# cvg/limap

Measured on AMD Instinct MI355X. Metric: 3D line candidates scored/sec (100 views x 500 segs per GPU, matched topk=10), higher is better.
Workload: dtype f64

## Files before the change

### limap_amd/csrc/lt_api_run.cpp

```cpp
#include "lt_host.h"

using namespace lt;
using namespace lt_impl;

extern "C" {

int lt_upload(lt_ctx *ctx) {
  LT_RANGE("lt_upload (match rows + job tables -> HBM)");
  LT_FINISH(ctx);
  if (!ctx->inited) return fail(ctx, LT_ERR_STATE, "upload before Init");
  if (ctx->uploaded) return LT_OK;
  HIPCHK(ctx, hipSetDevice(ctx->device));
  double t0 = now_ms();
  build_job_tables(ctx);
  ctx->blk_vorder_ok = false;
  int rc;
  {
    std::vector<char> need((size_t)std::max(ctx->n_img, 1), 0);
    for (size_t j = 0; j < ctx->job_imgs.size(); ++j) {
      need[(size_t)ctx->job_imgs[j]] = 1;
      for (int nb : ctx->job_nbs[j]) need[(size_t)nb] = 1;
    }
    std::vector<int> list;
    ctx->max_needed_segs = 0;
    for (int i = 0; i < ctx->n_img; ++i)
      if (need[(size_t)i]) {
        list.push_back(i);
        ctx->max_needed_segs = std::max(ctx->max_needed_segs, ctx->seg_off[i + 1] - ctx->seg_off[i]);
      }
    ctx->n_needed = (int)list.size();
    if (list.empty()) list.push_back(0);
    if ((rc = upload_vec(ctx, ctx->d_needed, list))) return rc;
  }
  if ((rc = upload_vec(ctx, ctx->d_nb_off, ctx->h_nb_off))) return rc;
  if ((rc = upload_vec(ctx, ctx->d_blk_img, ctx->h_blk_img))) return rc;
  if ((rc = upload_vec(ctx, ctx->d_blk_nb, ctx->h_blk_nb))) return rc;
  if ((rc = upload_vec(ctx, ctx->d_blk_slot, ctx->h_blk_slot))) return rc;
  if ((rc = upload_vec(ctx, ctx->d_blk_order, ctx->h_blk_order))) return rc;
  if ((rc = upload_vec(ctx, ctx->d_blk_line_base, ctx->h_blk_line_base))) return rc;
  if (ctx->job_mode == 1) {
    std::vector<long long> call_first_blk(ctx->job_imgs.size() + 1, 0);
    for (size_t j = 0; j < ctx->job_imgs.size(); ++j) call_first_blk[j + 1] = call_first_blk[j] + (long long)ctx->job_nbs[j].size();
    std::vector<int> job_pos(ctx->n_img, -1);
    for (size_t j = 0; j < ctx->job_imgs.size(); ++j) job_pos[ctx->job_imgs[j]] = (int)j;
    std::vector<long long> m_off(ctx->n_blk + 1, 0);
    std::vector<lt::RowDesc> desc((size_t)std::max(ctx->n_blk, 1));
    {
      long long b = 0;
      for (int i = 0; i < ctx->n_img; ++i) {
        int j = job_pos[i];
        if (j < 0) continue;
        for (size_t k = 0; k < ctx->job_nbs[j].size(); ++k, ++b) {
          long long cb = call_first_blk[j] + (long long)k;
          const long long n = ctx->h_m_off[cb + 1] - ctx->h_m_off[cb];
          m_off[b + 1] = m_off[b] + n;
          desc[(size_t)b] = lt::RowDesc{ctx->h_c_off[(size_t)cb], ctx->h_ovf_off[(size_t)cb], m_off[b], (int)n, ctx->h_line0[(size_t)cb]};
        }
      }
    }
    ctx->P = m_off[ctx->n_blk];
    ctx->n_conn = ctx->P;
    ctx->max_rows = 0;
    for (int bq = 0; bq < ctx->n_blk; ++bq) ctx->max_rows = std::max(ctx->max_rows, m_off[bq + 1] - m_off[bq]);
    if (ctx->P >= (1ll << 32) - 1) return fail(ctx, LT_ERR_ARGUMENT, "too many match rows in one batch (>= 2^32-1)");
    ENSURE(ctx, ctx->d_m_pairs, sizeof(int) * (size_t)std::max<long long>(ctx->P, 1));
    const size_t total_w = ctx->h_m_pairs.size();
    if (sizeof(int) * std::max<size_t>(total_w, 1) > ctx->d_c_stream.cap) {
      HIPCHK(ctx, hipStreamSynchronize(ctx->stream));
      ctx->streamed_ints = 0;
      ENSURE(ctx, ctx->d_c_stream, sizeof(int) * std::max<size_t>(total_w, 1));
    }
    {
      const size_t sent = std::min(ctx->streamed_ints, total_w);
      if (total_w > sent)
        HIPCHK(ctx, hipMemcpyAsync(ctx->d_c_stream.as<int>() + sent, ctx->h_m_pairs.data() + sent, sizeof(int) * (total_w - sent),
                                   hipMemcpyHostToDevice, ctx->stream));
      ctx->streamed_ints = total_w;
    }
    if ((rc = upload_vec(ctx, ctx->d_ovf, ctx->h_ovf))) return rc;
    if ((rc = upload_vec(ctx, ctx->d_rowdesc, desc))) return rc;
    const bool extras_cfg = (ctx->cfg.use_vp && !ctx->cfg.disable_vp_triangulation) ||
                            (ctx->pts_ready && (!ctx->cfg.disable_many_points_triangulation || !ctx->cfg.disable_one_point_triangulation));
    bool try_ln = ctx->rows_sorted && ctx->n_blk > 0 && ctx->P > 0 && ctx->max_nb_segs <= 1024 && !extras_cfg &&
                  !test_switch("LT_GEN_ROW_SLOTS") && !test_switch("LT_GEN_NO_LDS_TABLE");
    for (size_t cb = 0; try_ln && cb < ctx->h_ovf_off.size(); ++cb)
      if (ctx->h_ovf_off[cb] >= 0) try_ln = false;
    ctx->rows_ln = false;
    ctx->ln_slots = 0;
    if (try_ln) {
      ctx->ln_slots = gen_slots_ln(ctx->max_own_segs);
      const size_t n_entries = (size_t)std::max<long long>(ctx->h_blk_line_base[ctx->n_blk], 1);
      ENSURE(ctx, ctx->d_run_len, 4 * n_entries);
      ENSURE(ctx, ctx->d_base_bl, 4 * n_entries);
      ENSURE(ctx, ctx->d_slot_row0, 4 * (size_t)ctx->n_blk * (size_t)ctx->ln_slots);
      ENSURE(ctx, ctx->d_blk_nruns, 4 * (size_t)ctx->n_blk);
      ENSURE(ctx, ctx->d_ln_flag, 4);
      HIPCHK(ctx, hipMemsetAsync(ctx->d_ln_flag.p, 0, 4, ctx->stream));
      launch_rows_ln(ctx->stream, ctx->n_blk, ctx->ln_slots, ctx->d_rowdesc.p, ctx->d_c_stream.as<unsigned>(),
                     ctx->d_blk_line_base.as<long long>(), ctx->d_base_bl.as<unsigned>(), ctx->d_blk_nruns.as<int>(),
                     ctx->d_run_len.as<unsigned>(), ctx->d_slot_row0.as<unsigned>(), ctx->d_m_pairs.as<unsigned short>(),
                     ctx->d_ln_flag.as<int>());
      std::vector<unsigned> rnd0((size_t)ctx->n_blk + 1, 0u);
      for (int bq = 0; bq < ctx->n_blk; ++bq) rnd0[(size_t)bq + 1] = rnd0[(size_t)bq] + (unsigned)((m_off[bq + 1] - m_off[bq] + 63) / 64);
      ctx->n_round_slots = (long long)rnd0[(size_t)ctx->n_blk];
      if ((rc = upload_vec(ctx, ctx->d_blk_rnd0, rnd0))) return rc;
      int flag = 0;
      HIPCHK(ctx, hipMemcpyAsync(&flag, ctx->d_ln_flag.p, 4, hipMemcpyDeviceToHost, ctx->stream));
      HIPCHK(ctx, hipStreamSynchronize(ctx->stream));
      ctx->rows_ln = flag == 0;
    }
    if (!ctx->rows_ln)
      launch_expand_rows(ctx->stream, ctx->n_blk, ctx->d_rowdesc.p, ctx->d_c_stream.as<unsigned>(), ctx->d_ovf.as<unsigned>(),
                         ctx->d_m_pairs.as<unsigned>());
    if ((rc = upload_vec(ctx, ctx->d_m_off, m_off))) return rc;
    {
      std::vector<int> vo((size_t)std::max(ctx->n_blk, 1), 0);
      for (int b = 0; b < ctx->n_blk; ++b) vo[(size_t)b] = b;
      std::stable_sort(vo.begin(), vo.begin() + ctx->n_blk, [&](int x, int y) {
        return ctx->h_blk_nb[(size_t)x] != ctx->h_blk_nb[(size_t)y] ? ctx->h_blk_nb[(size_t)x] < ctx->h_blk_nb[(size_t)y]
                                                                    : ctx->h_blk_img[(size_t)x] < ctx->h_blk_img[(size_t)y];
      });
      if ((rc = upload_vec(ctx, ctx->d_blk_vorder, vo))) return rc;
      ctx->blk_vorder_ok = true;
    }
    ENSURE(ctx, ctx->d_blkrec, blk_rec_bytes() * (size_t)std::max(ctx->n_blk, 1));
    launch_build_blk(ctx->stream, ctx->n_blk, ctx->d_m_off.as<long long>(), ctx->d_blk_img.as<int>(),
                     ctx->d_blk_nb.as<int>(), ctx->d_blk_slot.as<int>(), ctx->d_seg_off.as<long long>(),
                     ctx->d_blk_line_base.as<long long>(), ctx->d_blkrec.p);
  } else if (ctx->job_mode == 2) {
    ctx->h_item_off.assign(ctx->G + 1, 0);
    std::vector<int> blk_chunk_off((size_t)std::max(ctx->n_blk, 1), 0);
    ctx->max_chunks = 1;
    long long items = 0, conns = 0;
    for (int i = 0; i < ctx->n_img; ++i) {
      long long per_node = 0, conn_node = 0;
      for (long long b = ctx->h_nb_off[i]; b < ctx->h_nb_off[i + 1]; ++b) {
        int i2 = ctx->h_blk_nb[b];
        long long M2 = ctx->seg_off[i2 + 1] - ctx->seg_off[i2];
        blk_chunk_off[(size_t)b] = (int)per_node;
        ctx->max_chunks = std::max(ctx->max_chunks, (int)((M2 + 63) / 64));
        per_node += (M2 + 63) / 64;
        conn_node += M2;
      }
      for (long long g = ctx->seg_off[i]; g < ctx->seg_off[i + 1]; ++g) {
        ctx->h_item_off[g] = items;
        items += per_node;
        conns += conn_node;
      }
    }
    ctx->h_item_off[ctx->G] = items;
    ctx->P = items;
    ctx->n_conn = conns;
    if ((rc = upload_vec(ctx, ctx->d_item_off, ctx->h_item_off))) return rc;
// ... 36 lines not shown
  }
  ctx->stat_survivors = -1;
  if (derr == 5) {
    if (ctx->ex_retry_depth > 0 || !ctx->ex_staged_set[ctx->pend_set])
      return fail(ctx, LT_ERR_RUNTIME, "internal: candidate staging overflow outside the one-pass exhaustive mode");
    ctx->ex_two_pass = true;
    if (hp && hp[3] > 0 && ctx->n_conn > 0)
      ctx->ex_frac = 1.4 * (double)hp[3] * (double)ex_regions() / (double)ctx->n_conn;
    if (ctx->in_run_async) return LT_OK;
    ctx->ex_retry_depth = 1;
    int rc2 = lt_run_device_async(ctx);
    if (!rc2) rc2 = finish_run(ctx);
    ctx->ex_retry_depth = 0;
    return rc2;
  }
  if (derr == 8) {
    if (ctx->score_two_kernels)
      return fail(ctx, LT_ERR_RUNTIME, "internal: device flag 8 outside the one-kernel scoring form");
    ctx->score_two_kernels = true;
    if (ctx->in_run_async) return LT_OK;
    const int depth = ctx->ex_retry_depth;
    ctx->ex_retry_depth = depth + 1;
    int rc2 = lt_run_device_async(ctx);
    if (!rc2) rc2 = finish_run(ctx);
    ctx->ex_retry_depth = depth;
    return rc2;
  }
  if (derr == 7) {
    if (ctx->ex_retry_depth > 1)
      return fail(ctx, LT_ERR_RUNTIME, "internal: pair chunk overflow outside the split scoring form");
    ctx->score_fused = true;
    if (ctx->in_run_async) return LT_OK;
    const int depth = ctx->ex_retry_depth;
    ctx->ex_retry_depth = depth + 1;
    int rc2 = lt_run_device_async(ctx);
    if (!rc2) rc2 = finish_run(ctx);
    ctx->ex_retry_depth = depth;
    return rc2;
  }
  ctx->timers[17] = ctx->timers[18] = 0.0;
  if (hp && ctx->ex_staged_set[ctx->pend_set]) {
    ctx->timers[17] = (double)hp[3] * (double)ex_regions();
    ctx->timers[18] = (double)ctx->ex_region_cap * (double)ex_regions();
  }
  if (ctx->job_mode == 2 && derr == 0 && ctx->n_conn > 0) {
    if (hp && ctx->ex_staged_set[ctx->pend_set])
      ctx->ex_frac = std::max(1.4 * (double)hp[3] * (double)ex_regions() / (double)ctx->n_conn, 1e-4);
    else if (ctx->ex_frac <= 0.0)
      ctx->ex_frac = std::max(2.2 * (double)ctx->C_last / (double)ctx->n_conn, 1e-4);
    ctx->ex_two_pass = false;
  }
  if (derr == 4) return fail(ctx, LT_ERR_RUNTIME, "internal: the scan of the node counts did not complete");
  if (derr == 3)
    return fail(ctx, LT_ERR_RUNTIME, "more than 65 000 candidates on one connection of the exhaustive mode (16-bit counts)");
  if (derr == 2)
    return fail(ctx, LT_ERR_RUNTIME, "map::at: a point shared by two lines has a point3D_id that is not among the SfM points");
  if (derr != 0) return fail(ctx, LT_ERR_RUNTIME, "IndexError! Out-of-index matches detected on the device");
  float ms;
  ctx->timers[1] = ctx->timers[2] = ctx->timers[7] = 0.0;
  const int eg = ctx->pend_ev_gen_end, ep = ctx->pend_ev_place_end;
  const hipEvent_t e_start = ctx->pend_ev_start ? ctx->pend_ev_start : ev[0];
  const hipEvent_t e_end = hp ? ctx->pend_ev_end : ev[7];
  HIPCHK(ctx, hipEventElapsedTime(&ms, e_start, e_end));
  ctx->timers[0] = ms;
  const bool sampled = ctx->pend_sampled;
  if (sampled) {
  const hipEvent_t kA[4] = {e_start, ev[eg], ev[ep], ev[5]}, kB[4] = {ev[eg], ev[ep], ev[5], e_end};
  const int kT[4] = {3, 4, 5, 6};
  for (int k = 0; k < 4; ++k) {
    HIPCHK(ctx, hipEventElapsedTime(&ms, kA[k], kB[k]));
    ctx->timers[kT[k]] = ms;
  }
  ctx->timers[13] = ctx->timers[14] = ctx->timers[15] = 0.0;
  if (ctx->pend_fine_gen && ctx->job_mode == 1 && ctx->n_blk > 0 && ctx->max_rows > 0) {
    if (hipEventElapsedTime(&ms, ev[8], ev[9]) == hipSuccess) ctx->timers[13] = ms;
    if (hipEventElapsedTime(&ms, ev[9], ev[10]) == hipSuccess) ctx->timers[14] = ms;
  }
  if (ctx->pend_fine_score && ctx->C_last > 0 && hipEventElapsedTime(&ms, ev[11], ev[5]) == hipSuccess) ctx->timers[15] = ms;
  (void)hipGetLastError();
  ++ctx->timer_stage_runs;
  }
  ctx->timers[11] = (double)ctx->stat_pairs_eval;
  for (int k = 0; k < 24; ++k) {
    const bool stage = (k >= 3 && k <= 6) || (k >= 13 && k <= 15);
    if (k != 8 && k != 9 && k != 10 && k != 12 && k != 16 && (sampled || !stage)) ctx->timer_sums[k] += ctx->timers[k];
  }
  ++ctx->timer_runs;
  return LT_OK;
}
}
}
int lt_sync(lt_ctx *ctx) { return finish_run(ctx); }

int lt_run_device_async(lt_ctx *ctx) {
  LT_RANGE("lt_run_device (enqueue: generation, placement, scoring, selection)");
  if (!ctx->uploaded) return fail(ctx, LT_ERR_STATE, "lt_run_device before lt_upload");
  if (!ctx->h_pinned) LT_FINISH(ctx);
  ctx->shard_keys = ctx->shard_own_keys = -1;
  if (ctx->inited && !ctx->best_c_set.empty())
    for (int idx : ctx->job_imgs)
      if (ctx->best_c_set[(size_t)idx] == 1) {
        ctx->best_c_set[(size_t)idx] = 0;
        for (long long g = ctx->seg_off[idx]; g < ctx->seg_off[idx + 1]; ++g) {
          if ((size_t)g < ctx->has_best.size()) ctx->has_best[(size_t)g] = 0;
          if ((size_t)g < ctx->valid_edges.cnt.size()) ctx->valid_edges.cnt[(size_t)g] = 0;
        }
      }
  const int set = ctx->run_pending ? (ctx->pend_set ^ 1) : 0;
  if (ctx->h_pinned) std::memset(ctx->h_pinned + 8 * set, 0, 32);
  if (set == 1 && !ctx->ev_b[0])
    for (auto &e : ctx->ev_b) HIPCHK(ctx, hipEventCreate(&e));
  hipEvent_t *ev = set ? ctx->ev_b : ctx->ev;
  long long *hp = ctx->h_pinned ? ctx->h_pinned + 8 * set : nullptr;
  ctx->ex_staged_set[set] = false;
  int sample_n = 8;
  if (const char *e = getenv("LT_TIMER_SAMPLE")) sample_n = std::max(1, atoi(e));
  if (!(ctx->run_pending && hp)) ctx->async_seq = 0;
  const bool sampled = (ctx->async_seq++ % (unsigned)sample_n) == 0u;
  const bool fine_gen = sampled && fine_gen_timers(), fine_score = sampled && fine_timers();
  HIPCHK(ctx, hipSetDevice(ctx->device));
  hipStream_t st = ctx->stream;
  const long long G = ctx->G, P = ctx->P;
  {
    int rcp = upload_points(ctx);
    if (rcp) return rcp;
  }
  GenCfg gcfg = make_gen(ctx);
  if (ctx->pts_ready && (!ctx->cfg.disable_many_points_triangulation || !ctx->cfg.disable_one_point_triangulation))
    gcfg.force_undecided = 1;
  const ScoreCfg scfg = make_score(ctx);
  const bool score_f32 = !test_switch("LT_TEST_SCORE_F64");
  const bool guards_on = scfg.l3.th_scaleinv > 0.0 && scfg.l3.score_th > 0.0 && scfg.l3.score_th < 1.0 &&
                         !test_switch("LT_TEST_NO_SCORE_GUARDS");
  const double guard2 = guards_on ? (scfg.l3.th_scaleinv * (1.0 + 1e-6)) * (scfg.l3.th_scaleinv * (1.0 + 1e-6)) : 1e300;
  ENSURE(ctx, ctx->d_err, sizeof(int));
  ENSURE(ctx, ctx->d_pair_counter, 8);
  ENSURE(ctx, ctx->d_result3, 32);
  ENSURE(ctx, ctx->d_pairs, sizeof(PairRec) * (size_t)std::max(ctx->n_blk, 1));
  ENSURE(ctx, ctx->d_tri_off, sizeof(long long) * (size_t)(G + 1));
  hipEvent_t ev_start = ev[0];
  if (ctx->run_pending && hp && ctx->pend_ev_end && !test_switch("LT_TEST_OWN_START_EVENT")) ev_start = ctx->pend_ev_end;
  else HIPCHK(ctx, hipEventRecord(ev[0], st));
  const int n_status_scan = (int)((G + 1 + 255) / 256) + 1;
  const int n_status = n_status_scan + score3_tile_buckets() * 16 + ex_regions() * 16 + 8 * 16;
  ENSURE(ctx, ctx->d_scan_status, 8 * (size_t)n_status);
  const bool ln_job = ctx->job_mode == 1 && ctx->rows_ln && ctx->rows_sorted;
  if (ln_job) ENSURE(ctx, ctx->d_blk_surv, 4 * (size_t)std::max(ctx->n_blk, 1));
  launch_build_pairs(st, ctx->n_blk, ctx->d_blk_img.as<int>(), ctx->d_blk_nb.as<int>(), ctx->d_cams.as<Cam>(),
                     ctx->d_pairs.as<PairRec>(), ctx->d_err.as<int>(),
                     ctx->d_pair_counter.as<unsigned long long>(), ctx->d_scan_status.as<unsigned long long>(),
                     n_status, ln_job ? ctx->d_blk_surv.as<unsigned>() : nullptr);

  bool node_rec_valid = false;
  long long C_known = -1;
  long long C_bound = 0;
  int ev_gen_end = 3, ev_place_end = 4;
  long long C_run = 0;
  if (ctx->job_mode == 1) {
    const size_t Pn = (size_t)std::max<long long>(P, 1);
    const bool fast = ctx->rows_sorted;
    {
      const bool vp_now = ctx->cfg.use_vp && !ctx->cfg.disable_vp_triangulation;
      const bool pts_now = ctx->pts_ready && (!ctx->cfg.disable_many_points_triangulation || !ctx->cfg.disable_one_point_triangulation);
      if (ctx->rows_ln && (vp_now || pts_now)) {
        launch_expand_rows(st, ctx->n_blk, ctx->d_rowdesc.p, ctx->d_c_stream.as<unsigned>(), ctx->d_ovf.as<unsigned>(),
                           ctx->d_m_pairs.as<unsigned>());
        ctx->rows_ln = false;
      }
    }
    const bool ln = ctx->rows_ln && fast;
    const int ln_slots = ln ? ctx->ln_slots : 0;
    if (ln) ENSURE(ctx, ctx->d_round_count, 4 * (size_t)std::max<long long>(ctx->n_round_slots, 1));
    const long long n_waves = (long long)ctx->n_blk * gen_groups(ctx->max_rows);
    const long long n_slots_all = (long long)ctx->n_blk * (ln ? ln_slots : gen_slots(ctx->max_rows));
    const long long n_entries = ctx->h_blk_line_base[ctx->n_blk];
    const bool vp_on = ctx->cfg.use_vp && !ctx->cfg.disable_vp_triangulation;
    if (vp_on && !ctx->vp_ready) return fail(ctx, LT_ERR_STATE, "use_vp is set but InitVPResults was not called");
    const bool pts_any = ctx->pts_ready && (!ctx->cfg.disable_many_points_triangulation || !ctx->cfg.disable_one_point_triangulation);
    const bool many_on = pts_any && !ctx->cfg.disable_many_points_triangulation;
    const bool one_on = pts_any && !ctx->cfg.disable_one_point_triangulation;
    const bool pts_on = pts_any;
    const bool extras = vp_on || pts_on;
    long long staged_total = -1;
    if (!extras) {
      ENSURE(ctx, ctx->d_st_c, sizeof(CRec) * Pn); ENSURE(ctx, ctx->d_st_l, sizeof(double) * Pn);
      ENSURE(ctx, ctx->d_st_key, 4 * (Pn + 64));
    }
    ENSURE(ctx, ctx->d_wave_count, 4 * (size_t)(n_waves + 1));
    if (extras) ENSURE(ctx, ctx->d_wave_pos, 8 * (size_t)(n_waves + 1));
    const long long *group_base = extras ? ctx->d_wave_pos.as<long long>() : nullptr;
    ENSURE(ctx, ctx->d_ntris_u, 4 * (size_t)(G + 1));
    if (fast) {
      const size_t nb = 4 * (size_t)std::max<long long>(n_entries, 1);
      const void *before = ctx->d_cnt_bl.p;
      ENSURE(ctx, ctx->d_cnt_bl, nb);
      ENSURE(ctx, ctx->d_base_bl, nb);
      if (ctx->d_cnt_bl.p != before || !ctx->cnt_bl_clean || ctx->cnt_bl_bytes != nb) {
        HIPCHK(ctx, hipMemsetAsync(ctx->d_cnt_bl.p, 0, ctx->d_cnt_bl.cap, st));
        ctx->cnt_bl_bytes = nb;
      }
      ctx->cnt_bl_clean = false;
    }
    const bool no_lds_table = test_switch("LT_GEN_NO_LDS_TABLE") != nullptr;
    int lds_segs = (!no_lds_table && ctx->max_nb_segs <= 1024) ? ctx->max_nb_segs : 0;
    int lds_segs1 = (!no_lds_table && ctx->max_own_segs <= 1024) ? ctx->max_own_segs : 0;
    if (lds_segs + lds_segs1 > 1024) lds_segs1 = 0;
    if (ln) {
      lds_segs = std::max(ctx->max_nb_segs, 1);
      lds_segs1 = 0;
    }
    {
      ENSURE(ctx, ctx->d_st_row, 8 * Pn);
      ENSURE(ctx, ctx->d_surv_count, 4 * (size_t)(n_slots_all + 1));
      if (!ctx->d_seg_gates.p) return fail(ctx, LT_ERR_STATE, "segment gate records missing (Init not run?)");
      auto gen = [&](int phase) {
      launch_gen_split(st, ctx->n_blk, ctx->max_rows, gcfg, ctx->d_m_off.as<long long>(), ctx->d_m_pairs.as<int>(),
                       ctx->d_blk_img.as<int>(), ctx->d_blk_nb.as<int>(), ctx->d_blk_slot.as<int>(),
                       ctx->d_seg_off.as<long long>(), ctx->d_cams.as<Cam>(), ctx->d_segs.as<Seg>(),
                       ctx->d_pairs.as<PairRec>(), ctx->d_blk_line_base.as<long long>(), ctx->d_st_c.as<CRec>(),
                       ctx->d_st_l.as<double>(), ctx->d_st_key.as<unsigned>(), ctx->d_wave_count.as<unsigned>(),
                       fast ? ctx->d_cnt_bl.as<unsigned>() : nullptr, lds_segs, lds_segs1, ctx->d_st_row.p,
                       ctx->d_surv_count.as<unsigned>(), G, ctx->d_seg_gates.p, ctx->d_blkrec.p, fine_gen ? &ev[8] : nullptr,
                       vp_on ? ctx->d_seg_vp.as<double>() : nullptr,
                       vp_on ? ctx->d_seg_has_vp.as<unsigned char>() : nullptr,
                       pts_on ? ctx->d_seg_pt_off.as<long long>() : nullptr, pts_on ? ctx->d_seg_pts.p : nullptr,
                       (pts_on && ctx->sfm_given) ? ctx->d_sfm_xyz.as<double>() : nullptr, ctx->d_err.as<int>(),
                       many_on ? 1 : 0, one_on ? 1 : 0, group_base, phase, ln_slots, ctx->d_m_pairs.as<unsigned short>(),
                       ctx->d_run_len.as<unsigned>(), ctx->d_slot_row0.as<unsigned>(), ctx->d_blk_surv.as<unsigned>(),
                       ctx->d_blk_rnd0.as<unsigned>(), ctx->d_round_count.as<unsigned>(),
                       (ctx->blk_vorder_ok && !test_switch("LT_TEST_GATES_IMAGE_MAJOR")) ? ctx->d_blk_vorder.as<int>() : nullptr,
                       test_switch("LT_TEST_TRI_STATIC") ? nullptr
                           : (unsigned *)(ctx->d_scan_status.as<unsigned long long>() + n_status_scan + score3_tile_buckets() * 16 + ex_regions() * 16));
      };
      if (!extras) {
        gen(0);
      } else {
        gen(1);
        HIPCHK(ctx, hipMemsetAsync(ctx->d_wave_count.as<unsigned>() + n_waves, 0, 4, st));
        size_t tmp = scan_temp_bytes_u32_to_i64(n_waves + 1);
        ENSURE(ctx, ctx->d_scan_tmp, std::max<size_t>(tmp, 16));
        if (launch_scan_u32_to_i64(st, ctx->d_scan_tmp.p, tmp, n_waves + 1, ctx->d_wave_count.as<unsigned>(),
                                   ctx->d_wave_pos.as<long long>()) != 0)
          return fail(ctx, LT_ERR_HIP, "rocprim scan failed");
        HIPCHK(ctx, hipMemcpyAsync(&staged_total, ctx->d_wave_pos.as<long long>() + n_waves, 8, hipMemcpyDeviceToHost, st));
        HIPCHK(ctx, hipStreamSynchronize(st));
        if (staged_total >= (1ll << 32) - 1)
          return fail(ctx, LT_ERR_ARGUMENT, "too many candidates in one batch (>= 2^32-1): triangulate the images in smaller batches");
        const size_t Sn = (size_t)std::max<long long>(staged_total, 1);
        ENSURE(ctx, ctx->d_st_c, sizeof(CRec) * Sn); ENSURE(ctx, ctx->d_st_l, sizeof(double) * Sn);
        ENSURE(ctx, ctx->d_st_key, 4 * Sn);
        gen(2);
      }
    }
    bool gen_event_pending = false;
    if (fine_gen && ctx->n_blk > 0 && ctx->max_rows > 0) ev_gen_end = 10;
    else gen_event_pending = true;
    long long *hC = hp;
    long long hC_fallback = 0;
    if (!hC) hC = &hC_fallback;
    if (fast) {
      ENSURE(ctx, ctx->d_node_rec, 16 * (size_t)std::max<long long>(G, 1));
      launch_node_prefix(st, G, ctx->d_node_img.as<int>(), ctx->d_seg_off.as<long long>(),
                         ctx->d_nb_off.as<long long>(), ctx->d_blk_line_base.as<long long>(),
                         ctx->d_cnt_bl.as<unsigned>(), ctx->d_base_bl.as<unsigned>(), ctx->d_ntris_u.as<unsigned>(),
                         ctx->d_tri_off.as<long long>(), ctx->d_scan_status.as<unsigned long long>(),
                         ctx->d_err.as<int>(), ctx->d_node_rec.p);
      node_rec_valid = true;
      ctx->cnt_bl_clean = true;
      const long long bound = P;
      constexpr long long kCountFreeBytes = 48ll << 30;
      const bool perm_bound = !test_switch("LT_TEST_PLACE_COPY");
      const long long per_cand = (perm_bound ? 4 : (long long)(sizeof(CRec) + 8)) + 8 + 4 + 4 + (long long)cand_meta_bytes() +
                                 (long long)score_split_entry_bytes() * 256 / 64;
      if (extras) {
        C_known = staged_total;
      } else if (ctx->h_pinned && bound * per_cand <= kCountFreeBytes && !test_switch("LT_TEST_SYNC_COUNT")) {
        C_known = -1;
        C_bound = bound;
      } else {
        HIPCHK(ctx, hipMemcpyAsync(hC, ctx->d_tri_off.as<long long>() + G, 8, hipMemcpyDeviceToHost, st));
        HIPCHK(ctx, hipStreamSynchronize(st));
        C_known = *hC;
      }
    } else {
      ENSURE(ctx, ctx->d_wave_pos, 8 * (size_t)(n_waves + 1));
      HIPCHK(ctx, hipMemsetAsync(ctx->d_wave_count.as<unsigned>() + n_waves, 0, 4, st));
      size_t tmp = scan_temp_bytes_u32_to_i64(n_waves + 1);
      ENSURE(ctx, ctx->d_scan_tmp, std::max<size_t>(tmp, 16));
      if (launch_scan_u32_to_i64(st, ctx->d_scan_tmp.p, tmp, n_waves + 1, ctx->d_wave_count.as<unsigned>(),
                                 ctx->d_wave_pos.as<long long>()) != 0)
        return fail(ctx, LT_ERR_HIP, "rocprim scan failed");
      HIPCHK(ctx, hipMemcpyAsync(hC, ctx->d_wave_pos.as<long long>() + n_waves, 8, hipMemcpyDeviceToHost, st));
      HIPCHK(ctx, hipStreamSynchronize(st));
      C_known = *hC;
    }
    const bool perm_mode = fast && !test_switch("LT_TEST_PLACE_COPY");
    ctx->perm_mode = perm_mode;
    ctx->compact_valid = !perm_mode;
    if (C_known < 0) {
      const size_t Bn = (size_t)std::max<long long>(C_bound, 1);
      const bool got = (perm_mode ? ctx->d_place_perm.ensure(4 * Bn)
                                  : (ctx->d_cand.ensure(sizeof(CRec) * Bn) && ctx->d_lite.ensure(sizeof(double) * Bn))) &&
                       ctx->d_score.ensure(8 * Bn) && ctx->d_edge_flag.ensure(4 * Bn) && ctx->d_cand_node.ensure(4 * Bn) &&
                       ctx->d_cand_meta.ensure(cand_meta_bytes() * Bn);
      if (!got) {
        (void)hipGetLastError();
        HIPCHK(ctx, hipMemcpyAsync(hC, ctx->d_tri_off.as<long long>() + G, 8, hipMemcpyDeviceToHost, st));
        HIPCHK(ctx, hipStreamSynchronize(st));
        C_known = *hC;
      }
    }
    if (C_known >= 0) C_bound = C_known;
    const size_t Cn = (size_t)std::max<long long>(C_bound, 1);
    if (perm_mode) {
      ENSURE(ctx, ctx->d_place_perm, 4 * Cn);
    } else {
      ENSURE(ctx, ctx->d_cand, sizeof(CRec) * Cn); ENSURE(ctx, ctx->d_lite, sizeof(double) * Cn);
    }
    ENSURE(ctx, ctx->d_score, 8 * Cn); ENSURE(ctx, ctx->d_edge_flag, 4 * Cn); ENSURE(ctx, ctx->d_cand_node, 4 * Cn);
    ctx->cand_cap = (long long)Cn;
    if (fast) {
      launch_place(st, ctx->n_blk, ctx->max_rows, ctx->d_m_off.as<long long>(), ctx->d_blk_img.as<int>(),
                   ctx->d_seg_off.as<long long>(), ctx->d_blk_line_base.as<long long>(),
                   ctx->d_base_bl.as<unsigned>(), ctx->d_wave_count.as<unsigned>(), ctx->d_tri_off.as<long long>(),
                   ctx->d_st_c.as<CRec>(), ctx->d_st_l.as<double>(), ctx->d_st_key.as<unsigned>(),
                   ctx->d_cand.as<CRec>(), ctx->d_lite.as<double>(), ctx->d_cand_node.as<unsigned>(), group_base,
                   perm_mode ? ctx->d_place_perm.as<unsigned>() : nullptr, ctx->d_blk_surv.as<unsigned>(),
                   ctx->d_blk_rnd0.as<unsigned>(), ln ? ctx->d_round_count.as<unsigned>() : nullptr);
    } else {
      ENSURE(ctx, ctx->d_keys, 4 * Cn); ENSURE(ctx, ctx->d_rows, 4 * Cn);
      ENSURE(ctx, ctx->d_skeys, 4 * Cn); ENSURE(ctx, ctx->d_srows, 4 * Cn);
      launch_pack_keys(st, ctx->n_blk, ctx->max_rows, ctx->d_m_off.as<long long>(),
                       ctx->d_wave_count.as<unsigned>(), ctx->d_wave_pos.as<long long>(),
                       ctx->d_st_key.as<unsigned>(), ctx->d_keys.as<unsigned>(), ctx->d_rows.as<unsigned>(), group_base);
      if (C_known > 0) {
        int end_bit = bits_for(G + 1);
        size_t tmp = sort_temp_bytes(C_known, end_bit);
        ENSURE(ctx, ctx->d_sort_tmp, std::max<size_t>(tmp, 16));
        if (launch_sort(st, ctx->d_sort_tmp.p, tmp, C_known, ctx->d_keys.as<unsigned>(), ctx->d_skeys.as<unsigned>(),
                        ctx->d_rows.as<unsigned>(), ctx->d_srows.as<unsigned>(), end_bit) != 0)
          return fail(ctx, LT_ERR_HIP, "rocprim radix sort failed");
      }
      launch_node_offsets(st, C_known, G, ctx->d_skeys.as<unsigned>(), ctx->d_tri_off.as<long long>());
      launch_permute(st, C_known, ctx->d_skeys.as<unsigned>(), ctx->d_srows.as<unsigned>(), ctx->d_st_c.as<CRec>(),
                     ctx->d_st_l.as<double>(), ctx->d_cand.as<CRec>(), ctx->d_lite.as<double>(),
                     ctx->d_cand_node.as<unsigned>());
    }
    if (fine_score && C_bound > 0) ev_place_end = 11;
    else if (sampled) HIPCHK(ctx, hipEventRecord(ev[4], st));
    if (gen_event_pending) ev_gen_end = ev_place_end;
  } else if (ctx->job_mode == 2) {
    ctx->perm_mode = false;
    ctx->compact_valid = true;
    const size_t In = (size_t)std::max<long long>(P, 1);
    const bool vp_on = ctx->cfg.use_vp && !ctx->cfg.disable_vp_triangulation;
    if (vp_on && !ctx->vp_ready) return fail(ctx, LT_ERR_STATE, "use_vp is set but InitVPResults was not called");
    const double *seg_vp = vp_on ? ctx->d_seg_vp.as<double>() : nullptr;
    const unsigned char *seg_has_vp = vp_on ? ctx->d_seg_has_vp.as<unsigned char>() : nullptr;
    const int n_masks = vp_on ? 3 : 1;
    const bool pts_any = ctx->pts_ready && (!ctx->cfg.disable_many_points_triangulation || !ctx->cfg.disable_one_point_triangulation);
    const int many_on = (pts_any && !ctx->cfg.disable_many_points_triangulation) ? 1 : 0;
    const int one_on = (pts_any && !ctx->cfg.disable_one_point_triangulation) ? 1 : 0;
    const double *sfm_xyz = (pts_any && ctx->sfm_given) ? ctx->d_sfm_xyz.as<double>() : nullptr;
    ENSURE(ctx, ctx->d_masks, pts_any ? 128 * In : 8 * (In * n_masks + 1)); ENSURE(ctx, ctx->d_mask_cnt, 4 * (In + 1));
    ENSURE(ctx, ctx->d_mask_pos, 8 * (In + 1));
    const bool plain = !pts_any && !vp_on;
    bool staged = plain && ctx->h_pinned && !ctx->ex_two_pass && P > 0 && !test_switch("LT_TEST_EX_TWO_PASS") &&
                  !test_switch("LT_TEST_EX_PASS1_BLOCK");
    long long ex_cap = 0;
    unsigned region_cap = 0;
    unsigned long long *ex_ctr = ctx->d_scan_status.as<unsigned long long>() + n_status_scan + score3_tile_buckets() * 16;
    if (staged) {
      double frac = ctx->ex_frac > 0.0 ? ctx->ex_frac : 1.0 / 6.0;
      long long slack = 65536;
      if (const char *f = test_switch("LT_TEST_EX_CAP_FRAC")) {
        frac = atof(f);
        slack = 0;
      }
      const long long want = (long long)((double)ctx->n_conn * frac) + slack;
      const long long nreg = ex_regions();
      const long long rc8 = ((want + nreg - 1) / nreg + 63) & ~63ll;
      ex_cap = nreg * rc8;
      if (ex_cap >= (1ll << 32) - 1 || ex_cap * 210 > (64ll << 30)) staged = false;
      else {
        region_cap = (unsigned)rc8;
        const size_t Bn = (size_t)ex_cap;
        const bool got = ctx->d_st_c.ensure(sizeof(CRec) * Bn) && ctx->d_st_l.ensure(sizeof(double) * Bn) &&
                         ctx->d_st_key.ensure(4 * Bn) && ctx->d_place_perm.ensure(4 * Bn) && ctx->d_score.ensure(8 * Bn) &&
                         ctx->d_edge_flag.ensure(4 * Bn) && ctx->d_cand_node.ensure(4 * Bn) &&
                         ctx->d_cand_meta.ensure(cand_meta_bytes() * Bn) && ctx->d_ex_rec.ensure(4 * Bn) &&
                         ctx->d_ex_ent.ensure(8 * Bn) && ctx->d_ex_z.ensure(4 * Bn);
        if (!got) {
          (void)hipGetLastError();
          staged = false;
        }
      }
    }
    ctx->ex_staged_set[set] = staged;
    if (pts_any) {
      launch_gen_exhaustive_pts(st, false, P, gcfg, ctx->d_item_off.as<long long>(), G, ctx->d_node_img.as<int>(),
                                ctx->d_nb_off.as<long long>(), ctx->d_blk_nb.as<int>(), ctx->d_seg_off.as<long long>(),
                                ctx->d_cams.as<Cam>(), ctx->d_segs.as<Seg>(), ctx->d_pairs.as<PairRec>(),
                                ctx->d_masks.as<unsigned short>(), ctx->d_mask_cnt.as<unsigned>(), nullptr, nullptr,
                                nullptr, seg_vp, seg_has_vp, ctx->d_seg_pt_off.as<long long>(), ctx->d_seg_pts.p,
                                sfm_xyz, ctx->d_err.as<int>(), many_on, one_on, ctx->d_blk_chunk_off.as<int>(),
                                ctx->max_nb, ctx->max_chunks, ctx->d_seg_gates.p);
    } else {
      if (plain && !test_switch("LT_TEST_EX_PASS1_BLOCK"))
        launch_gates_exhaustive(st, ctx->n_blk, ctx->max_chunks, P, gcfg, ctx->d_item_off.as<long long>(),
                                ctx->d_blk_img.as<int>(), ctx->d_blk_nb.as<int>(), ctx->d_seg_off.as<long long>(),
                                ctx->d_cams.as<Cam>(), ctx->d_segs.as<Seg>(), ctx->d_pairs.as<PairRec>(),
                                ctx->d_masks.as<unsigned long long>(), ctx->d_blk_chunk_off.as<int>(), ctx->d_seg_gates.p,
                                staged ? ctx->d_ex_ent.as<unsigned long long>() : nullptr, ex_ctr, region_cap,
                                ctx->d_err.as<int>());
      else
      launch_gen_exhaustive(st, false, P, gcfg, ctx->d_item_off.as<long long>(), G, ctx->d_node_img.as<int>(),
                            ctx->d_nb_off.as<long long>(), ctx->d_blk_nb.as<int>(), ctx->d_seg_off.as<long long>(),
                            ctx->d_cams.as<Cam>(), ctx->d_segs.as<Seg>(), ctx->d_pairs.as<PairRec>(),
                            ctx->d_masks.as<unsigned long long>(), nullptr, nullptr, nullptr, seg_vp, seg_has_vp,
                            ctx->d_blk_chunk_off.as<int>(), ctx->max_nb, ctx->max_chunks, ctx->d_seg_gates.p);
      if (staged) {
        HIPCHK(ctx, hipMemsetAsync(ctx->d_masks.p, 0, 8 * In, st));
        launch_tri_exhaustive(st, ctx->d_ex_ent.as<unsigned long long>(), ex_ctr, region_cap, gcfg, P,
                              ctx->d_item_off.as<long long>(), ctx->d_blk_img.as<int>(), ctx->d_blk_nb.as<int>(),
                              ctx->d_nb_off.as<long long>(), ctx->d_seg_off.as<long long>(), ctx->d_cams.as<Cam>(),
                              ctx->d_segs.as<Seg>(), ctx->d_pairs.as<PairRec>(), ctx->d_blk_chunk_off.as<int>(),
                              ctx->d_masks.as<unsigned long long>(), ctx->d_st_c.as<CRec>(), ctx->d_st_l.as<double>(),
                              ctx->d_st_key.as<unsigned>(), ctx->d_ex_z.as<float>());
      }
      if (!plain) launch_popc(st, P, ctx->d_masks.as<unsigned long long>(), ctx->d_mask_cnt.as<unsigned>(), n_masks);
    }
    if (plain) {
      HIPCHK(ctx, hipMemsetAsync(ctx->d_masks.as<unsigned long long>() + P, 0, 8, st));
      size_t tmp = scan_temp_bytes_popc(P + 1);
      ENSURE(ctx, ctx->d_scan_tmp, std::max<size_t>(tmp, 16));
      if (launch_scan_popc(st, ctx->d_scan_tmp.p, tmp, P + 1, ctx->d_masks.as<unsigned long long>(),
                           ctx->d_mask_pos.as<long long>()) != 0)
        return fail(ctx, LT_ERR_HIP, "rocprim scan failed");
    } else {
      HIPCHK(ctx, hipMemsetAsync(ctx->d_mask_cnt.as<unsigned>() + P, 0, 4, st));
      size_t tmp = scan_temp_bytes_u32_to_i64(P + 1);
      ENSURE(ctx, ctx->d_scan_tmp, std::max<size_t>(tmp, 16));
      if (launch_scan_u32_to_i64(st, ctx->d_scan_tmp.p, tmp, P + 1, ctx->d_mask_cnt.as<unsigned>(),
                                 ctx->d_mask_pos.as<long long>()) != 0)
        return fail(ctx, LT_ERR_HIP, "rocprim scan failed");
    }
    if (staged) {
      launch_tri_offsets_ex(st, G, ctx->d_item_off.as<long long>(), ctx->d_mask_pos.as<long long>(), P, -1, ex_cap,
                            ctx->d_tri_off.as<long long>(), ctx->d_err.as<int>());
      if (sampled) HIPCHK(ctx, hipEventRecord(ev[3], st));
      launch_place_exhaustive(st, ex_ctr, region_cap, ctx->d_ex_ent.as<unsigned long long>(),
                              ctx->d_st_key.as<unsigned>(), ctx->d_item_off.as<long long>(),
                              ctx->d_blk_chunk_off.as<int>(), ctx->d_masks.as<unsigned long long>(),
                              ctx->d_mask_pos.as<long long>(), P, ctx->d_tri_off.as<long long>(), G,
                              ctx->d_place_perm.as<unsigned>(), (hp ? hp : ctx->d_result3.as<long long>()) + 3);
      ctx->ex_region_cap = region_cap;
      launch_cand_node(st, G, ctx->d_tri_off.as<long long>(), ctx->d_cand_node.as<unsigned>());
      ctx->perm_mode = true;
      ctx->compact_valid = false;
      ctx->cand_cap = ex_cap;
      C_known = -1;
      C_bound = ex_cap;
      if (sampled) HIPCHK(ctx, hipEventRecord(ev[4], st));
    } else {
    long long total = 0;
    HIPCHK(ctx, hipMemcpyAsync(&total, ctx->d_mask_pos.as<long long>() + P, 8, hipMemcpyDeviceToHost, st));
    HIPCHK(ctx, hipStreamSynchronize(st));
    if (sampled) HIPCHK(ctx, hipEventRecord(ev[3], st));
    const size_t Cn = (size_t)std::max<long long>(total, 1);
    ENSURE(ctx, ctx->d_cand, sizeof(CRec) * Cn); ENSURE(ctx, ctx->d_lite, sizeof(double) * Cn);
    ENSURE(ctx, ctx->d_score, 8 * Cn); ENSURE(ctx, ctx->d_edge_flag, 4 * Cn);
    ctx->cand_cap = (long long)Cn;
    if (pts_any)
      launch_gen_exhaustive_pts(st, true, P, gcfg, ctx->d_item_off.as<long long>(), G, ctx->d_node_img.as<int>(),
                                ctx->d_nb_off.as<long long>(), ctx->d_blk_nb.as<int>(), ctx->d_seg_off.as<long long>(),
                                ctx->d_cams.as<Cam>(), ctx->d_segs.as<Seg>(), ctx->d_pairs.as<PairRec>(),
                                ctx->d_masks.as<unsigned short>(), ctx->d_mask_cnt.as<unsigned>(),
                                ctx->d_mask_pos.as<long long>(), ctx->d_cand.as<CRec>(), ctx->d_lite.as<double>(),
                                seg_vp, seg_has_vp, ctx->d_seg_pt_off.as<long long>(), ctx->d_seg_pts.p, sfm_xyz,
                                ctx->d_err.as<int>(), many_on, one_on, ctx->d_blk_chunk_off.as<int>(), ctx->max_nb,
                                ctx->max_chunks, ctx->d_seg_gates.p);
    else if (!vp_on && !test_switch("LT_TEST_EX_PASS2_BLOCK"))
      launch_fill_exhaustive(st, ctx->n_blk, P, gcfg, ctx->d_item_off.as<long long>(), ctx->d_blk_img.as<int>(),
                             ctx->d_blk_nb.as<int>(), ctx->d_nb_off.as<long long>(), ctx->d_seg_off.as<long long>(),
                             ctx->d_cams.as<Cam>(), ctx->d_segs.as<Seg>(), ctx->d_pairs.as<PairRec>(),
                             ctx->d_masks.as<unsigned long long>(), ctx->d_mask_pos.as<long long>(),
                             ctx->d_cand.as<CRec>(), ctx->d_lite.as<double>(), ctx->d_blk_chunk_off.as<int>());
    else
      launch_gen_exhaustive(st, true, P, gcfg, ctx->d_item_off.as<long long>(), G, ctx->d_node_img.as<int>(),
                            ctx->d_nb_off.as<long long>(), ctx->d_blk_nb.as<int>(), ctx->d_seg_off.as<long long>(),
                            ctx->d_cams.as<Cam>(), ctx->d_segs.as<Seg>(), ctx->d_pairs.as<PairRec>(),
                            ctx->d_masks.as<unsigned long long>(), ctx->d_mask_pos.as<long long>(),
                            ctx->d_cand.as<CRec>(), ctx->d_lite.as<double>(), seg_vp, seg_has_vp,
                            ctx->d_blk_chunk_off.as<int>(), ctx->max_nb, ctx->max_chunks, ctx->d_seg_gates.p);
    launch_tri_offsets_ex(st, G, ctx->d_item_off.as<long long>(), ctx->d_mask_pos.as<long long>(), P, total, -1,
                          ctx->d_tri_off.as<long long>(), ctx->d_err.as<int>());
    ENSURE(ctx, ctx->d_cand_node, 4 * Cn);
    launch_cand_node(st, G, ctx->d_tri_off.as<long long>(), ctx->d_cand_node.as<unsigned>());
    C_known = total;
    C_bound = total;
    if (sampled) HIPCHK(ctx, hipEventRecord(ev[4], st));
    }
  } else {
    ctx->perm_mode = false;
    ctx->compact_valid = true;
    HIPCHK(ctx, hipMemsetAsync(ctx->d_tri_off.p, 0, sizeof(long long) * (size_t)(G + 1), st));
    ENSURE(ctx, ctx->d_cand, sizeof(CRec)); ENSURE(ctx, ctx->d_lite, sizeof(double));
    ENSURE(ctx, ctx->d_score, 8); ENSURE(ctx, ctx->d_edge_flag, 4); ENSURE(ctx, ctx->d_cand_node, 4);
    C_known = 0;
    C_bound = 0;
    for (int k = 3; k <= 4; ++k)
      if (sampled) HIPCHK(ctx, hipEventRecord(ev[k], st));
  }

  if (score3_lds_bytes(ctx->max_nb, score_f32) > 160 * 1024)
    return fail(ctx, LT_ERR_ARGUMENT, "too many neighbours for the scoring kernel's LDS budget");
  {
    if (ctx->h_nb_off[ctx->n_img] >= (1ll << 24))
      return fail(ctx, LT_ERR_ARGUMENT, "too many (image, neighbour) blocks in one batch (>= 2^24)");
    ENSURE(ctx, ctx->d_cand_meta, cand_meta_bytes() * (size_t)std::max<long long>(C_bound, 1));
    ENSURE(ctx, ctx->d_tile_order, 64 * 128);
    const bool tile_classes = !test_switch("LT_TEST_NO_TILE_CLASSES") && ctx->job_mode == 1;
    const unsigned tile_cap = (unsigned)(((std::max<long long>(C_bound, 1) + 63) / 64 + 7) / 8);
    if (tile_classes) ENSURE(ctx, ctx->d_tile_list, 16 * (size_t)tile_cap * (size_t)score3_tile_buckets());
    const bool score_sorted = score_f32 && ctx->job_mode == 2 && !test_switch("LT_TEST_SCORE_UNSORTED");
    if (score_sorted) {
      ENSURE(ctx, ctx->d_perm, 4 * (size_t)std::max<long long>(C_bound, 1));
      ENSURE(ctx, ctx->d_rng, 4 * (size_t)std::max<long long>(C_bound, 1));
    }
    const bool staged_sorted = score_sorted && ctx->perm_mode && ctx->job_mode == 2;
    C_run = C_bound;
    const bool split = score_f32 && !ctx->score_fused && !test_switch("LT_SCORE_FUSED") &&
                       (tile_classes || staged_sorted || test_switch("LT_SCORE_SPLIT"));
    long long sp_chunks = 0;
    int sp_slot_cap = ctx->job_mode == 2 ? 64 : 256;
    if (split) {
      const long long n_tiles_b = (std::max<long long>(C_bound, 1) + 63) / 64;
      sp_chunks = score_split_chunks(std::max<long long>(C_bound, 1));
      if (const char *e = test_switch("LT_TEST_SPLIT_CHUNKS")) sp_chunks = std::max(0, atoi(e));
      if (const char *e = test_switch("LT_TEST_SPLIT_SLOT")) sp_slot_cap = std::max(1, atoi(e));
      ENSURE(ctx, ctx->d_sp_slots, score_split_entry_bytes() * (size_t)sp_slot_cap * (size_t)n_tiles_b);
      ENSURE(ctx, ctx->d_sp_cnt, 4 * (size_t)n_tiles_b);
      ENSURE(ctx, ctx->d_sp_ovf, 4 * (size_t)n_tiles_b);
      ENSURE(ctx, ctx->d_sp_pairs, score_split_chunk_bytes() * (size_t)std::max<long long>(sp_chunks, 1));
      ENSURE(ctx, ctx->d_sp_desc, 8 * (size_t)std::max<long long>(sp_chunks, 1));
    }
    const bool pair_classes = split && tile_classes && !test_switch("LT_TEST_NO_PAIR_CLASSES");
    if (pair_classes) {
      ENSURE(ctx, ctx->d_pc_cnt, 128 * (size_t)score3_tile_buckets());
      ENSURE(ctx, ctx->d_pc_list, 8 * (size_t)tile_cap * (size_t)score3_tile_buckets());
    }
    launch_score3(st, C_bound, G, ctx->d_tri_off.as<long long>(), ctx->d_cand_node.as<unsigned>(), ctx->d_cand_meta.p,
                  ctx->perm_mode ? ctx->d_st_c.as<CRec>() : ctx->d_cand.as<CRec>(), ctx->d_node_img.as<int>(),
                  ctx->d_nb_off.as<long long>(), ctx->d_blk_order.as<int>(), ctx->d_cams.as<Cam>(),
                  ctx->d_score.as<double>(), ctx->d_pair_counter.as<unsigned long long>(), ctx->max_nb, scfg,
                  guard2, fine_score ? ev[11] : nullptr, ctx->d_tile_order.as<unsigned>(), score_f32,
                  (ctx->perm_mode && !staged_sorted) ? ctx->d_place_perm.as<unsigned>()
                                                     : (score_sorted ? ctx->d_perm.as<unsigned>() : nullptr),
                  score_sorted ? ctx->d_rng.p : nullptr, ctx->perm_mode && !staged_sorted,
                  tile_classes ? (unsigned *)(ctx->d_scan_status.as<unsigned long long>() + n_status_scan) : nullptr,
                  tile_classes ? ctx->d_tile_list.as<unsigned>() : nullptr, tile_cap,
                  staged_sorted ? ctx->d_place_perm.as<unsigned>() : nullptr,
                  staged_sorted ? ctx->d_ex_rec.as<unsigned>() : nullptr,
                  staged_sorted ? ctx->d_ex_z.as<float>() : nullptr, ctx->d_err.as<int>(),
                  split ? ctx->d_sp_slots.p : nullptr, sp_slot_cap, ctx->d_sp_cnt.as<unsigned>(),
                  ctx->d_sp_ovf.as<unsigned>(), ctx->d_sp_pairs.p, ctx->d_sp_desc.p, sp_chunks, sampled ? ev[5] : nullptr,
                  node_rec_valid ? ctx->d_node_rec.p : nullptr, pair_classes ? ctx->d_pc_cnt.as<unsigned>() : nullptr,
                  pair_classes ? ctx->d_pc_list.p : nullptr, tile_cap,
                  (((ctx->score_two_kernels || test_switch("LT_SCORE_TWO_KERNELS") || ctx->n_img >= (1 << 18))
                        ? 0 : (test_switch("LT_TEST_Q_LOSE_TILE") ? 2 : 1)) |
                   (test_switch("LT_TEST_DENSE_TABLES") ? 4 : 0) | (test_switch("LT_TEST_DENSE_FEW_ROWS") ? 8 : 0)));
    if (C_bound <= 0 && sampled) HIPCHK(ctx, hipEventRecord(ev[5], st));
  }
  ENSURE(ctx, ctx->d_best_idx, 8 * (size_t)std::max<long long>(G, 1));
  ENSURE(ctx, ctx->d_nvalid, 4 * (size_t)(G + 1));
  ENSURE(ctx, ctx->d_edge_off, 8 * (size_t)(G + 1));
  ENSURE(ctx, ctx->d_best_c, sizeof(Cand) * (size_t)std::max<long long>(G, 1));
  ENSURE(ctx, ctx->d_best_score, 8 * (size_t)std::max<long long>(G, 1));
  ENSURE(ctx, ctx->d_best_src, 8 * (size_t)std::max<long long>(G, 1));
  ENSURE(ctx, ctx->d_ntris, 4 * (size_t)std::max<long long>(G, 1));
  launch_select(st, G, ctx->d_tri_off.as<long long>(), ctx->d_score.as<double>(), scfg.fullscore_th,
                scfg.max_valid_conns, ctx->d_best_idx.as<long long>(), ctx->d_edge_flag.as<unsigned>(),
                ctx->d_nvalid.as<unsigned>(), ctx->perm_mode ? ctx->d_st_c.as<CRec>() : ctx->d_cand.as<CRec>(),
                ctx->perm_mode ? ctx->d_st_l.as<double>() : ctx->d_lite.as<double>(),
                ctx->d_best_c.as<Cand>(), ctx->d_best_score.as<double>(), ctx->d_best_src.as<int>(),
                ctx->d_ntris.as<int>(), ctx->job_mode == 2, ctx->d_err.as<int>(),
                ctx->d_pair_counter.as<unsigned long long>(), hp ? hp : ctx->d_result3.as<long long>(),
                ctx->perm_mode ? ctx->d_place_perm.as<unsigned>() : nullptr);
  if (!hp) HIPCHK(ctx, hipEventRecord(ev[7], st));
  HIPCHK(ctx, hipGetLastError());
  hipEvent_t ev_end = nullptr;
  if (hp) {
    if (!ctx->ev_end[0])
      for (auto &e : ctx->ev_end) HIPCHK(ctx, hipEventCreate(&e));
    ev_end = ctx->ev_end[ctx->run_seq++ % 3u];
    HIPCHK(ctx, hipEventRecord(ev_end, st));
  }
  int rc_prev = LT_OK;
  if (ctx->run_pending) {
    ctx->in_run_async = true;
    rc_prev = finish_run(ctx);
    ctx->in_run_async = false;
  }
  ctx->run_pending = true;
  ctx->pend_ev_start = ev_start;
  ctx->pend_sampled = sampled;
  ctx->pend_ev_end = ev_end;
  ctx->pend_set = set;
  ctx->pend_count_on_device = C_known < 0;
  ctx->pend_fine_gen = fine_gen;
  ctx->pend_fine_score = fine_score;
  ctx->pend_C = C_run;
  ctx->pend_ev_gen_end = ev_gen_end;
  ctx->pend_ev_place_end = ev_place_end;
  ctx->ran = true;
  ctx->downloaded = false;
  ctx->host_view_valid = false;
  return rc_prev;
}

int lt_run_device(lt_ctx *ctx) {
  int rc = lt_run_device_async(ctx);
  if (rc) return rc;
  return finish_run(ctx);
}

extern "C++" {
namespace lt_impl {
void define_best_of_other_images(lt_ctx *ctx) {
  for (int i = 0; i < ctx->n_img; ++i)
    if (!ctx->best_c_set[(size_t)i]) {
      const long long a = ctx->seg_off[i], b = ctx->seg_off[i + 1];
      if (b > a) std::memset((void *)(ctx->best_c + a), 0, sizeof(Cand) * (size_t)(b - a));
      ctx->best_c_set[(size_t)i] = 2;
    }
}
}
}

extern "C++" {
namespace lt_impl {
int materialize_compact(lt_ctx *ctx) {
  if (ctx->host_view_valid) return LT_OK;
  const long long C = ctx->C_last;
  const size_t Cn = (size_t)std::max<long long>(C, 1);
  ENSURE(ctx, ctx->d_hcand, sizeof(Cand) * Cn); ENSURE(ctx, ctx->d_hlite, sizeof(CandLite) * Cn);
  launch_host_view(ctx->stream, C, ctx->perm_mode ? ctx->d_place_perm.as<unsigned>() : nullptr,
                   ctx->perm_mode ? ctx->d_st_c.as<CRec>() : ctx->d_cand.as<CRec>(),
                   ctx->perm_mode ? ctx->d_st_l.as<double>() : ctx->d_lite.as<double>(), ctx->d_hcand.as<Cand>(),
                   ctx->d_hlite.as<CandLite>());
  HIPCHK(ctx, hipStreamSynchronize(ctx->stream));
  ctx->host_view_valid = true;
  return LT_OK;
}
}
}

int lt_download(lt_ctx *ctx) {
  LT_RANGE("lt_download (per-node results -> host)");
  LT_FINISH(ctx);
  if (!ctx->ran) return fail(ctx, LT_ERR_STATE, "lt_download before lt_run_device");
  if (ctx->downloaded) return LT_OK;
  HIPCHK(ctx, hipSetDevice(ctx->device));
  double t0 = now_ms();
  hipStream_t st = ctx->stream;
  const long long G = ctx->G;
  HIPCHK(ctx, hipMemsetAsync(ctx->d_nvalid.as<unsigned>() + G, 0, 4, st));
  {
    size_t tmp = scan_temp_bytes_u32_to_i64(G + 1);
    ENSURE(ctx, ctx->d_scan_tmp, std::max<size_t>(tmp, 16));
    if (launch_scan_u32_to_i64(st, ctx->d_scan_tmp.p, tmp, G + 1, ctx->d_nvalid.as<unsigned>(),
                               ctx->d_edge_off.as<long long>()) != 0)
      return fail(ctx, LT_ERR_HIP, "rocprim scan failed");
  }
  std::vector<long long> tri_off(G + 1), edge_off(G + 1);
  HIPCHK(ctx, hipMemcpyAsync(tri_off.data(), ctx->d_tri_off.p, 8 * (size_t)(G + 1), hipMemcpyDeviceToHost, st));
  HIPCHK(ctx, hipMemcpyAsync(edge_off.data(), ctx->d_edge_off.p, 8 * (size_t)(G + 1), hipMemcpyDeviceToHost, st));
  HIPCHK(ctx, hipStreamSynchronize(st));
  ctx->C = tri_off[G];
  ctx->E = edge_off[G];
  ENSURE(ctx, ctx->d_edges, 8 * (size_t)std::max<long long>(ctx->E, 1));
  launch_edge_fill(st, G, ctx->d_tri_off.as<long long>(), ctx->d_edge_flag.as<unsigned>(),
                   ctx->d_edge_off.as<long long>(), ctx->perm_mode ? ctx->d_st_c.as<CRec>() : ctx->d_cand.as<CRec>(),
                   ctx->d_edges.as<int>(), ctx->perm_mode ? ctx->d_place_perm.as<unsigned>() : nullptr);
  const size_t Gn = (size_t)std::max<long long>(G, 1), En = (size_t)std::max<long long>(ctx->E, 1);
  const size_t o_bc = 0, o_bs = o_bc + sizeof(Cand) * Gn, o_src = o_bs + 8 * Gn, o_nt = o_src + 8 * Gn,
               o_ed = (o_nt + 4 * Gn + 15) / 16 * 16, total = o_ed + 8 * En;
  lt_host::HostBlock hb = lt_host::host_block_acquire(total);
  if (!hb.p) return fail(ctx, LT_ERR_RUNTIME, "out of host memory for the results");
  struct Rel {
    lt_host::HostBlock b;
    ~Rel() { lt_host::host_block_release(b); }
  } rel{hb};
  char *base = (char *)hb.p;
  const Cand *bc = (const Cand *)(base + o_bc);
  const double *bs = (const double *)(base + o_bs);
  const int *bsrc = (const int *)(base + o_src);
  const int *nt = (const int *)(base + o_nt);
  const int *edges = (const int *)(base + o_ed);
  if (G > 0) {
    HIPCHK(ctx, hipMemcpyAsync(base + o_bc, ctx->d_best_c.p, sizeof(Cand) * (size_t)G, hipMemcpyDeviceToHost, st));
    HIPCHK(ctx, hipMemcpyAsync(base + o_bs, ctx->d_best_score.p, 8 * (size_t)G, hipMemcpyDeviceToHost, st));
    HIPCHK(ctx, hipMemcpyAsync(base + o_src, ctx->d_best_src.p, 8 * (size_t)G, hipMemcpyDeviceToHost, st));
    HIPCHK(ctx, hipMemcpyAsync(base + o_nt, ctx->d_ntris.p, 4 * (size_t)G, hipMemcpyDeviceToHost, st));
  }
  if (ctx->E > 0)
    HIPCHK(ctx, hipMemcpyAsync(base + o_ed, ctx->d_edges.p, 8 * (size_t)ctx->E, hipMemcpyDeviceToHost, st));
  HIPCHK(ctx, hipStreamSynchronize(st));
  const long long pool_base = (long long)ctx->valid_edges.pool.size();
  ctx->valid_edges.pool.insert(ctx->valid_edges.pool.end(), edges, edges + 2 * (size_t)ctx->E);
  long long pairs = 0;
  const long long n_job = (long long)ctx->job_imgs.size();
#pragma omp parallel for num_threads(lt::host_threads()) schedule(dynamic, 4) reduction(+ : pairs)
  for (long long j = 0; j < n_job; ++j) {
    const int idx = ctx->job_imgs[(size_t)j];
    ctx->best_c_set[(size_t)idx] = 1;
    for (long long g = ctx->seg_off[idx]; g < ctx->seg_off[idx + 1]; ++g) {
      ctx->n_tris[g] = nt[g];
      pairs += (long long)nt[g] * nt[g];
      ctx->has_best[g] = nt[g] > 0 ? 1 : 0;
      ctx->best_c[g] = bc[g];
      ctx->best_score[g] = bs[g];
      ctx->best_src2[2 * g] = nt[g] > 0 ? ctx->img_ids[bsrc[2 * g]] : 0;
      ctx->best_src2[2 * g + 1] = nt[g] > 0 ? bsrc[2 * g + 1] : 0;
// ... 55 lines not shown
```

### limap_amd/csrc/lt_devfn.h

```cpp
#pragma once

#include "lt_device.h"

namespace lt {

static __device__ __forceinline__ int lane_id() { return threadIdx.x & 63; }
static __device__ __forceinline__ unsigned long long lanemask_lt() {
  return (1ull << lane_id()) - 1ull;
}
template <class Op>
static __device__ __forceinline__ int wave_reduce_dpp(int v, Op op) {
  v = op(v, __builtin_amdgcn_update_dpp(v, v, 0x111, 0xF, 0xF, false));
  v = op(v, __builtin_amdgcn_update_dpp(v, v, 0x112, 0xF, 0xF, false));
  v = op(v, __builtin_amdgcn_update_dpp(v, v, 0x114, 0xF, 0xF, false));
  v = op(v, __builtin_amdgcn_update_dpp(v, v, 0x118, 0xF, 0xF, false));
  v = op(v, __builtin_amdgcn_update_dpp(v, v, 0x142, 0xA, 0xF, false));
  v = op(v, __builtin_amdgcn_update_dpp(v, v, 0x143, 0xC, 0xF, false));
  return __builtin_amdgcn_readlane(v, 63);
}
static __device__ __forceinline__ unsigned wave_incl_scan_u32(unsigned x) {
  int v = (int)x;
  v += __builtin_amdgcn_update_dpp(0, v, 0x111, 0xF, 0xF, true);
  v += __builtin_amdgcn_update_dpp(0, v, 0x112, 0xF, 0xF, true);
  v += __builtin_amdgcn_update_dpp(0, v, 0x114, 0xF, 0xF, true);
  v += __builtin_amdgcn_update_dpp(0, v, 0x118, 0xF, 0xF, true);
  v += __builtin_amdgcn_update_dpp(0, v, 0x142, 0xA, 0xF, true);
  v += __builtin_amdgcn_update_dpp(0, v, 0x143, 0xC, 0xF, true);
  return (unsigned)v;
}
static __device__ __forceinline__ int wave_max_i32(int v) {
  return wave_reduce_dpp(v, [](int a, int b) { return a > b ? a : b; });
}
static __device__ __forceinline__ unsigned wave_max_u32(unsigned v) {
  return (unsigned)wave_reduce_dpp((int)v, [](int a, int b) { return (unsigned)a > (unsigned)b ? a : b; });
}
static __device__ __forceinline__ unsigned wave_min_u32(unsigned v) {
  return (unsigned)wave_reduce_dpp((int)v, [](int a, int b) { return (unsigned)a < (unsigned)b ? a : b; });
}
static __device__ __forceinline__ float wave_max_f32_nan(float v) {
  return __int_as_float(wave_reduce_dpp(__float_as_int(v), [](int a, int b) {
    const float x = __int_as_float(a), y = __int_as_float(b);
    return (y > x || y != y) ? b : a;
  }));
}
static __device__ __forceinline__ double readlane_f64(double v, int src) {
  const int lo = __builtin_amdgcn_readlane(__double2loint(v), src);
  const int hi = __builtin_amdgcn_readlane(__double2hiint(v), src);
  return __hiloint2double(hi, lo);
}

static __device__ __forceinline__ void wave_lds_sync() {
  asm volatile("s_waitcnt lgkmcnt(0)" ::: "memory");
  __builtin_amdgcn_wave_barrier();
}


struct GenOut {
  CRec r;
  double unc;
};

static __device__ __forceinline__ bool tri_point(const Cam &c1, d3 r1, const Cam &c2, d3 r2, d3 *out) {
  d3 C1 = cam_center(c1), C2 = cam_center(c2);
  double a00 = dot(r1, r1), a10 = -dot(r2, r1), a11 = dot(r2, r2);
  double b0 = dot(r1, sub(C2, C1));
  double b1 = dot(r2, sub(C1, C2));
  bool sw = fabs(a11) > fabs(a00);
  double dd0 = sw ? a11 : a00, dd1 = sw ? a00 : a11;
  double q0 = sw ? b1 : b0, q1 = sw ? b0 : b1;
  double l10 = a10 / dd0;
  double s1d = dd1 - l10 * (dd0 * l10);
  double y1 = q1 - l10 * q0;
  double z0 = q0 / dd0, z1 = y1 / s1d;
  double s0 = z0 - l10 * z1;
  double x0 = sw ? z1 : s0, x1 = sw ? s0 : z1;
  d3 p = add(add(add(scale(r1, x0), C1), scale(r2, x1)), C2);
  p = d3{0.5 * p.x, 0.5 * p.y, 0.5 * p.z};
  if (cam_depth(c1, p) < kEps || cam_depth(c2, p) < kEps) return false;
  *out = p;
  return true;
}

static __device__ __forceinline__ double sensitivity(const Cam &c, d3 s, d3 e, d3 dir3) {
  d2 ps = cam_project(c, s), pe = cam_project(c, e);
  d2 mid = d2{0.5 * (ps.x + pe.x), 0.5 * (ps.y + pe.y)};
  d3 ray = cam_ray(c, mid);
  double cv = fabs(dot(dir3, ray));
  return 90 - acos(cv) * 180.0 / kPi;
}

static __device__ __forceinline__ bool sensitivity_gt(const GenCfg &cfg, const Cam &c, d3 s, d3 e, d3 dir3) {
  d2 ps = cam_project(c, s), pe = cam_project(c, e);
  d2 mid = d2{0.5 * (ps.x + pe.x), 0.5 * (ps.y + pe.y)};
  d3 ray = cam_ray(c, mid);
  double cv = fabs(dot(dir3, ray));
  if (cv > cfg.sens_hi) return true;
  if (cv < cfg.sens_lo) return false;
  return 90 - acos(cv) * 180.0 / kPi > cfg.sens_th;
}

static __device__ __forceinline__ double epipolar_iou(const Seg &s1, const Seg &s2, const double *F) {
  L2 l2{mk2(s2.x1, s2.y1), mk2(s2.x2, s2.y2)};
  double ln2 = len(l2);
  d3 lc2 = mk3(s2.lc[0], s2.lc[1], s2.lc[2]);
  d3 eps = unit(mv(F, mk3(s1.x1, s1.y1, 1.0)));
  d3 hs = cross(lc2, eps);
  double zs = hs.z + kEps;
  d2 cs = d2{hs.x / zs, hs.y / zs};
  d3 epe = unit(mv(F, mk3(s1.x2, s1.y2, 1.0)));
  d3 he = cross(lc2, epe);
  double ze = he.z + kEps;
  d2 ce = d2{he.x / ze, he.y / ze};
  d2 dv = dir(l2);
  double c1v = dot(sub(cs, l2.s), dv) / ln2;
  double c2v = dot(sub(ce, l2.s), dv) / ln2;
  if (c1v > c2v) {
    double t = c1v; c1v = c2v; c2v = t;
  }
  return (dmin(c2v, 1.0) - dmax(c1v, 0.0)) / (dmax(c2v, 1.0) - dmin(c1v, 0.0));
}

static __device__ __forceinline__ bool tri_line(const Cam &c1, const Cam &c2, const Seg &s1, const Seg &s2,
                                                const double *Bv, d3 *ps_o, d3 *pe_o, double *z_start,
                                                double *z_end, double *d21, double *d22) {
  d3 r1s = mk3(s1.rs[0], s1.rs[1], s1.rs[2]), r1e = mk3(s1.re[0], s1.re[1], s1.re[2]);
  d3 c2s = mk3(s2.rs[0], s2.rs[1], s2.rs[2]), c2e = mk3(s2.re[0], s2.re[1], s2.re[2]);
  d3 u = mk3(-c2s.x, -c2s.y, -c2s.z), v = mk3(-c2e.x, -c2e.y, -c2e.z);
  double k0 = u.y * v.z - v.y * u.z;
  double k1 = u.z * v.x - v.z * u.x;
  double k2 = u.x * v.y - v.x * u.y;
  d3 B = mk3(Bv[0], Bv[1], Bv[2]);
  d3 C1 = cam_center(c1);
  d3 ps, pe;
  {
    double det = (k0 * r1s.x + k1 * r1s.y) + k2 * r1s.z;
    double id = 1.0 / det;
    double x0 = ((k0 * id) * B.x + (k1 * id) * B.y) + (k2 * id) * B.z;
    ps = add(scale(r1s, x0), C1);
    *z_start = cam_depth(c1, ps);
  }
  {
    double det = (k0 * r1e.x + k1 * r1e.y) + k2 * r1e.z;
    double id = 1.0 / det;
    double x0 = ((k0 * id) * B.x + (k1 * id) * B.y) + (k2 * id) * B.z;
    pe = add(scale(r1e, x0), C1);
    *z_end = cam_depth(c1, pe);
  }
  *ps_o = ps;
  *pe_o = pe;
  if (*z_start < kEps || *z_end < kEps) return false;
  *d21 = cam_depth(c2, ps);
  *d22 = cam_depth(c2, pe);
  if (*d21 < kEps || *d22 < kEps) return false;
  if (isnan(ps.x) || isnan(pe.x)) return false;
  return true;
}

static __device__ __forceinline__ bool gen_gates(const GenCfg &cfg, const Seg &s1, const Seg &s2,
                                                 const double *F) {
  L2 l1{mk2(s1.x1, s1.y1), mk2(s1.x2, s1.y2)};
  L2 l2{mk2(s2.x1, s2.y1), mk2(s2.x2, s2.y2)};
  if (len(l1) <= cfg.min_length_2d) return false;
  if (len(l2) <= cfg.min_length_2d) return false;
  if (cfg.disable_algebraic) return false;
  d3 n2 = mk3(s2.n[0], s2.n[1], s2.n[2]);
  d3 r1s = mk3(s1.rs[0], s1.rs[1], s1.rs[2]), r1e = mk3(s1.re[0], s1.re[1], s1.re[2]);
  double as = fabs(dot(n2, r1s));
  if (as < cfg.sin_lo) return false;
  if (!(as > cfg.sin_hi)) {
    double ang = 90 - acos(as) * 180.0 / kPi;
    if (ang < cfg.angle_th) return false;
  }
  double ae = fabs(dot(n2, r1e));
  if (ae < cfg.sin_lo) return false;
  if (!(ae > cfg.sin_hi)) {
    double ang = 90 - acos(ae) * 180.0 / kPi;
    if (ang < cfg.angle_th) return false;
  }
  double iou = epipolar_iou(s1, s2, F);
  if (iou < cfg.iou_th) return false;
  return true;
}

static __device__ __forceinline__ double fast_rcp(double x) {
  double r = __builtin_amdgcn_rcp(x);
  r = __builtin_fma(__builtin_fma(-x, r, 1.0), r, r);
  r = __builtin_fma(__builtin_fma(-x, r, 1.0), r, r);
  return r;
}

struct SegGate {
  double n[3];
  double lcx, lcy;
  double P, Q, w1;
  double sv;
  double q2;
};
static_assert(sizeof(SegGate) == 80, "SegGate layout");

static __device__ __forceinline__ void seg_gate_build(const Seg &s, SegGate *g) {
  const double vx = s.x2 - s.x1, vy = s.y2 - s.y1;
  g->n[0] = s.n[0]; g->n[1] = s.n[1]; g->n[2] = s.n[2];
  g->lcx = s.lc[0]; g->lcy = s.lc[1];
  g->P = s.lc[2] * vy;
  g->Q = -(s.lc[2] * vx);
  g->w1 = s.lc[1] * vx - s.lc[0] * vy;
// ... 620 lines not shown
```

### limap_amd/csrc/lt_device.h

```cpp
#pragma once

#include "lt_geom.h"

#include <hip/hip_runtime.h>
#include <stddef.h>

#define LT_ERR_MATCH_LINE_RANGE 1
#define LT_ERR_MATCH_NGLINE_RANGE 2

namespace lt {

struct SceneChunk {
  const double *k, *q, *t, *s;
  long long seg_begin;
  int img_begin, pad_;
};
void launch_build_scene_chunked(hipStream_t st, int n_img, long long n_segs, int n_chunks, const SceneChunk *ch,
                                const long long *seg_off, double halfpix, Cam *cams, Seg *segs,
                                const int *img_list, int n_list, long long max_segs_per_img, void *gates);

void launch_build_cams(hipStream_t st, int n, const double *k, const double *q, const double *t, Cam *cams);
void launch_build_segs(hipStream_t st, long long n_segs, int n_img, const long long *seg_off,
                       const double *segs, double halfpix, const Cam *cams, Seg *out, void *gates);
void launch_build_pairs(hipStream_t st, int n_blk, const int *blk_img, const int *blk_nb, const Cam *cams,
                        PairRec *out, int *err_flag, unsigned long long *pair_counter,
                        unsigned long long *scan_status, int n_status, unsigned *blk_surv);
size_t sort_temp_bytes(long long P, int end_bit);
int launch_sort(hipStream_t st, void *temp, size_t temp_bytes, long long P, const unsigned *keys_in,
                unsigned *keys_out, const unsigned *vals_in, unsigned *vals_out, int end_bit);
void launch_node_offsets(hipStream_t st, long long P, long long G, const unsigned *skeys, long long *conn_off);
size_t scan_temp_bytes_u32_to_i64(long long n);
size_t scan_temp_bytes_popc(long long n);
int launch_scan_popc(hipStream_t st, void *temp, size_t temp_bytes, long long n, const unsigned long long *masks,
                     long long *out);
int launch_scan_u32_to_i64(hipStream_t st, void *temp, size_t temp_bytes, long long n, const unsigned *in,
                           long long *out);
void launch_gen_exhaustive(hipStream_t st, bool fill, long long n_items, const GenCfg &cfg,
                           const long long *item_off, long long G, const int *node_img, const long long *nb_off,
                           const int *blk_nb, const long long *seg_off, const Cam *cams, const Seg *segs,
                           const PairRec *pairs, unsigned long long *masks, const long long *mask_pos,
                           CRec *out_r, double *out_unc, const double *seg_vp, const unsigned char *seg_has_vp,
                           const int *blk_chunk_off, int max_nb, int max_chunks, const void *gates);
int ex_regions();
void launch_gates_exhaustive(hipStream_t st, int n_blk, int max_chunks, long long n_items, const GenCfg &cfg,
                             const long long *item_off, const int *blk_img, const int *blk_nb, const long long *seg_off,
                             const Cam *cams, const Seg *segs, const PairRec *pairs, unsigned long long *masks,
                             const int *blk_chunk_off, const void *gates, unsigned long long *ent_out,
                             unsigned long long *ctr, unsigned region_cap, int *err_flag);
void launch_tri_exhaustive(hipStream_t st, unsigned long long *ent, const unsigned long long *ctr,
                           unsigned region_cap, const GenCfg &cfg, long long n_items, const long long *item_off,
                           const int *blk_img, const int *blk_nb, const long long *nb_off, const long long *seg_off,
                           const Cam *cams, const Seg *segs, const PairRec *pairs, const int *blk_chunk_off,
                           unsigned long long *masks, CRec *st_r, double *st_unc, unsigned *st_node, float *st_z);
void launch_place_exhaustive(hipStream_t st, const unsigned long long *ctr, unsigned region_cap,
                             const unsigned long long *ent, const unsigned *st_node, const long long *item_off,
                             const int *blk_chunk_off, const unsigned long long *masks, const long long *mask_pos,
                             long long n_items, const long long *tri_off, long long G, unsigned *perm,
                             long long *fill_out);
void launch_fill_exhaustive(hipStream_t st, int n_blk, long long n_items, const GenCfg &cfg, const long long *item_off,
                            const int *blk_img, const int *blk_nb, const long long *nb_off, const long long *seg_off,
                            const Cam *cams, const Seg *segs, const PairRec *pairs, const unsigned long long *masks,
                            const long long *mask_pos, CRec *out_r, double *out_unc, const int *blk_chunk_off);
void launch_gen_exhaustive_pts(hipStream_t st, bool fill, long long n_items, const GenCfg &cfg,
                               const long long *item_off, long long G, const int *node_img, const long long *nb_off,
                               const int *blk_nb, const long long *seg_off, const Cam *cams, const Seg *segs,
                               const PairRec *pairs, unsigned short *cnt8, unsigned *item_cnt,
                               const long long *mask_pos, CRec *out_r, double *out_unc, const double *seg_vp,
                               const unsigned char *seg_has_vp, const long long *seg_pt_off, const void *seg_pts,
                               const double *sfm_xyz, int *err_flag, int many_on, int one_on,
                               const int *blk_chunk_off, int max_nb, int max_chunks, const void *gates);
void launch_popc(hipStream_t st, long long n, const unsigned long long *masks, unsigned *cnt, int n_masks);
void launch_tri_offsets_ex(hipStream_t st, long long G, const long long *item_off, const long long *mask_pos,
                           long long n_items, long long total, long long cap, long long *tri_off, int *err_flag);

void launch_select(hipStream_t st, long long G, const long long *tri_off, const double *score, double th,
                   int max_valid, long long *best_idx, unsigned *edge_flag, unsigned *n_valid, const CRec *cand,
                   const double *cand_unc, Cand *best_c, double *best_score, int *best_src2, int *n_tris,
                   bool wide, const int *err_flag, const unsigned long long *pair_counter, long long *result3,
                   const unsigned *perm);
void launch_edge_fill(hipStream_t st, long long G, const long long *tri_off, const unsigned *edge_flag,
                      const long long *edge_off, const CRec *cand, int *edges2, const unsigned *perm);

size_t tail_rec_bytes();
size_t tail_sort_temp_bytes(long long E, int end_bit);
void launch_tail_keys(hipStream_t st, long long G, const long long *tri_off, const unsigned *edge_flag,
                      const long long *edge_off, const CRec *cand, const long long *seg_off, int kb,
                      unsigned long long *keys, const unsigned *perm, int directed);
int launch_tail_sort(hipStream_t st, void *temp, size_t temp_bytes, long long E, const unsigned long long *keys_in,
                     unsigned long long *keys_out, int end_bit);
void launch_tail_sims(hipStream_t st, long long E, const unsigned long long *skeys, const int *n_tris, const Cand *best_c,
                      const LinkCfg3 &cfg, int kb, double *sims, unsigned *mark, unsigned *keep, const unsigned char *flags);
void launch_check_keys(hipStream_t st, long long n, const unsigned long long *keys, int kb, long long G, int *bad, int directed);
void launch_outer_pass_keys(hipStream_t st, long long E, const unsigned long long *keys, int kb, long long G, unsigned *counts,
                            int min_outer, unsigned char *flags, int *changed);
void launch_keys_undirect(hipStream_t st, long long E, unsigned long long *keys, int kb);
void launch_outer_filter(hipStream_t st, long long G, const long long *tri_off, const unsigned *edge_flag, const CRec *cand,
                         const long long *seg_off, const unsigned *perm, int min_outer, unsigned char *flags, int *changed);
void launch_tail_compact(hipStream_t st, long long E, const unsigned long long *skeys, const double *sims,
                         const unsigned *keep, const long long *kpos, void *out_pairs, long long *n_out, const long long *npos,
                         int kb);
void launch_tail_gather(hipStream_t st, long long G, const unsigned *mark, const long long *pos, const Cand *best_c,
                        const double *best_score, const int *best_src2, void *recs, int *nodes, long long *n_out);

struct MLine {
  double s[3], e[3];
  double dir[3];
  double unc;
  double len;
  double seg[4];
  double pad_;
};
static_assert(sizeof(MLine) == 128, "MLine layout");
struct MBlock {
  int img, nb, slot, row0;
  int img_id, nb_id, pad_[2];
};
struct MEdge {
  int img, line, slot, ng_line;
};
void launch_merge_pairs(hipStream_t st, bool self, int n_blk, const MBlock *blks, const long long *seg_off,
                        const MLine *lines, const Cam *cams, const LinkCfg2 &l2, const LinkCfg3 &l3, double cos_guard,
                        int parity_fast, MEdge *edges, unsigned long long capacity, unsigned long long *n_edges);

void launch_track_connect(hipStream_t st, int T, const double *line7, const unsigned char *active, int all_active,
                          const LinkCfg3 &cfg, double cos_guard, unsigned long long *edges,
                          unsigned long long capacity, unsigned long long *n_edges);

}
```

### limap_amd/csrc/lt_host.h

```cpp
#pragma once

#include "lt_ctx.h"
#include "lt_hostutil.h"
#include "lt_tail.h"
#include "lt_rows.h"
#include "lt_pool.h"

#include <algorithm>
#include <atomic>
#include <parallel/algorithm>
#include <chrono>
#include <cmath>
#include <cstdio>
#include <cstring>
#include <dlfcn.h>
#include <map>
#include <mutex>
#include <queue>
#include <set>
#include <string>
#include <unordered_map>
#include <vector>

namespace lt {
void launch_fn_query(hipStream_t st, const double *in30, int by_endpoints, double *out32);
void launch_fn_gate_outcomes(hipStream_t st, int n, const double *conn30, const GenCfg &cfg, int *out10,
                             unsigned long long *iou_bits);
int gen_slots(long long max_rows);
int gen_groups(long long max_rows);
int gen_slots_ln(int max_own_segs);
int gen_max_run();
void launch_rows_ln(hipStream_t st, int n_blk, int n_slots, const void *desc, const unsigned *stream,
                    const long long *blk_line_base, unsigned *rstart, int *blk_nruns, unsigned *run_len,
                    unsigned *slot_row0, unsigned short *tr, int *ln_flag);
size_t seg_gate_bytes();
void launch_build_blk(hipStream_t st, int n_blk, const long long *m_off, const int *blk_img, const int *blk_nb,
                      const int *blk_slot, const long long *seg_off, const long long *blk_line_base, void *blkrec);
size_t blk_rec_bytes();
void launch_gen_split(hipStream_t st, int n_blk, long long max_rows, const GenCfg &cfg, const long long *m_off,
                      const int *m_pairs, const int *blk_img, const int *blk_nb, const int *blk_slot,
                      const long long *seg_off, const Cam *cams, const Seg *segs, const PairRec *pairs,
                      const long long *blk_line_base, CRec *st_r, double *st_unc, unsigned *st_key,
                      unsigned *wave_count, unsigned *cnt_bl, int lds_segs, int lds_segs1, void *st_row,
                      unsigned *surv_count, long long n_segs, void *gates, void *blkrec, hipEvent_t *ev3,
                      const double *seg_vp, const unsigned char *seg_has_vp, const long long *seg_pt_off,
                      const void *seg_pts, const double *sfm_xyz, int *err_flag, int many_on, int one_on,
                      const long long *group_base, int phase, int ln_slots, const unsigned short *tr,
                      const unsigned *run_len, const unsigned *slot_row0, unsigned *blk_surv, const unsigned *blk_rnd0,
                      unsigned *round_count, const int *blk_vorder, unsigned *tri_unit_ctr);
size_t seg_point_bytes();
void launch_node_prefix(hipStream_t st, long long G, const int *node_img, const long long *seg_off,
                        const long long *nb_off, const long long *blk_line_base, unsigned *cnt_bl,
                        unsigned *base_bl, unsigned *n_tris, long long *tri_off, unsigned long long *status,
                        int *err_flag, void *node_rec);
void launch_expand_rows(hipStream_t st, int n_blk, const void *desc, const unsigned *stream, const unsigned *ovf, unsigned *rows);
void launch_place(hipStream_t st, int n_blk, long long max_rows, const long long *m_off, const int *blk_img,
                  const long long *seg_off, const long long *blk_line_base, const unsigned *base_bl,
                  const unsigned *wave_count, const long long *tri_off, const CRec *st_r, const double *st_unc,
                  const unsigned *st_key, CRec *cand, double *cand_unc, unsigned *cand_node, const long long *group_base,
                  unsigned *perm, const unsigned *blk_surv, const unsigned *blk_rnd0, const unsigned *round_count);
void launch_pack_keys(hipStream_t st, int n_blk, long long max_rows, const long long *m_off,
                      const unsigned *wave_count, const long long *wave_pos, const unsigned *st_key,
                      unsigned *keys_c, unsigned *src_c, const long long *group_base);
void launch_permute(hipStream_t st, long long C, const unsigned *skeys, const unsigned *ssrc, const CRec *st_r,
                    const double *st_unc, CRec *cand, double *cand_unc, unsigned *cand_node);
void launch_host_view(hipStream_t st, long long C, const unsigned *perm, const CRec *rec, const double *unc, Cand *out_c,
                      CandLite *out_l);
void launch_cand_node(hipStream_t st, long long G, const long long *tri_off, unsigned *cand_node);
size_t score3_lds_bytes(int max_nb, bool f32);
size_t cand_meta_bytes();
void launch_score3(hipStream_t st, long long C, long long G, const long long *tri_off, const unsigned *cand_node,
                   void *meta, const CRec *cand, const int *node_img, const long long *nb_off,
                   const int *blk_order, const Cam *cams, double *score, unsigned long long *pair_counter,
                   int max_nb, const ScoreCfg &cfg, double scaleinv_guard2, hipEvent_t ev_before, unsigned *draw,
                   bool f32, unsigned *perm, void *rng, bool perm_is_placement, unsigned *bucket_cnt,
                   unsigned *bucket_list, unsigned bucket_cap, const unsigned *place, unsigned *rec, const float *st_z,
                   int *err_flag, void *sp_slots, int sp_slot_cap, unsigned *sp_cnt, unsigned *sp_ovf, void *sp_pairs,
                   void *sp_desc, long long sp_chunks, hipEvent_t ev_after, const void *node_rec, unsigned *pc_cnt,
                   void *pc_list, unsigned pc_cap, int one_kernel);
size_t score_split_chunk_bytes();
size_t score_split_entry_bytes();
long long score_split_chunks(long long C);
int score3_tile_buckets();
}

namespace lt_trace {
struct Range {
  bool on;
  explicit Range(const char *name);
  ~Range();
};
}
#define LT_CONCAT2(a, b) a##b
#define LT_CONCAT(a, b) LT_CONCAT2(a, b)
#define LT_RANGE(name) lt_trace::Range LT_CONCAT(lt_range_, __LINE__)(name)

namespace lt_impl {
const char *test_switch(const char *name);
int fine_level();
bool fine_timers();
bool fine_gen_timers();
double now_ms();
double multiplier(double score_th);
lt::LinkCfg2 make_l2(const lt_config &c);
lt::LinkCfg3 make_l3(const lt_config &c);
lt::GenCfg make_gen(const lt_ctx *ctx);
lt::ScoreCfg make_score(const lt_ctx *ctx);
int bits_for(long long n);
void build_job_tables(lt_ctx *ctx);
int upload_points(lt_ctx *ctx);
int finish_run(lt_ctx *ctx);
void define_best_of_other_images(lt_ctx *ctx);
int materialize_compact(lt_ctx *ctx);
int refine_with_ctx_cams(lt_ctx *ctx, int64_t n_tracks, const double *line6, const int64_t *off, const int32_t *img,
                         const double *line2d4, const double *line3d6, const lt_refine_config *cfg);
}

#define LT_FINISH(ctx)                       \
  do {                                       \
    int rc_fin_ = lt_impl::finish_run(ctx);  \
    if (rc_fin_) return rc_fin_;             \
  } while (0)
```

### limap_amd/csrc/lt_kernels_score.hip

```cpp

#include "lt_devfn.h"

#include <hip/hip_ext.h>

#include <algorithm>

namespace lt {

#ifndef LT_SCORE_WIN
#define LT_SCORE_WIN 128
#endif
#ifndef LT_SCORE_RESIDENT
#define LT_SCORE_RESIDENT 16
#endif
#ifdef LT_SCORE_WAVES_PER_EU
#define LT_SCORE_OCC __attribute__((amdgpu_waves_per_eu(LT_SCORE_WAVES_PER_EU, LT_SCORE_WAVES_PER_EU)))
#else
#define LT_SCORE_OCC
#endif

#ifdef LT_TRACE
__device__ unsigned long long g_trace[4 * 4 * 65536];
#define LT_TRACE_MARK(kern, id, slot) \
  if (((kern) == 3 ? threadIdx.x == 0 : lane_id() == 0) && (id) < 65536u) g_trace[(kern) * 4 * 65536 + 4 * (id) + (slot)] = wall_clock64()
#else
#define LT_TRACE_MARK(kern, id, slot)
#endif

static inline unsigned nblk2(long long n, int bs) { return (unsigned)((n + bs - 1) / bs); }

struct CandMeta {
  unsigned off_lo, off_hi;
  unsigned n;
  unsigned nb;
};

constexpr int kTileQueues = 8;
constexpr int kTileBuckets = 32;
__device__ __forceinline__ int tile_bucket(unsigned cost_sum_n) {
  const unsigned b = cost_sum_n >> 7;
  return (int)(b < (unsigned)(kTileBuckets - 1) ? b : (unsigned)(kTileBuckets - 1));
}
__global__ void __launch_bounds__(256)
k_cand_meta(long long G, const unsigned *__restrict__ cand_node, const long long *__restrict__ tri_off,
            const int *__restrict__ node_img, const long long *__restrict__ nb_off, CandMeta *__restrict__ meta,
            unsigned *__restrict__ draw, unsigned *__restrict__ bucket_cnt, unsigned *__restrict__ bucket_list,
            unsigned bucket_cap, const uint4 *__restrict__ node_rec, unsigned *__restrict__ pc_cnt,
            uint2 *__restrict__ fifo, unsigned fifo_cap) {
  const long long C = tri_off[G];
  const long long stride = (long long)gridDim.x * blockDim.x;
  long long i = (long long)blockIdx.x * blockDim.x + threadIdx.x;
  if (pc_cnt && i < kTileQueues * kTileBuckets) pc_cnt[i * 32] = 0;
  if (i < 2 * kTileQueues + 1) draw[i * 32] = 0;
  if (fifo) {
    if (i >= 2 * kTileQueues + 1 && i < 3 * kTileQueues + 1) draw[i * 32] = 0xFFFFFFFFu;
    if (i >= 3 * kTileQueues + 1 && i < 4 * kTileQueues + 1) draw[i * 32] = 0;
    const long long per = ((C + 63) / 64 + kTileQueues - 1) / kTileQueues;
    for (long long j = i; j < per * kTileQueues; j += stride)
      fifo[(size_t)(j / per) * fifo_cap + (size_t)(j % per)] = make_uint2(0xFFFFFFFFu, 0u);
  }
  const long long C_up = (C + 63) & ~63ll;
  for (; i < C_up; i += stride) {
    unsigned n = 0, w_lo = 0, w_hi = 0;
    if (i < C) {
      const unsigned g = cand_node[i];
      CandMeta m;
      if (node_rec) {
        const uint4 r = node_rec[g];
        m.off_lo = r.x; m.off_hi = r.y; m.n = r.z; m.nb = r.w;
      } else {
        const long long off = tri_off[g];
        const int img = node_img[g];
        const long long nb0 = nb_off[img];
        m.off_lo = (unsigned)(off & 0xFFFFFFFFll);
        m.off_hi = (unsigned)(off >> 32);
        m.n = (unsigned)(tri_off[g + 1] - off);
        m.nb = ((unsigned)nb0 << 8) | (unsigned)(nb_off[img + 1] - nb0);
      }
      meta[i] = m;
      n = m.n;
      w_lo = m.off_lo; w_hi = m.off_lo + m.n;
    }
    if (bucket_cnt) {
      unsigned sum = n;
      for (int d = 32; d >= 1; d >>= 1) sum += (unsigned)__shfl_xor((int)sum, d);
      const long long base = i - lane_id();
      const int last = (int)((C - base) < 64 ? (C - base) : 64) - 1;
      const unsigned t_hi = (unsigned)__builtin_amdgcn_readlane((int)w_hi, last);
      if (lane_id() == 0) {
        const unsigned tile = (unsigned)(i >> 6);
        const int qb = (int)(tile & (kTileQueues - 1)) * kTileBuckets + tile_bucket(sum);
        const unsigned idx = atomicAdd(&bucket_cnt[qb * 32], 1u);
        if (idx < bucket_cap)
          reinterpret_cast<uint4 *>(bucket_list)[(size_t)qb * bucket_cap + idx] = uint4{tile, w_lo, t_hi, 0u};
      }
    }
  }
}

__global__ void __launch_bounds__(256)
k_cand_node(long long G, const long long *__restrict__ tri_off, unsigned *__restrict__ cand_node) {
  long long g = ((long long)blockIdx.x * blockDim.x + threadIdx.x) >> 6;
  if (g >= G) return;
  for (long long t = tri_off[g] + lane_id(); t < tri_off[g + 1]; t += 64) cand_node[t] = (unsigned)g;
}

static __device__ __forceinline__ unsigned mt_key(long long off) { return (unsigned)off & 0xFFFFFFu; }
constexpr int kSQCap = 512;
constexpr int kSQCapSplit = 384;
constexpr int kWin = LT_SCORE_WIN;

struct Score3Args {
  long long G;
  const long long *tri_off;
  const CandMeta *meta;
  const CRec *cand;
  const int *blk_order;
  const Cam *cams;
  double *score;
  unsigned long long *pair_counter;
  unsigned *draw;
  const unsigned *perm;
  const unsigned *spos;
  const unsigned *rng;
  const unsigned *bucket_cnt;
  const unsigned *bucket_list;
  unsigned bucket_cap;
  int max_nb;
  int *err_flag;
  uint4 *sp_slots;
  unsigned *sp_cnt;
  unsigned *sp_ovf;
  uint4 *sp_pairs;
  uint2 *sp_desc;
  unsigned *sp_counters;
  unsigned sp_chunk_cap;
  int sp_slot_cap;
  int sp_t_max;
  int sp_wave_lds;
  unsigned *pc_cnt;
  uint2 *pc_list;
  unsigned pc_cap;
};
__device__ __forceinline__ int pair_bucket(unsigned pairs) {
  const unsigned b = pairs >> 4;
  return (int)(b < (unsigned)(kTileBuckets - 1) ? b : (unsigned)(kTileBuckets - 1));
}

constexpr int kChunkCap = 512;
constexpr int kChunkTiles = 8;
constexpr unsigned kNoChunk = 0xFFFFFFFFu;
constexpr int kErrPairChunks = 7;
constexpr int kDenseHdrBytes = 16 + kChunkTiles * 8 + 256 * 4 + 64 * 4;

constexpr int kSortMax = 2048;

template <int kX>
static __device__ __forceinline__ unsigned lane_xor(unsigned x, int lane) {
  if constexpr (kX == 1) return (unsigned)__builtin_amdgcn_update_dpp(0, (int)x, 0xB1, 0xF, 0xF, true);
  else if constexpr (kX == 2) return (unsigned)__builtin_amdgcn_update_dpp(0, (int)x, 0x4E, 0xF, 0xF, true);
  else if constexpr (kX == 3) return (unsigned)__builtin_amdgcn_update_dpp(0, (int)x, 0x1B, 0xF, 0xF, true);
  else if constexpr (kX == 7) return (unsigned)__builtin_amdgcn_update_dpp(0, (int)x, 0x141, 0xF, 0xF, true);
  else if constexpr (kX == 4) return lane_xor<3>(lane_xor<7>(x, lane), lane);
  else if constexpr (kX == 8) return (unsigned)__builtin_amdgcn_update_dpp(0, (int)x, 0x128, 0xF, 0xF, true);
  else if constexpr (kX == 15) return (unsigned)__builtin_amdgcn_update_dpp(0, (int)x, 0x140, 0xF, 0xF, true);
  else if constexpr (kX == 16) {
    const auto p = __builtin_amdgcn_permlane16_swap(x, x, false, false);
    return (lane & 16) ? p[0] : p[1];
  } else if constexpr (kX == 32) {
    const auto p = __builtin_amdgcn_permlane32_swap(x, x, false, false);
    return (lane & 32) ? p[0] : p[1];
  } else {
    return (unsigned)__shfl_xor((int)x, kX);
  }
}

template <int R, int kStep, bool kMirror>
static __device__ __forceinline__ void bitonic_lanes(unsigned (&v)[R], int lane) {
  const bool lower = (lane & (kMirror ? (kStep + 1) >> 1 : kStep)) == 0;
  unsigned mn[R], mx[R];
#pragma unroll
  for (int r = 0; r < R; ++r) {
    if constexpr (!kMirror && (kStep == 16 || kStep == 32)) {
      const auto p = kStep == 16 ? __builtin_amdgcn_permlane16_swap(v[r], v[r], false, false)
                                 : __builtin_amdgcn_permlane32_swap(v[r], v[r], false, false);
      mn[r] = min(p[0], p[1]); mx[r] = max(p[0], p[1]);
    } else {
      const unsigned o = lane_xor<kStep>(v[kMirror ? R - 1 - r : r], lane);
      mn[r] = min(v[r], o); mx[r] = max(v[r], o);
    }
  }
#pragma unroll
  for (int r = 0; r < R; ++r) v[r] = lower ? mn[r] : mx[r];
}
template <int R, int K>
static __device__ __forceinline__ void bitonic_merge(unsigned (&v)[R], int lane) {
  if constexpr (K <= R) {
#pragma unroll
    for (int r = 0; r < R; ++r)
      if ((r & (K >> 1)) == 0) {
        const unsigned x = v[r], y = v[r ^ (K - 1)];
        v[r] = min(x, y);
        v[r ^ (K - 1)] = max(x, y);
      }
  } else {
    bitonic_lanes<R, K / R - 1, true>(v, lane);
  }
  if constexpr (K >= 4) {
    if constexpr (K / 4 >= 32 * R) bitonic_lanes<R, 32, false>(v, lane);
    if constexpr (K / 4 >= 16 * R) bitonic_lanes<R, 16, false>(v, lane);
    if constexpr (K / 4 >= 8 * R) bitonic_lanes<R, 8, false>(v, lane);
    if constexpr (K / 4 >= 4 * R) bitonic_lanes<R, 4, false>(v, lane);
    if constexpr (K / 4 >= 2 * R) bitonic_lanes<R, 2, false>(v, lane);
    if constexpr (K / 4 >= R) bitonic_lanes<R, 1, false>(v, lane);
#pragma unroll
    for (int j = (K / 4 < R ? K / 4 : R / 2); j > 0; j >>= 1) {
#pragma unroll
      for (int r = 0; r < R; ++r)
        if ((r & j) == 0) {
          const unsigned x = v[r], y = v[r | j];
          v[r] = min(x, y);
          v[r | j] = max(x, y);
        }
    }
  }
}
template <int R, int K>
static __device__ __forceinline__ void bitonic_from(unsigned (&v)[R], int lane) {
  bitonic_merge<R, K>(v, lane);
  if constexpr (K < R * 64) bitonic_from<R, 2 * K>(v, lane);
}
template <int R>
static __device__ __forceinline__ void wave_bitonic(unsigned (&v)[R], int lane) {
  bitonic_from<R, 2>(v, lane);
}

constexpr unsigned kDepthKeyMask = 0xFFFFF800u;
#ifndef LT_DEPTH_GROUP
#define LT_DEPTH_GROUP 4
#endif
constexpr int kDepthGroup = LT_DEPTH_GROUP;
static __device__ __forceinline__ float depth_key(unsigned w) { return __uint_as_float(w & kDepthKeyMask); }
template <bool kStrict>
static __device__ __forceinline__ int depth_bound(const unsigned *kw, int a, int b, float t) {
  while (a < b) {
    const int m = (a + b) >> 1;
    const float k = depth_key(kw[m]);
    if (kStrict ? (k <= t) : (k < t)) a = m + 1; else b = m;
  }
// ... 1476 lines not shown
      long long pos[2];
      unsigned rrec[2];
#pragma unroll
      for (int h = 0; h < 2; ++h) {
        const int ti = wave + kWaves * h;
        pos[h] = -1;
        rrec[h] = 0;
        mt[h] = CandMeta{0u, 0u, 0u, 0u};
        if (ti < nt) {
          const long long p = (long long)(unsigned)__builtin_amdgcn_readlane((int)h_tile, ti & (kChunkTiles - 1)) * 64 + lane;
          if (p < C) {
            pos[h] = p;
            if (score_by == 0) rrec[h] = a.perm ? a.perm[p] : (unsigned)p;
            mt[h] = a.meta[p];
          }
        }
      }
      __syncthreads();
      if (s_hdr[1]) return;
      LT_TRACE_MARK(3, u_cur * 8u + (unsigned)x, 1);
      int ordv[2] = {0, 0};
      long long wnb0[2] = {-1, -1};
      unsigned nb0_l[2] = {0u, 0u};
      int nn_l[2] = {0, 0};
#pragma unroll
      for (int h = 0; h < 2; ++h) {
        if (wave + kWaves * h < nt) {
          nb0_l[h] = mt[h].nb >> 8;
          nn_l[h] = pos[h] >= 0 ? (int)(mt[h].nb & 0xFFu) : 0;
          wnb0[h] = (long long)(unsigned)__builtin_amdgcn_readfirstlane((int)nb0_l[h]);
          const int n0 = __builtin_amdgcn_readfirstlane(nn_l[h]);
          if (lane < n0) ordv[h] = a.blk_order[wnb0[h] + lane];
          if (n0 > 64) wnb0[h] = -1;
        }
      }
      const int n_it3 = total > kThreads - 64 ? (total - (kThreads - 64) + kThreads - 1) / kThreads : 0;
      auto claim = [&]() {
        if (tid == kThreads - 64) c_raw = atomicAdd(q_claim, 1u);
      };
      if (n_it3 <= 1) claim();
      auto eval = [&](const uint4 e, const int k) {
        const CRec &ci = a.cand[e.y];
        const CRec &cj = a.cand[e.x];
        const int nbs_j = (int)(e.z >> 6);
        const d3 si_ = mk3(ci.s[0], ci.s[1], ci.s[2]), ei_ = mk3(ci.e[0], ci.e[1], ci.e[2]), di_ = mk3(ci.dir[0], ci.dir[1], ci.dir[2]);
        const d3 sj_ = mk3(cj.s[0], cj.s[1], cj.s[2]), ej_ = mk3(cj.e[0], cj.e[1], cj.e[2]), dj_ = mk3(cj.dir[0], cj.dir[1], cj.dir[2]);
        const Cam &camj = a.cams[(int)((unsigned)nbs_j >> 8)];
        double sc;
        if constexpr (kFast) sc = pair_score_fused(cfg, si_, ei_, di_, ci.depth[0], ci.depth[1], sj_, ej_, dj_, cj.seg, camj);
        else sc = pair_score_terms(cfg, si_, ei_, di_, ci.depth[0], ci.depth[1], sj_, ej_, dj_, cj.seg, camj);
        if (sc > 0.0)
          atomicMax(&S[(k * max_nb + (nbs_j & 0xFF)) * 64 + (int)(e.z & 63u)], (unsigned long long)__double_as_longlong(sc));
      };
      const int n_it = total > (wave << 6) ? (total - (wave << 6) + kThreads - 1) / kThreads : 0;
      for (int it = 0; it < n_it; ++it) {
        if (it > 0 && it == n_it3 - 1) claim();
        const int p = tid + it * kThreads;
        int k = k0e;
        uint4 e = e0v;
        if (it > 0) e = entry_of(p < total ? p : 0, k);
        if (p < total) eval(e, k);
      }
      for (int k = 0; k < nt; ++k) {
        if ((int)(unsigned)__builtin_amdgcn_readlane((int)h_cnt, k & (kChunkTiles - 1)) <= cap) continue;
        unsigned cc = q_word3(a.sp_slots + (size_t)(unsigned)__builtin_amdgcn_readlane((int)h_tile, k & (kChunkTiles - 1)) * (size_t)cap);
        while (cc != kNoChunk) {
          const unsigned nxt = q_word3(a.sp_pairs + (size_t)cc * kChunkCap);
          const unsigned fill = q_word3(a.sp_pairs + (size_t)cc * kChunkCap + 1);
          for (int p = tid; p < (int)fill; p += kThreads) eval(a.sp_pairs[(size_t)cc * kChunkCap + p], k);
          cc = nxt;
        }
      }
      if (tid == kThreads - 64) s_hdr[0] = d_wgs + c_raw;
      __syncthreads();
      LT_TRACE_MARK(3, u_cur * 8u + (unsigned)x, 2);
      asm volatile("" : "+v"(ordv[0]), "+v"(ordv[1]));
#pragma unroll
      for (int h = 0; h < 2; ++h) {
        const int ti = wave + kWaves * h;
        if (ti >= nt) continue;
        const bool act = pos[h] >= 0;
        const long long nb0 = (long long)nb0_l[h];
        const int n_nb = nn_l[h];
        const bool own = nb0 == wnb0[h];
        const int n_max = wave_max_i32(n_nb);
        double sum = 0.0;
        if (!__any(act && !own)) {
          for (int kk0 = 0; kk0 < n_max; kk0 += kSumChunk) {
            unsigned long long v[kSumChunk];
            int sl[kSumChunk];
#pragma unroll
            for (int u = 0; u < kSumChunk; ++u) {
              const int k = kk0 + u;
              sl[u] = __builtin_amdgcn_readlane(ordv[h], k & 63);
              v[u] = k < n_nb ? S[(ti * max_nb + sl[u]) * 64 + lane] : 0ull;
            }
#pragma unroll
            for (int u = 0; u < kSumChunk; ++u) sum += __longlong_as_double((long long)v[u]);
#pragma unroll
            for (int u = 0; u < kSumChunk; ++u)
              if (kk0 + u < n_nb) S[(ti * max_nb + sl[u]) * 64 + lane] = 0ull;
          }
        } else {
          for (int k = 0; k < n_nb; ++k) {
            unsigned long long *cell = &S[(ti * max_nb + a.blk_order[nb0 + k]) * 64 + lane];
            sum += __longlong_as_double((long long)*cell);
            *cell = 0ull;
          }
        }
        if (act) a.score[score_by == 1 ? pos[h] : (score_by == 2 ? (long long)a.spos[pos[h]] : (long long)rrec[h])] = sum;
      }
      LT_TRACE_MARK(3, u_cur * 8u + (unsigned)x, 3);
      u_cur = (unsigned)__builtin_amdgcn_readfirstlane((int)s_hdr[0]);
    }
  }
  if (tid < 64) {
    unsigned long long np = (unsigned long long)n_pairs_wg;
    for (int d = 32; d >= 1; d >>= 1) np += (unsigned long long)__shfl_xor((long long)np, d);
    if (tid == 0) {
      if (a.pair_counter && np) atomicAdd(a.pair_counter, np);
      unsigned xcc = 0;
      asm volatile("s_getreg_b32 %0, hwreg(HW_REG_XCC_ID)" : "=s"(xcc));
      xcc &= 0xFu;
      const unsigned seen = atomicCAS(&a.draw[(2 * kTileQueues + 1 + x) * 32], kFifoEmpty, xcc);
      if (seen != kFifoEmpty && seen != xcc && a.err_flag) atomicCAS(a.err_flag, 0, kErrXcdMap);
    }
  }
}

#ifdef LT_TRACE
int score_read_trace(unsigned long long *host, size_t n) {
  if (n < 4 * 4 * 65536) return -1;
  return (int)hipMemcpyFromSymbol(host + 2 * 4 * 65536, HIP_SYMBOL(g_trace), (size_t)2 * 4 * 65536 * 8,
                                  (size_t)2 * 4 * 65536 * 8, hipMemcpyDeviceToHost);
}
#endif
void launch_cand_node(hipStream_t st, long long G, const long long *tri_off, unsigned *cand_node) {
  if (G > 0)
    hipLaunchKernelGGL(k_cand_node, dim3(nblk2(G * 64, 256)), dim3(256), 0, st, G, tri_off, cand_node);
}
size_t score3_lds_bytes(int max_nb, bool f32) {
  const size_t base = (f32 ? (size_t)kWin * 48 : (size_t)9 * kWin * 8 + (size_t)kWin * 4) + 64 * 8 + kSQCap * 4;
  return ((base + (size_t)max_nb * 4 + 15) & ~(size_t)15) + (size_t)max_nb * 64 * 8;
}
size_t cand_meta_bytes() { return sizeof(CandMeta); }
int score_split_t_max(int max_nb) {
  const int t = (kDenseLdsBudget) / (std::max(max_nb, 1) * 512);
  return std::max(1, std::min(kChunkTiles, t));
}
size_t score_split_chunk_bytes() { return (size_t)kChunkCap * 16; }
size_t score_split_entry_bytes() { return 16; }
long long score_split_chunks(long long C) { return C / kChunkCap + 1024; }
int score3_tile_buckets() { return kTileBuckets * kTileQueues; }
void launch_score3(hipStream_t st, long long C, long long G, const long long *tri_off, const unsigned *cand_node,
                   void *meta, const CRec *cand, const int *node_img, const long long *nb_off,
                   const int *blk_order, const Cam *cams, double *score, unsigned long long *pair_counter,
                   int max_nb, const ScoreCfg &cfg, double scaleinv_guard2, hipEvent_t ev_before, unsigned *draw,
                   bool f32, unsigned *perm, void *rng, bool perm_is_placement, unsigned *bucket_cnt,
                   unsigned *bucket_list, unsigned bucket_cap, const unsigned *place, unsigned *rec, const float *st_z,
                   int *err_flag, void *sp_slots, int sp_slot_cap, unsigned *sp_cnt, unsigned *sp_ovf, void *sp_pairs,
                   void *sp_desc, long long sp_chunks, hipEvent_t ev_after, const void *node_rec, unsigned *pc_cnt,
                   void *pc_list, unsigned pc_cap, int one_kernel) {
  if (C <= 0) return;
  const bool dense_tables = (one_kernel & 4) != 0;
  const bool few_rows = (one_kernel & 8) != 0;
  one_kernel &= 3;
  const bool q_form = one_kernel != 0 && sp_slots != nullptr && f32 && perm != nullptr && perm_is_placement && rng == nullptr &&
                      bucket_cnt != nullptr && pc_list != nullptr;
  static int n_cu = 0;
  if (n_cu == 0) {
    int dev = 0;
    if (hipGetDevice(&dev) != hipSuccess ||
        hipDeviceGetAttribute(&n_cu, hipDeviceAttributeMultiprocessorCount, dev) != hipSuccess || n_cu <= 0)
      n_cu = 256;
  }
  const long long n_tiles = (C + 63) / 64;
  static const bool ev_markers = getenv("LT_EV_MARKERS") != nullptr;
  hipExtLaunchKernelGGL(k_cand_meta, dim3((unsigned)std::min<long long>(nblk2(C, 256), 16ll * n_cu)), dim3(256), 0, st,
                        nullptr, ev_markers ? nullptr : ev_before, 0, G, cand_node, tri_off, node_img, nb_off,
                        reinterpret_cast<CandMeta *>(meta), draw, bucket_cnt, bucket_list, bucket_cap,
                        reinterpret_cast<const uint4 *>(node_rec), pc_cnt,
                        q_form ? reinterpret_cast<uint2 *>(pc_list) : nullptr, pc_cap);
  hipEvent_t ev_stop = ev_markers ? nullptr : ev_after;
  Score3Args a;
  a.G = G; a.tri_off = tri_off; a.meta = reinterpret_cast<const CandMeta *>(meta); a.cand = cand;
  a.blk_order = blk_order; a.cams = cams; a.score = score; a.pair_counter = pair_counter;
  a.draw = draw;
  a.perm = perm; a.rng = reinterpret_cast<const unsigned *>(rng);
  a.spos = nullptr;
  a.bucket_cnt = bucket_cnt; a.bucket_list = bucket_list; a.bucket_cap = bucket_cap;
  a.max_nb = max_nb;
  a.err_flag = err_flag;
  const bool split = sp_slots != nullptr && f32;
  a.sp_slots = reinterpret_cast<uint4 *>(sp_slots);
  a.sp_cnt = sp_cnt;
  a.sp_ovf = sp_ovf;
  a.sp_pairs = reinterpret_cast<uint4 *>(sp_pairs);
  a.sp_desc = reinterpret_cast<uint2 *>(sp_desc);
  a.sp_counters = draw + kTileQueues * 32;
  a.sp_chunk_cap = (unsigned)std::max<long long>(0, std::min<long long>(sp_chunks, 0x7FFFFFFFll));
  a.sp_slot_cap = sp_slot_cap;
  a.sp_t_max = score_split_t_max(max_nb);
  const bool use_pc = split && bucket_cnt != nullptr && pc_cnt != nullptr && pc_list != nullptr;
  a.pc_cnt = use_pc ? pc_cnt : nullptr;
  a.pc_list = reinterpret_cast<uint2 *>(pc_list);
  a.pc_cap = pc_cap;
  if (ev_before && ev_markers) (void)hipEventRecord(ev_before, st);
  const bool sorted = perm != nullptr && f32 && !perm_is_placement;
  if (sorted && G > 0) {
    const double guard = scaleinv_guard2 < 1e299 ? std::sqrt(scaleinv_guard2) : 1e300;
    hipLaunchKernelGGL(k_depth_order<true>, dim3((unsigned)G), dim3(64), 0, st, G, tri_off, cand, guard, perm,
                       reinterpret_cast<unsigned *>(rng), place, rec, place ? st_z : nullptr);
    hipLaunchKernelGGL(k_depth_order<false>, dim3((unsigned)G), dim3(64), 0, st, G, tri_off, cand, guard, perm,
                       reinterpret_cast<unsigned *>(rng), place, rec, place ? st_z : nullptr);
  }
  if (sorted && place) {
    a.perm = rec;
    a.spos = perm;
  }
  const size_t lds = split ? (size_t)kWin * 48 + 64 * 8 + (size_t)kSQCapSplit * 8 + 64 * 4 : score3_lds_bytes(max_nb, f32);
  const long long per_cu = std::max<long long>(1, std::min<long long>(LT_SCORE_RESIDENT, (long long)(160 * 1024 / lds)));
  const dim3 grid((unsigned)std::min<long long>(n_tiles, per_cu * n_cu)), block(64);
  if (split && q_form) {
    a.pc_cnt = nullptr;
    const size_t ldsq = (size_t)kQHdrBytes + std::max((size_t)kDenseWaves * (size_t)kQSweepWaveBytes, (size_t)a.sp_t_max * (size_t)max_nb * 512);
    static int occ_q[2] = {0, 0};
    static size_t occ_q_lds[2] = {0, 0};
    const int v = cfg.fast ? 1 : 0;
    if (occ_q[v] == 0 || occ_q_lds[v] != ldsq) {
      int o = 0;
      hipError_t e = v ? hipOccupancyMaxActiveBlocksPerMultiprocessor(&o, k_score_q<true, true>, 64 * kDenseWaves, ldsq)
                       : hipOccupancyMaxActiveBlocksPerMultiprocessor(&o, k_score_q<false, true>, 64 * kDenseWaves, ldsq);
      occ_q[v] = (e == hipSuccess && o > 0) ? o : 1;
      occ_q_lds[v] = ldsq;
    }
    const long long slots = std::max<long long>(8, ((long long)occ_q[v] * n_cu) & ~7ll);
    const long long n_sw = std::max<long long>(8, std::min<long long>(slots, ((n_tiles + kDenseWaves - 1) / kDenseWaves + 7) & ~7ll));
    const long long n_units_b = (n_tiles + a.sp_t_max - 1) / a.sp_t_max;
    const long long n_de = std::max<long long>(0, std::min<long long>(slots - n_sw, (n_units_b + 7) & ~7ll));
    const dim3 gq((unsigned)(n_sw + n_de));
    if (cfg.fast) hipExtLaunchKernelGGL((k_score_q<true, true>), gq, dim3(64 * kDenseWaves), ldsq, st, nullptr, ev_stop, 0, a, cfg, scaleinv_guard2, 1, (unsigned)n_sw, one_kernel == 2 ? 1 : 0);
    else hipExtLaunchKernelGGL((k_score_q<false, true>), gq, dim3(64 * kDenseWaves), ldsq, st, nullptr, ev_stop, 0, a, cfg, scaleinv_guard2, 1, (unsigned)n_sw, one_kernel == 2 ? 1 : 0);
    if (ev_after && ev_markers) (void)hipEventRecord(ev_after, st);
    return;
  }
  if (split) {
    static int occ_split[3] = {0, 0, 0};
    const int var = perm_is_placement ? 0 : (sorted ? 1 : 2);
    if (occ_split[var] == 0) {
      int o = 0;
      const size_t ldsw = lds * kSweepWaves;
      hipError_t e = var == 0 ? hipOccupancyMaxActiveBlocksPerMultiprocessor(&o, k_score3<true, false, true, true>, 64 * kSweepWaves, ldsw)
                   : var == 1 ? hipOccupancyMaxActiveBlocksPerMultiprocessor(&o, k_score3<true, true, false, true>, 64 * kSweepWaves, ldsw)
                              : hipOccupancyMaxActiveBlocksPerMultiprocessor(&o, k_score3<true, false, false, true>, 64 * kSweepWaves, ldsw);
      occ_split[var] = (e == hipSuccess && o > 0) ? o : 8;
    }
    a.sp_wave_lds = (int)lds;
    const dim3 grid1((unsigned)std::max<long long>(1, std::min<long long>((n_tiles + kSweepWaves - 1) / kSweepWaves, (long long)occ_split[var] * n_cu)));
    const dim3 block1(64 * kSweepWaves);
    const size_t lds1 = lds * kSweepWaves;
    if (perm_is_placement) hipLaunchKernelGGL((k_score3<true, false, true, true>), grid1, block1, lds1, st, a, cfg, scaleinv_guard2);
    else if (sorted) hipLaunchKernelGGL((k_score3<true, true, false, true>), grid1, block1, lds1, st, a, cfg, scaleinv_guard2);
    else hipLaunchKernelGGL((k_score3<true, false, false, true>), grid1, block1, lds1, st, a, cfg, scaleinv_guard2);
    const size_t lds2 = (size_t)kDenseHdrBytes + (size_t)a.sp_t_max * (size_t)max_nb * 512;
    const long long fit = std::max<long long>(1, std::min<long long>(kDensePerCU, (long long)(160 * 1024 / lds2)));
    const int by = perm_is_placement ? 1 : (sorted && a.spos ? 2 : 0);
    const int rows_cap = few_rows ? 64 : kDenseLdsBudget / (std::max(max_nb, 1) * 8);
    if (sorted && !use_pc && bucket_cnt == nullptr && rows_cap >= 64 && !dense_tables) {
      const size_t lds3 = (size_t)((kRowsHdrBytes + 15) & ~15) + (size_t)rows_cap * (size_t)max_nb * 8;
      const long long fit3 = std::max<long long>(1, std::min<long long>(kDensePerCU, (long long)(160 * 1024 / lds3)));
      const dim3 g3((unsigned)std::max<long long>(8, (fit3 * n_cu) & ~7ll));
      if (cfg.fast) hipExtLaunchKernelGGL(k_dense_rows<true>, g3, dim3(64 * kDenseWaves), lds3, st, nullptr, ev_stop, 0, a, cfg, by, rows_cap);
      else hipExtLaunchKernelGGL(k_dense_rows<false>, g3, dim3(64 * kDenseWaves), lds3, st, nullptr, ev_stop, 0, a, cfg, by, rows_cap);
      if (ev_after && ev_markers) (void)hipEventRecord(ev_after, st);
      return;
    }
    const dim3 g2((unsigned)std::max<long long>(8, (fit * n_cu) & ~7ll));
    if (cfg.fast) hipExtLaunchKernelGGL(k_dense8<true>, g2, dim3(64 * kDenseWaves), lds2, st, nullptr, ev_stop, 0, a, cfg, by);
    else hipExtLaunchKernelGGL(k_dense8<false>, g2, dim3(64 * kDenseWaves), lds2, st, nullptr, ev_stop, 0, a, cfg, by);
    if (ev_after && ev_markers) (void)hipEventRecord(ev_after, st);
    return;
  }
  if (perm_is_placement) {
    if (f32) hipExtLaunchKernelGGL((k_score3<true, false, true, false>), grid, block, lds, st, nullptr, ev_stop, 0, a, cfg, scaleinv_guard2);
    else hipExtLaunchKernelGGL((k_score3<false, false, true, false>), grid, block, lds, st, nullptr, ev_stop, 0, a, cfg, scaleinv_guard2);
  } else if (sorted) hipExtLaunchKernelGGL((k_score3<true, true, false, false>), grid, block, lds, st, nullptr, ev_stop, 0, a, cfg, scaleinv_guard2);
  else if (f32) hipExtLaunchKernelGGL((k_score3<true, false, false, false>), grid, block, lds, st, nullptr, ev_stop, 0, a, cfg, scaleinv_guard2);
  else hipExtLaunchKernelGGL((k_score3<false, false, false, false>), grid, block, lds, st, nullptr, ev_stop, 0, a, cfg, scaleinv_guard2);
  if (ev_after && ev_markers) (void)hipEventRecord(ev_after, st);
}

}
```

### limap_amd/csrc/lt_kernels_v2.hip

```cpp

#include "lt_devfn.h"

#include <algorithm>

namespace lt {

#ifndef LT_GEN_CHUNKS
#define LT_GEN_CHUNKS 5
#endif
#ifndef LT_GATE_WAVES
#define LT_GATE_WAVES 8
#endif
#ifndef LT_GATE_WAVES_PER_EU
#define LT_GATE_WAVES_PER_EU 4
#endif
#define LT_GATE_OCC __attribute__((amdgpu_waves_per_eu(LT_GATE_WAVES_PER_EU, LT_GATE_WAVES_PER_EU)))
constexpr int kGenChunks = LT_GEN_CHUNKS;
constexpr int kRowsPerWave = 64 * kGenChunks;
constexpr int kGateWaves = LT_GATE_WAVES;
#ifndef LT_TRI_SLOTS
#define LT_TRI_SLOTS 4
#endif
constexpr int kTriSlots = LT_TRI_SLOTS;
#ifndef LT_TRI_WAVES
#define LT_TRI_WAVES 4
#endif
constexpr int kTriWaves = LT_TRI_WAVES;
constexpr int kTriRows = kTriSlots * kRowsPerWave;
static_assert(kGateWaves % kTriSlots == 0, "a group must not straddle k_gates workgroups' slot ranges");

#ifdef LT_TRACE
__device__ unsigned long long g_trace[4 * 4 * 65536];
#define LT_TRACE_MARK(kern, id, slot) \
  if (lane_id() == 0 && (id) < 65536u) g_trace[(kern) * 4 * 65536 + 4 * (id) + (slot)] = wall_clock64()
#else
#define LT_TRACE_MARK(kern, id, slot)
#endif

struct GenArgs {
  const long long *m_off;
  const int *m_pairs;
  const int *blk_img, *blk_nb, *blk_slot;
  const long long *seg_off;
  const Cam *cams;
  const Seg *segs;
  const SegGate *gates;
  const PairRec *pairs;
  const long long *blk_line_base;
  uint2 *st_row;
  unsigned *surv_count;
  CRec *st_r;
  double *st_unc;
  unsigned *st_key;
  unsigned *wave_count;
  unsigned *cnt_bl;
  const struct BlkRec *blk;
  int n_blk;
  int n_slots;
  int lds_segs;
  int lds_segs1;
  const double *seg_vp;
  const unsigned char *seg_has_vp;
  const long long *seg_pt_off;
  const SegPoint *seg_pts;
  const double *sfm_xyz;
  int *err_flag;
  const long long *group_base;
  int count_only;
  int many_on, one_on;
  const unsigned short *tr;
  const unsigned *run_len;
  const unsigned *slot_row0;
};
static __device__ __forceinline__ long long slot_first_row(const unsigned *__restrict__ slot_row0, int n_slots, int b, int s,
                                                           long long rb) {
  return slot_row0 ? (long long)slot_row0[(size_t)b * n_slots + s] : rb + (long long)s * kRowsPerWave;
}


struct BlkRec {
  long long rb, re;
  long long g1, g2;
  long long lbase;
  int M2;
  int i1, i2, nbslot;
  int M1;
  int pad_;
};
static_assert(sizeof(BlkRec) == 64, "BlkRec layout");

__global__ void k_build_blk(int n_blk, const long long *__restrict__ m_off, const int *__restrict__ blk_img,
                            const int *__restrict__ blk_nb, const int *__restrict__ blk_slot,
                            const long long *__restrict__ seg_off, const long long *__restrict__ blk_line_base,
                            BlkRec *__restrict__ out) {
  int b = blockIdx.x * blockDim.x + threadIdx.x;
  if (b >= n_blk) return;
  BlkRec r;
  r.rb = m_off[b]; r.re = m_off[b + 1];
  r.i1 = blk_img[b]; r.i2 = blk_nb[b]; r.nbslot = blk_slot[b];
  r.g1 = seg_off[r.i1]; r.g2 = seg_off[r.i2];
  r.M2 = (int)(seg_off[r.i2 + 1] - r.g2);
  r.lbase = blk_line_base[b];
  r.M1 = (int)(seg_off[r.i1 + 1] - r.g1);
  r.pad_ = 0;
  out[b] = r;
}

constexpr int kExpandWaves = 4;
__global__ void __launch_bounds__(64 * kExpandWaves)
k_expand_rows(int n_blk, const RowDesc *__restrict__ desc, const unsigned *__restrict__ stream,
              const unsigned *__restrict__ ovf, unsigned *__restrict__ rows) {
  const int b = blockIdx.x;
  if (b >= n_blk) return;
  const RowDesc d = desc[b];
  const int lane = lane_id();
  const int wave = threadIdx.x >> 6;
  unsigned *out = rows + d.row_off;
  if (d.ooff >= 0) {
    for (int r = threadIdx.x; r < d.n; r += 64 * kExpandWaves) out[r] = ovf[d.ooff + r];
    return;
  }
  const long long nbw = ((((long long)d.n + 1) / 2) + 1) & ~1ll;
  const unsigned short *nb = reinterpret_cast<const unsigned short *>(stream + d.coff);
  const unsigned long long *bits = reinterpret_cast<const unsigned long long *>(stream + d.coff + nbw);
  const int n_words = (d.n + 63) >> 6;
  unsigned base = (unsigned)d.line0;
  for (int w0 = 0; w0 < n_words; w0 += 64) {
    const unsigned long long mine = (w0 + lane < n_words) ? bits[w0 + lane] : 0ull;
    const unsigned cnt = (unsigned)__popcll(mine);
    unsigned incl = cnt;
#pragma unroll
    for (int s = 1; s < 64; s <<= 1) {
      const unsigned o = __shfl_up(incl, s, 64);
      if (lane >= s) incl += o;
    }
    const unsigned first = base + incl - cnt;
    const int k_end = min(64, n_words - w0);
#pragma unroll 4
    for (int k = wave; k < k_end; k += kExpandWaves) {
      const unsigned long long w = __shfl(mine, k, 64);
      const unsigned lb = __shfl(first, k, 64);
      const int r = ((w0 + k) << 6) + lane;
      const unsigned line = lb + (unsigned)__popcll(w & ((2ull << lane) - 1ull));
      if (r < d.n) out[r] = (line & 0xFFFFu) | ((unsigned)nb[r] << 16);
    }
    base += __shfl(incl, 63, 64);
  }
}

template <bool kLds1, bool kLds2>
__global__ void __launch_bounds__(64 * kGateWaves) LT_GATE_OCC
k_gates(GenArgs a, GenCfg cfg, const BlkRec *__restrict__ blk_r, const PairRec *__restrict__ pairs_r) {
  extern __shared__ __align__(16) unsigned char smem_raw[];
  double2 *T2 = reinterpret_cast<double2 *>(smem_raw);
// ... 582 lines not shown
          (void)one_points(true, p);
          p += n_one;
        }
        if (okx[w]) {
          GenOut ov;
          (void)extra(w, &ov);
          ov.r.nb_slot = lite_pack(nbslot, i2);
          ov.r.ng_line = ng;
          a.st_r[p] = ov.r;
          a.st_unc[p] = ov.unc;
          a.st_key[p] = (unsigned)(g1 + line);
          ++p;
        }
      }
      if (wr && a.cnt_bl && mine) atomicAdd(&a.cnt_bl[lbase + line], mine);
      if (ok && wr) {
        a.st_r[p] = o.r;
        a.st_unc[p] = o.unc;
        a.st_key[p] = (unsigned)(g1 + line);
        if (a.cnt_bl) atomicAdd(&a.cnt_bl[lbase + line], 1u);
      }
    } else {
      static_assert(sizeof(CRec) == 8 * 16, "record size in 16-byte units");
      double2 *Lc = reinterpret_cast<double2 *>(smem_raw) + (size_t)wave * (64 * 9 + 16);
      double *Lu = reinterpret_cast<double *>(Lc + 64 * 8);
      unsigned *Lk = reinterpret_cast<unsigned *>(Lu + 64);
      if (ok) {
        const double2 *oc = reinterpret_cast<const double2 *>(&o.r);
#pragma unroll
        for (int k = 0; k < 8; ++k) Lc[below * 8 + k] = oc[k];
        Lu[below] = o.unc;
        Lk[below] = (unsigned)(g1 + line);
        if (a.cnt_bl) atomicAdd(&a.cnt_bl[lbase + line], 1u);
      }
      wave_lds_sync();
      const long long p0 = out0 + wcount;
      double2 *dc = reinterpret_cast<double2 *>(a.st_r + p0);
      for (unsigned u = lane; u < total * 8u; u += 64) dc[u] = Lc[u];
      if ((unsigned)lane < total) {
        a.st_unc[p0 + lane] = Lu[lane];
        a.st_key[p0 + lane] = Lk[lane];
      }
      wave_lds_sync();
    }
    wcount += total;
#ifdef LT_TRACE
    if (e0 == 0) LT_TRACE_MARK(1, lin, 3);
#endif
  }
  LT_TRACE_MARK(1, lin, 2);
  if (lane == 0) a.wave_count[lin] = wcount;
}

__global__ void __launch_bounds__(64 * kTriWaves) __attribute__((amdgpu_waves_per_eu(4, 4)))
k_tri_rounds(GenArgs a, GenCfg cfg, const Cam *__restrict__ cams_r, const PairRec *__restrict__ pairs_r,
             const BlkRec *__restrict__ blk_r, const unsigned *__restrict__ blk_surv, const unsigned *__restrict__ blk_rnd0,
             unsigned *__restrict__ round_count, const int *__restrict__ vorder, unsigned *__restrict__ unit_ctr) {
  extern __shared__ __align__(16) unsigned char smem_raw[];
  const int wave = threadIdx.x >> 6;
  const int lane = lane_id();
  const bool xcd_major = vorder != nullptr && (gridDim.x & 7u) == 0u;
  const int n8 = xcd_major ? (a.n_blk + 7) / 8 : a.n_blk;
  const int v_begin = xcd_major ? (int)(blockIdx.x & 7u) * n8 : 0;
  const int v_end = xcd_major ? min(a.n_blk, v_begin + n8) : a.n_blk;
  const int v_step = xcd_major ? (int)(gridDim.x >> 3) : (int)gridDim.x;
  const bool claims = xcd_major && unit_ctr != nullptr && (long long)a.n_blk >= 4ll * (long long)gridDim.x;
  unsigned *ctr = claims ? unit_ctr + 32u * (blockIdx.x & 7u) : nullptr;
  const unsigned n_static = claims ? (gridDim.x >> 3) * (unsigned)kTriWaves : 0u;
  unsigned c_raw = 0;
  bool first = true;
  int v = v_begin + (xcd_major ? (int)(blockIdx.x >> 3) : (int)blockIdx.x);
  int x_dyn = -1;
  for (;;) {
  if (claims) {
    if (!first) {
      const unsigned u = n_static + (unsigned)__builtin_amdgcn_readfirstlane((int)c_raw);
      v = v_begin + (int)(u / (unsigned)kTriWaves);
      x_dyn = (int)(u % (unsigned)kTriWaves);
    }
    if (v >= v_end) break;
    if (lane == 0) c_raw = atomicAdd(ctr, 1u);
  } else {
    if (!first) v += v_step;
    if (v >= v_end) break;
  }
  first = false;
  const int b = vorder ? vorder[v] : v;
  const int x = x_dyn >= 0 ? x_dyn : (wave + b) % kTriWaves;
  const unsigned n_s = blk_surv[b];
  const int n_rounds = (int)((n_s + 63u) >> 6);
  if (x >= n_rounds) continue;
  const BlkRec *rec = blk_r + b;
  const long long rb = rec->rb;
  const unsigned rnd0 = blk_rnd0[b];
  const int i1 = rec->i1, i2 = rec->i2, nbslot = rec->nbslot;
  const long long g1 = rec->g1, g2 = rec->g2;
  const PairRec *pr = pairs_r + b;
  const long long lbase = rec->lbase;
  for (int r = x; r < n_rounds; r += kTriWaves) {
    LT_TRACE_MARK(1, rnd0 + (unsigned)r, 0);
    const unsigned e = 64u * (unsigned)r + (unsigned)lane;
    bool ok = false;
    GenOut o;
    int line = 0;
    if (e < n_s) {
      const uint2 u = a.st_row[rb + e];
      line = (int)(u.x & 0x7FFFFFFFu);
      const int ng = (int)u.y;
#ifdef LT_TRACE
      if (line >= 0) LT_TRACE_MARK(1, rnd0 + (unsigned)r, 1);
#endif
      const Seg &s1 = a.segs[g1 + line];
      const Seg &s2 = a.segs[g2 + ng];
      ok = true;
      if (u.x >> 31) ok = gen_gates(cfg, s1, s2, pr->F);
      if (ok) ok = gen_finish(cfg, cams_r[i1], cams_r[i2], s1, s2, pr->B, &o);
      o.r.nb_slot = lite_pack(nbslot, i2);
      o.r.ng_line = ng;
    }
    LT_TRACE_MARK(1, rnd0 + (unsigned)r, 3);
    const unsigned long long m = __ballot(ok);
    const unsigned below = (unsigned)__popcll(m & lanemask_lt());
    const unsigned total = (unsigned)__popcll(m);
    static_assert(sizeof(CRec) == 8 * 16, "record size in 16-byte units");
    double2 *Lc = reinterpret_cast<double2 *>(smem_raw) + (size_t)wave * (64 * 9 + 16);
    double *Lu = reinterpret_cast<double *>(Lc + 64 * 8);
    unsigned *Lk = reinterpret_cast<unsigned *>(Lu + 64);
    if (ok) {
      const double2 *oc = reinterpret_cast<const double2 *>(&o.r);
#pragma unroll
      for (int k = 0; k < 8; ++k) Lc[below * 8 + k] = oc[k];
      Lu[below] = o.unc;
      Lk[below] = (unsigned)(g1 + line);
      atomicAdd(&a.cnt_bl[lbase + line], 1u);
    }
    wave_lds_sync();
    const long long p0 = rb + 64ll * r;
    double2 *dc = reinterpret_cast<double2 *>(a.st_r + p0);
    for (unsigned u = lane; u < total * 8u; u += 64) dc[u] = Lc[u];
    if ((unsigned)lane < total) {
      a.st_unc[p0 + lane] = Lu[lane];
      a.st_key[p0 + lane] = Lk[lane];
    }
    if (lane == 0) round_count[rnd0 + (unsigned)r] = total;
    wave_lds_sync();
    LT_TRACE_MARK(1, rnd0 + (unsigned)r, 2);
  }
  }
}

#ifndef LT_PLACE_WG_PER_CU
#define LT_PLACE_WG_PER_CU 8
#endif
__global__ void __launch_bounds__(256)
k_place_rounds(const long long *__restrict__ m_off, const int *__restrict__ blk_img, const long long *__restrict__ seg_off,
               const long long *__restrict__ blk_line_base, const unsigned *__restrict__ base_bl,
               const long long *__restrict__ tri_off, const CRec *__restrict__ st_r, const double *__restrict__ st_unc,
               const unsigned *__restrict__ st_key, CRec *__restrict__ cand, double *__restrict__ cand_unc,
               unsigned *__restrict__ cand_node, unsigned *__restrict__ perm, const unsigned *__restrict__ blk_surv,
               const unsigned *__restrict__ blk_rnd0, const unsigned *__restrict__ round_count, int n_blk) {
  const int wave = threadIdx.x >> 6;
  const int lane = lane_id();
  for (int b = (int)blockIdx.x; b < n_blk; b += (int)gridDim.x) {
  const int x = (wave + b) & 3;
  const int n_rounds = (int)((blk_surv[b] + 63u) >> 6);
  if (x >= n_rounds) continue;
  const long long rb = m_off[b];
  const unsigned rnd0 = blk_rnd0[b];
  const long long g1 = seg_off[blk_img[b]];
  const long long lbase = blk_line_base[b];
  unsigned count_n = round_count[rnd0 + (unsigned)x];
  unsigned key_n = st_key[rb + 64ll * x + lane];
  for (int r = x; r < n_rounds; r += 4) {
    const unsigned count = count_n;
    const unsigned key_raw = key_n;
    if (r + 4 < n_rounds) {
      count_n = round_count[rnd0 + (unsigned)(r + 4)];
      key_n = st_key[rb + 64ll * (r + 4) + lane];
    }
    if (count == 0) continue;
    const long long s0 = rb + 64ll * r;
    const bool act = (unsigned)lane < count;
    const unsigned key = act ? key_raw : 0xFFFFFFFFu;
    const unsigned prev = (unsigned)__shfl_up((int)key, 1);
    const bool head = act && (lane == 0 || key != prev);
    const unsigned long long heads = __ballot(head);
    const int my_head = 63 - __builtin_clzll(heads & ((2ull << lane) - 1ull) | 1ull);
    const unsigned key0 = (unsigned)__builtin_amdgcn_readfirstlane((int)key);
    unsigned carry = 0;
    for (int pr_ = r - 1; pr_ >= 0; --pr_) {
      const unsigned pc = round_count[rnd0 + (unsigned)pr_];
      if (pc == 0) continue;
      const long long j = (long long)pc - 64 + lane;
      const bool valid = j >= 0;
      const unsigned k = valid ? st_key[rb + 64ll * pr_ + j] : 0u;
      const unsigned long long m = __ballot(valid && k == key0);
      const unsigned lead = m == ~0ull ? 64u : (unsigned)__builtin_clzll(~m);
      carry += lead;
      if (lead < pc) break;
    }
    unsigned pos32 = 0;
    if (act) {
      const unsigned rank = (unsigned)(lane - my_head) + (my_head == 0 ? carry : 0u);
      const long long pos = tri_off[key] + base_bl[lbase + (long long)(key - g1)] + rank;
      pos32 = (unsigned)pos;
      cand_node[pos] = key;
      if (perm) perm[pos] = (unsigned)(s0 + lane);
    }
    if (perm) continue;
    const double2 *src_c = reinterpret_cast<const double2 *>(st_r + s0);
    double2 *dst_c = reinterpret_cast<double2 *>(cand);
#pragma unroll
    for (int it = 0; it < 8; ++it) {
      const unsigned u = (unsigned)it * 64u + (unsigned)lane;
      const unsigned ci = u >> 3, piece = u & 7u;
      const unsigned p = (unsigned)__shfl((int)pos32, (int)ci);
      if (u < count * 8u) dst_c[(size_t)p * 8u + piece] = src_c[u];
    }
    if (act) cand_unc[pos32] = st_unc[s0 + lane];
  }
  }
}

__global__ void __launch_bounds__(256)
k_node_prefix(long long G, const int *__restrict__ node_img, const long long *__restrict__ seg_off,
              const long long *__restrict__ nb_off, const long long *__restrict__ blk_line_base,
              unsigned *__restrict__ cnt_bl, unsigned *__restrict__ base_bl, unsigned *__restrict__ n_tris,
              long long *__restrict__ tri_off, unsigned long long *__restrict__ status, int *__restrict__ err_flag,
              uint4 *__restrict__ node_rec) {
  __shared__ unsigned s_tile;
  __shared__ long long s_wave[4];
  __shared__ long long s_prefix;
  if (threadIdx.x == 0) s_tile = (unsigned)atomicAdd(&status[0], 1ull);
  __syncthreads();
  const long long tile = s_tile;
  const long long g = tile * 256 + threadIdx.x;
  const int lane = lane_id(), wave = threadIdx.x >> 6;
  unsigned run = 0;
  unsigned nbv = 0;
  if (g < G) {
    int img = node_img[g];
    int line = (int)(g - seg_off[img]);
    const long long b0 = nb_off[img], b1 = nb_off[img + 1];
    nbv = ((unsigned)b0 << 8) | (unsigned)(b1 - b0);
    for (long long bb = b0; bb < b1; bb += 16) {
      long long e[16];
      unsigned c[16];
#pragma unroll
      for (int k = 0; k < 16; ++k) {
        e[k] = (bb + k < b1) ? blk_line_base[bb + k] + line : -1;
      }
#pragma unroll
      for (int k = 0; k < 16; ++k) c[k] = e[k] >= 0 ? cnt_bl[e[k]] : 0u;
#pragma unroll
      for (int k = 0; k < 16; ++k) {
        if (e[k] >= 0) {
          cnt_bl[e[k]] = 0;
          base_bl[e[k]] = run;
        }
        run += c[k];
      }
    }
  }
  long long incl = (long long)run;
#pragma unroll
  for (int d = 1; d < 64; d <<= 1) {
    const long long o = __shfl_up(incl, d);
    if (lane >= d) incl += o;
  }
  if (lane == 63) s_wave[wave] = incl;
  __syncthreads();
  long long wbase = 0;
  for (int w = 0; w < wave; ++w) wbase += s_wave[w];
  const long long total = s_wave[0] + s_wave[1] + s_wave[2] + s_wave[3];
  constexpr unsigned long long kMask = (1ull << 62) - 1ull;
  if (wave == 0) {
    long long prefix = 0;
    if (tile > 0) {
      if (lane == 0) atomicExch(&status[1 + tile], (1ull << 62) | (unsigned long long)total);
      long long hi = tile;
      bool done = false;
      while (!done) {
        const long long k = hi - 1 - lane;
        unsigned long long v = 2ull << 62;
        if (k >= 0) {
          int budget = 1 << 22;
          do {
            v = atomicAdd(&status[1 + k], 0ull);
          } while ((v >> 62) == 0ull && --budget > 0);
          if ((v >> 62) == 0ull) {
            *err_flag = 4;
            v = 2ull << 62;
          }
        }
        const unsigned long long incl_lanes = __ballot((v >> 62) == 2ull);
        const int first = incl_lanes ? __builtin_ctzll(incl_lanes) : 64;
        long long part = (lane <= first) ? (long long)(v & kMask) : 0ll;
        for (int d = 32; d >= 1; d >>= 1) part += __shfl_xor(part, d);
        prefix += part;
        if (first < 64) done = true;
        else hi -= 64;
      }
    }
    if (lane == 0) {
      atomicExch(&status[1 + tile], (2ull << 62) | (unsigned long long)(prefix + total));
      s_prefix = prefix;
    }
  }
  __syncthreads();
  const long long off = s_prefix + wbase + incl - (long long)run;
  if (g <= G) {
    tri_off[g] = off;
    n_tris[g] = run;
  }
  if (node_rec && g < G) node_rec[g] = uint4{(unsigned)(off & 0xFFFFFFFFll), (unsigned)(off >> 32), run, nbv};
}

template <int kTS>
__global__ void __launch_bounds__(256)
k_place(const long long *__restrict__ m_off, const int *__restrict__ blk_img,
        const long long *__restrict__ seg_off, const long long *__restrict__ blk_line_base,
        const unsigned *__restrict__ base_bl, const unsigned *__restrict__ wave_count,
        const long long *__restrict__ tri_off, const CRec *__restrict__ st_r,
        const double *__restrict__ st_unc, const unsigned *__restrict__ st_key, CRec *__restrict__ cand,
        double *__restrict__ cand_unc, unsigned *__restrict__ cand_node, int n_groups,
        const long long *__restrict__ group_base, unsigned *__restrict__ perm,
        const unsigned *__restrict__ slot_row0) {
  const int wave = threadIdx.x >> 6;
  const int lane = lane_id();
  const int b = blockIdx.y;
  const int g = blockIdx.x * 4 + wave;
  if (g >= n_groups) return;
  const int n_slots = n_groups * kTS;
  const long long rb = m_off[b], re = m_off[b + 1];
  const long long r0 = slot_first_row(slot_row0, n_slots, b, g * kTS, rb);
  if (r0 >= re) return;
  const unsigned lin = (unsigned)b * (unsigned)n_groups + (unsigned)g;
  const unsigned count = wave_count[lin];
  if (count == 0) return;
  const long long g1 = seg_off[blk_img[b]];
  const long long lbase = blk_line_base[b];
  const long long s0 = group_base ? group_base[lin] : r0;
  static_assert(sizeof(CRec) == 8 * 16, "record size in 16-byte units");
  for (unsigned e0 = 0; e0 < count; e0 += 64) {
    const unsigned e = e0 + lane;
    const bool act = e < count;
    unsigned pos32 = 0;
    const unsigned key = act ? st_key[s0 + e] : 0xFFFFFFFFu;
    const unsigned prev = (unsigned)__shfl_up((int)key, 1);
    const bool head = act && (lane == 0 || key != prev);
    const unsigned long long heads = __ballot(head);
    const int my_head = 63 - __builtin_clzll(heads & ((2ull << lane) - 1ull) | 1ull);
    const unsigned key0 = (unsigned)__builtin_amdgcn_readfirstlane((int)key);
    unsigned carry = 0;
    {
      long long cur_r0 = r0;
      int cur_g = g;
      long long idx_end = (long long)e0;
      unsigned cur_lin = lin;
      while (true) {
        bool more = true;
        while (idx_end > 0) {
          const long long j = idx_end - 64 + lane;
          const bool valid = j >= 0;
          const unsigned k = valid ? st_key[(group_base ? group_base[cur_lin] : cur_r0) + j] : 0u;
          const unsigned long long m = __ballot(valid && k == key0);
          const unsigned lead = m == ~0ull ? 64u : (unsigned)__builtin_clzll(~m);
          carry += lead;
          const long long n_valid = idx_end < 64 ? idx_end : 64;
          if ((long long)lead < n_valid) { more = false; break; }
          idx_end -= n_valid;
        }
        if (!more) break;
        if (cur_g == 0) break;
        cur_g -= 1;
        cur_r0 = slot_first_row(slot_row0, n_slots, b, cur_g * kTS, rb);
        cur_lin -= 1;
        idx_end = (long long)wave_count[cur_lin];
      }
    }
    if (act) {
      const unsigned rank = (unsigned)(lane - my_head) + (my_head == 0 ? carry : 0u);
      const long long toff = tri_off[key];
      const long long pos = toff + base_bl[lbase + (long long)(key - g1)] + rank;
      pos32 = (unsigned)pos;
      cand_node[pos] = key;
      if (perm) perm[pos] = (unsigned)(s0 + e);
    }
    if (perm) continue;
    const unsigned nb = min(64u, count - e0);
    const double2 *src_c = reinterpret_cast<const double2 *>(st_r + s0 + e0);
    double2 *dst_c = reinterpret_cast<double2 *>(cand);
#pragma unroll
    for (int it = 0; it < 8; ++it) {
      const unsigned u = (unsigned)it * 64u + (unsigned)lane;
      const unsigned ci = u >> 3, piece = u & 7u;
      const unsigned p = (unsigned)__shfl((int)pos32, (int)ci);
      if (u < nb * 8u) dst_c[(size_t)p * 8u + piece] = src_c[u];
    }
    if (act) cand_unc[pos32] = st_unc[s0 + e];
  }
}

__global__ void __launch_bounds__(256)
k_pack_keys(const long long *__restrict__ m_off, const unsigned *__restrict__ wave_count,
            const long long *__restrict__ wave_pos, const unsigned *__restrict__ st_key,
            unsigned *__restrict__ keys_c, unsigned *__restrict__ src_c, int n_groups,
            const long long *__restrict__ group_base) {
  const int wave = threadIdx.x >> 6;
  const int lane = lane_id();
  const int b = blockIdx.y;
  const int g = blockIdx.x * 4 + wave;
  if (g >= n_groups) return;
  const long long rb = m_off[b], re = m_off[b + 1];
  const long long r0 = rb + (long long)g * kTriRows;
  if (r0 >= re) return;
  const unsigned lin = (unsigned)b * (unsigned)n_groups + (unsigned)g;
  const unsigned count = wave_count[lin];
  const long long base = wave_pos[lin];
  for (unsigned e = lane; e < count; e += 64) {
    const long long s0 = group_base ? group_base[lin] : r0;
    keys_c[base + e] = st_key[s0 + e];
    src_c[base + e] = (unsigned)(s0 + e);
  }
}

__global__ void k_permute(long long C, const unsigned *__restrict__ skeys, const unsigned *__restrict__ ssrc,
                          const CRec *__restrict__ st_r, const double *__restrict__ st_unc,
                          CRec *__restrict__ cand, double *__restrict__ cand_unc, unsigned *__restrict__ cand_node) {
  long long t = (long long)blockIdx.x * blockDim.x + threadIdx.x;
  if (t >= C) return;
  unsigned src = ssrc[t];
  cand[t] = st_r[src];
  cand_unc[t] = st_unc[src];
  cand_node[t] = skeys[t];
}

__global__ void k_host_view(long long C, const unsigned *__restrict__ perm, const CRec *__restrict__ rec,
                            const double *__restrict__ unc, Cand *__restrict__ out_c, CandLite *__restrict__ out_l) {
  long long t = (long long)blockIdx.x * blockDim.x + threadIdx.x;
  if (t >= C) return;
  const long long src = perm ? (long long)perm[t] : t;
  Cand c;
  CandLite l;
  crec_split(rec[src], unc[src], &c, &l);
  out_c[t] = c;
  out_l[t] = l;
}

static inline unsigned nblk2(long long n, int bs) { return (unsigned)((n + bs - 1) / bs); }

int gen_slots(long long max_rows) {
  long long n = (max_rows + kRowsPerWave - 1) / kRowsPerWave;
  n = (n + kGateWaves - 1) / kGateWaves * kGateWaves;
  return (int)n;
}
int gen_groups(long long max_rows) { return gen_slots(max_rows) / kTriSlots; }
int gen_slots_ln(int max_own_segs) {
  int n = (max_own_segs + 63) / 64;
  return std::max((n + kGateWaves - 1) / kGateWaves * kGateWaves, kGateWaves);
}
int gen_max_run() { return kMaxRun; }
void launch_rows_ln(hipStream_t st, int n_blk, int n_slots, const void *desc, const unsigned *stream,
                    const long long *blk_line_base, unsigned *rstart, int *blk_nruns, unsigned *run_len,
                    unsigned *slot_row0, unsigned short *tr, int *ln_flag) {
  if (n_blk <= 0) return;
  hipLaunchKernelGGL(k_rows_starts, dim3((unsigned)n_blk), dim3(256), 0, st, n_blk, reinterpret_cast<const RowDesc *>(desc),
                     stream, blk_line_base, rstart, blk_nruns, ln_flag);
  hipLaunchKernelGGL(k_rows_transpose, dim3(nblk2(n_slots, 4), (unsigned)n_blk), dim3(256), 0, st, n_blk, n_slots,
                     reinterpret_cast<const RowDesc *>(desc), stream, blk_line_base, rstart, blk_nruns, run_len, slot_row0, tr,
                     ln_flag);
}
#ifdef LT_TRACE
int score_read_trace(unsigned long long *host, size_t n);
extern "C" int lt_debug_read_trace(unsigned long long *host, size_t n) {
  const int rc = (int)hipMemcpyFromSymbol(host, HIP_SYMBOL(g_trace), n * 8, 0, hipMemcpyDeviceToHost);
  return rc ? rc : score_read_trace(host, n);
}
#endif
size_t seg_gate_bytes() { return sizeof(SegGate); }
size_t seg_point_bytes() { return sizeof(SegPoint); }
size_t blk_rec_bytes() { return sizeof(BlkRec); }
void launch_expand_rows(hipStream_t st, int n_blk, const void *desc, const unsigned *stream, const unsigned *ovf, unsigned *rows) {
  if (n_blk > 0)
    hipLaunchKernelGGL(k_expand_rows, dim3((unsigned)n_blk), dim3(64 * kExpandWaves), 0, st, n_blk, reinterpret_cast<const RowDesc *>(desc), stream,
                       ovf, rows);
}
void launch_build_blk(hipStream_t st, int n_blk, const long long *m_off, const int *blk_img, const int *blk_nb,
                      const int *blk_slot, const long long *seg_off, const long long *blk_line_base, void *blkrec) {
  if (n_blk > 0)
    hipLaunchKernelGGL(k_build_blk, dim3(nblk2(n_blk, 128)), dim3(128), 0, st, n_blk, m_off, blk_img, blk_nb, blk_slot,
                       seg_off, blk_line_base, reinterpret_cast<BlkRec *>(blkrec));
}
void launch_gen_split(hipStream_t st, int n_blk, long long max_rows, const GenCfg &cfg, const long long *m_off,
                      const int *m_pairs, const int *blk_img, const int *blk_nb, const int *blk_slot,
                      const long long *seg_off, const Cam *cams, const Seg *segs, const PairRec *pairs,
                      const long long *blk_line_base, CRec *st_r, double *st_unc, unsigned *st_key,
                      unsigned *wave_count, unsigned *cnt_bl, int lds_segs, int lds_segs1, void *st_row,
                      unsigned *surv_count, long long n_segs, void *gates, void *blkrec, hipEvent_t *ev3,
                      const double *seg_vp, const unsigned char *seg_has_vp, const long long *seg_pt_off,
                      const void *seg_pts, const double *sfm_xyz, int *err_flag, int many_on, int one_on,
                      const long long *group_base, int phase, int ln_slots, const unsigned short *tr,
                      const unsigned *run_len, const unsigned *slot_row0, unsigned *blk_surv, const unsigned *blk_rnd0,
                      unsigned *round_count, const int *blk_vorder, unsigned *tri_unit_ctr) {
  if (n_blk <= 0 || max_rows <= 0) return;
  static int n_cu = 0;
  if (n_cu == 0) {
    int dev = 0;
    if (hipGetDevice(&dev) != hipSuccess ||
        hipDeviceGetAttribute(&n_cu, hipDeviceAttributeMultiprocessorCount, dev) != hipSuccess || n_cu <= 0)
      n_cu = 256;
  }
  GenArgs a;
  a.m_off = m_off; a.m_pairs = m_pairs; a.blk_img = blk_img; a.blk_nb = blk_nb; a.blk_slot = blk_slot;
  a.seg_off = seg_off; a.cams = cams; a.segs = segs; a.gates = reinterpret_cast<const SegGate *>(gates);
  a.pairs = pairs; a.blk_line_base = blk_line_base; a.st_row = reinterpret_cast<uint2 *>(st_row); a.surv_count = surv_count;
  a.st_r = st_r; a.st_unc = st_unc; a.st_key = st_key; a.wave_count = wave_count; a.cnt_bl = cnt_bl;
  const bool ln = ln_slots > 0;
  a.n_slots = ln ? ln_slots : gen_slots(max_rows); a.lds_segs = lds_segs; a.lds_segs1 = lds_segs1;
  a.tr = ln ? tr : nullptr; a.run_len = ln ? run_len : nullptr; a.slot_row0 = ln ? slot_row0 : nullptr;
  a.seg_vp = seg_vp; a.seg_has_vp = seg_has_vp;
  a.seg_pt_off = seg_pt_off; a.seg_pts = reinterpret_cast<const SegPoint *>(seg_pts); a.sfm_xyz = sfm_xyz;
  a.err_flag = err_flag;
  const bool extra = seg_vp || seg_pts;
  a.group_base = extra ? group_base : nullptr;
  a.count_only = (extra && phase == 1) ? 1 : 0;
  a.many_on = many_on; a.one_on = one_on;
  a.blk = reinterpret_cast<const BlkRec *>(blkrec); a.n_blk = n_blk;
  const bool ln_w4 = ln && (size_t)lds_segs * sizeof(SegGate) <= 40 * 1024;
  const int gate_waves = ln ? (ln_w4 ? 4 : 8) : kGateWaves;
  const long long n_items = (long long)n_blk * (a.n_slots / gate_waves);
  const size_t lds = ln ? (size_t)lds_segs * sizeof(SegGate) : (size_t)(lds_segs + lds_segs1) * sizeof(SegGate);
  int per_cu = std::max(16 / gate_waves, 1);
  if (lds > 0) per_cu = (int)std::max<size_t>(std::min<size_t>(160 * 1024 / lds, (size_t)per_cu), 1);
  const unsigned n_wg = (unsigned)std::min<long long>(n_items, (long long)n_cu * per_cu);
  const dim3 grid(n_wg), block(64 * gate_waves);
  if (ev3 && phase != 2) (void)hipEventRecord(ev3[0], st);
  if (phase != 2 && ln) {
    if (ln_w4)
      hipLaunchKernelGGL((k_gates_ln<4>), grid, block, lds, st, a, cfg, a.blk, a.pairs, a.tr, a.run_len, a.slot_row0, a.st_row,
                         blk_surv, blk_vorder);
    else
      hipLaunchKernelGGL((k_gates_ln<8>), grid, block, lds, st, a, cfg, a.blk, a.pairs, a.tr, a.run_len, a.slot_row0, a.st_row,
                         blk_surv, blk_vorder);
  } else if (phase != 2) {
    if (lds_segs1 > 0 && lds_segs > 0) hipLaunchKernelGGL((k_gates<true, true>), grid, block, lds, st, a, cfg, a.blk, a.pairs);
    else if (lds_segs > 0) hipLaunchKernelGGL((k_gates<false, true>), grid, block, lds, st, a, cfg, a.blk, a.pairs);
    else if (lds_segs1 > 0) hipLaunchKernelGGL((k_gates<true, false>), grid, block, lds, st, a, cfg, a.blk, a.pairs);
    else hipLaunchKernelGGL((k_gates<false, false>), grid, block, lds, st, a, cfg, a.blk, a.pairs);
  }
  if (ev3 && phase != 2) (void)hipEventRecord(ev3[1], st);
  const size_t tri_lds = kTriWaves * (64 * 9 + 16) * sizeof(double2);
  if (ln) {
    const dim3 tg((unsigned)std::min<long long>(n_blk, (long long)n_cu * (16 / kTriWaves)));
    hipLaunchKernelGGL(k_tri_rounds, tg, dim3(64 * kTriWaves), tri_lds, st, a, cfg, a.cams, a.pairs, a.blk, blk_surv, blk_rnd0,
                       round_count, blk_vorder, tri_unit_ctr);
  } else {
    const dim3 tg(nblk2(a.n_slots / kTriSlots, kTriWaves), n_blk);
    if (extra)
      hipLaunchKernelGGL((k_tri_rows<true, kTriSlots>), tg, dim3(64 * kTriWaves), 0, st, a, cfg, a.cams, a.pairs, a.blk, a.slot_row0);
    else
      hipLaunchKernelGGL((k_tri_rows<false, kTriSlots>), tg, dim3(64 * kTriWaves), tri_lds, st, a, cfg, a.cams, a.pairs, a.blk,
                         a.slot_row0);
  }
  if (ev3 && phase != 1) (void)hipEventRecord(ev3[2], st);
}
void launch_node_prefix(hipStream_t st, long long G, const int *node_img, const long long *seg_off,
                        const long long *nb_off, const long long *blk_line_base, unsigned *cnt_bl,
                        unsigned *base_bl, unsigned *n_tris, long long *tri_off, unsigned long long *status,
                        int *err_flag, void *node_rec) {
  hipLaunchKernelGGL(k_node_prefix, dim3(nblk2(G + 1, 256)), dim3(256), 0, st, G, node_img, seg_off, nb_off,
                     blk_line_base, cnt_bl, base_bl, n_tris, tri_off, status, err_flag, reinterpret_cast<uint4 *>(node_rec));
}
void launch_place(hipStream_t st, int n_blk, long long max_rows, const long long *m_off, const int *blk_img,
                  const long long *seg_off, const long long *blk_line_base, const unsigned *base_bl,
                  const unsigned *wave_count, const long long *tri_off, const CRec *st_r, const double *st_unc,
                  const unsigned *st_key, CRec *cand, double *cand_unc, unsigned *cand_node, const long long *group_base,
                  unsigned *perm, const unsigned *blk_surv, const unsigned *blk_rnd0, const unsigned *round_count) {
  if (n_blk <= 0 || max_rows <= 0) return;
  if (round_count) {
    static int n_cu = 0;
    if (n_cu == 0) {
      int dev = 0;
      if (hipGetDevice(&dev) != hipSuccess ||
          hipDeviceGetAttribute(&n_cu, hipDeviceAttributeMultiprocessorCount, dev) != hipSuccess || n_cu <= 0)
        n_cu = 256;
    }
    hipLaunchKernelGGL(k_place_rounds, dim3((unsigned)std::min<long long>(n_blk, (long long)n_cu * LT_PLACE_WG_PER_CU)), dim3(256), 0, st, m_off,
                       blk_img, seg_off, blk_line_base, base_bl, tri_off, st_r, st_unc, st_key, cand, cand_unc, cand_node, perm,
                       blk_surv, blk_rnd0, round_count, n_blk);
    return;
  }
  const int n_groups = gen_groups(max_rows);
  hipLaunchKernelGGL(k_place<kTriSlots>, dim3(nblk2(n_groups, 4), n_blk), dim3(256), 0, st, m_off, blk_img, seg_off,
                     blk_line_base, base_bl, wave_count, tri_off, st_r, st_unc, st_key, cand, cand_unc, cand_node, n_groups,
                     group_base, perm, (const unsigned *)nullptr);
}
void launch_pack_keys(hipStream_t st, int n_blk, long long max_rows, const long long *m_off,
                      const unsigned *wave_count, const long long *wave_pos, const unsigned *st_key,
                      unsigned *keys_c, unsigned *src_c, const long long *group_base) {
  if (n_blk <= 0 || max_rows <= 0) return;
  const int n_groups = gen_groups(max_rows);
  hipLaunchKernelGGL(k_pack_keys, dim3(nblk2(n_groups, 4), n_blk), dim3(256), 0, st, m_off, wave_count, wave_pos,
                     st_key, keys_c, src_c, n_groups, group_base);
}
void launch_permute(hipStream_t st, long long C, const unsigned *skeys, const unsigned *ssrc, const CRec *st_r,
                    const double *st_unc, CRec *cand, double *cand_unc, unsigned *cand_node) {
  if (C > 0)
    hipLaunchKernelGGL(k_permute, dim3(nblk2(C, 256)), dim3(256), 0, st, C, skeys, ssrc, st_r, st_unc, cand, cand_unc,
                       cand_node);
}
void launch_host_view(hipStream_t st, long long C, const unsigned *perm, const CRec *rec, const double *unc, Cand *out_c,
                      CandLite *out_l) {
  if (C > 0) hipLaunchKernelGGL(k_host_view, dim3(nblk2(C, 256)), dim3(256), 0, st, C, perm, rec, unc, out_c, out_l);
}
}
```

Before: 2.519 billion.

## Fuse candidate metadata into node prefix and tile lists into place kernel

k_node_prefix now writes the per-candidate CandMeta records directly, one per triangle run, and the separate k_cand_meta launch is skipped. The tile-bucket list building and score-stage counter resets move into extra workgroups of k_place_rounds, interleaved with the placement workgroups, and cand_node writes are dropped on this path. The goal is to remove a kernel launch and one pass over cand_node/meta ahead of scoring. In exchange, node_prefix threads with long runs do serial stores, and the list-building workgroups take slots away from placement.

```diff
diff --git a/limap_amd/csrc/lt_api_run.cpp b/limap_amd/csrc/lt_api_run.cpp
--- a/limap_amd/csrc/lt_api_run.cpp
+++ b/limap_amd/csrc/lt_api_run.cpp
@@ -1,4 +1,6 @@
 #include "lt_host.h"
+
+#include <functional>
 
 using namespace lt;
 using namespace lt_impl;
@@ -341,6 +343,9 @@
                      n_status, ln_job ? ctx->d_blk_surv.as<unsigned>() : nullptr);
 
   bool node_rec_valid = false;
+  bool meta_fused = false;
+  std::function<void(const lt::PlaceLists *, hipEvent_t)> place_args;
+  static const bool ev_markers = getenv("LT_EV_MARKERS") != nullptr;
   long long C_known = -1;
   long long C_bound = 0;
   int ev_gen_end = 3, ev_place_end = 4;
@@ -449,21 +454,26 @@
     if (!hC) hC = &hC_fallback;
     if (fast) {
       ENSURE(ctx, ctx->d_node_rec, 16 * (size_t)std::max<long long>(G, 1));
-      launch_node_prefix(st, G, ctx->d_node_img.as<int>(), ctx->d_seg_off.as<long long>(),
-                         ctx->d_nb_off.as<long long>(), ctx->d_blk_line_base.as<long long>(),
-                         ctx->d_cnt_bl.as<unsigned>(), ctx->d_base_bl.as<unsigned>(), ctx->d_ntris_u.as<unsigned>(),
-                         ctx->d_tri_off.as<long long>(), ctx->d_scan_status.as<unsigned long long>(),
-                         ctx->d_err.as<int>(), ctx->d_node_rec.p);
-      node_rec_valid = true;
-      ctx->cnt_bl_clean = true;
       const long long bound = P;
       constexpr long long kCountFreeBytes = 48ll << 30;
       const bool perm_bound = !test_switch("LT_TEST_PLACE_COPY");
       const long long per_cand = (perm_bound ? 4 : (long long)(sizeof(CRec) + 8)) + 8 + 4 + 4 + (long long)cand_meta_bytes() +
                                  (long long)score_split_entry_bytes() * 256 / 64;
+      const bool count_free = !extras && ctx->h_pinned && bound * per_cand <= kCountFreeBytes && !test_switch("LT_TEST_SYNC_COUNT");
+      meta_fused = ln && count_free && perm_bound && ctx->n_blk > 0 && ctx->max_rows > 0 && bound > 0 &&
+                   !test_switch("LT_TEST_SEPARATE_CAND_META") && ctx->d_cand_meta.ensure(cand_meta_bytes() * (size_t)bound);
+      if (!meta_fused) (void)hipGetLastError();
+      launch_node_prefix(st, G, ctx->d_node_img.as<int>(), ctx->d_seg_off.as<long long>(),
+                         ctx->d_nb_off.as<long long>(), ctx->d_blk_line_base.as<long long>(),
+                         ctx->d_cnt_bl.as<unsigned>(), ctx->d_base_bl.as<unsigned>(), ctx->d_ntris_u.as<unsigned>(),
+                         ctx->d_tri_off.as<long long>(), ctx->d_scan_status.as<unsigned long long>(),
+                         ctx->d_err.as<int>(), ctx->d_node_rec.p,
+                         meta_fused ? ctx->d_cand_meta.p : nullptr);
+      node_rec_valid = true;
+      ctx->cnt_bl_clean = true;
       if (extras) {
         C_known = staged_total;
-      } else if (ctx->h_pinned && bound * per_cand <= kCountFreeBytes && !test_switch("LT_TEST_SYNC_COUNT")) {
+      } else if (count_free) {
         C_known = -1;
         C_bound = bound;
       } else {
@@ -509,13 +519,16 @@
     ENSURE(ctx, ctx->d_score, 8 * Cn); ENSURE(ctx, ctx->d_edge_flag, 4 * Cn); ENSURE(ctx, ctx->d_cand_node, 4 * Cn);
     ctx->cand_cap = (long long)Cn;
     if (fast) {
+      place_args = [=](const lt::PlaceLists *lists, hipEvent_t ev_stop) {
       launch_place(st, ctx->n_blk, ctx->max_rows, ctx->d_m_off.as<long long>(), ctx->d_blk_img.as<int>(),
                    ctx->d_seg_off.as<long long>(), ctx->d_blk_line_base.as<long long>(),
                    ctx->d_base_bl.as<unsigned>(), ctx->d_wave_count.as<unsigned>(), ctx->d_tri_off.as<long long>(),
                    ctx->d_st_c.as<CRec>(), ctx->d_st_l.as<double>(), ctx->d_st_key.as<unsigned>(),
-                   ctx->d_cand.as<CRec>(), ctx->d_lite.as<double>(), ctx->d_cand_node.as<unsigned>(), group_base,
+                   ctx->d_cand.as<CRec>(), ctx->d_lite.as<double>(), lists ? nullptr : ctx->d_cand_node.as<unsigned>(), group_base,
                    perm_mode ? ctx->d_place_perm.as<unsigned>() : nullptr, ctx->d_blk_surv.as<unsigned>(),
-                   ctx->d_blk_rnd0.as<unsigned>(), ln ? ctx->d_round_count.as<unsigned>() : nullptr);
+                   ctx->d_blk_rnd0.as<unsigned>(), ln ? ctx->d_round_count.as<unsigned>() : nullptr, lists, ev_stop);
+      };
+      if (!meta_fused) place_args(nullptr, nullptr);
     } else {
       ENSURE(ctx, ctx->d_keys, 4 * Cn); ENSURE(ctx, ctx->d_rows, 4 * Cn);
       ENSURE(ctx, ctx->d_skeys, 4 * Cn); ENSURE(ctx, ctx->d_srows, 4 * Cn);
@@ -536,7 +549,7 @@
                      ctx->d_cand_node.as<unsigned>());
     }
     if (fine_score && C_bound > 0) ev_place_end = 11;
-    else if (sampled) HIPCHK(ctx, hipEventRecord(ev[4], st));
+    else if (sampled && !meta_fused) HIPCHK(ctx, hipEventRecord(ev[4], st));
     if (gen_event_pending) ev_gen_end = ev_place_end;
   } else if (ctx->job_mode == 2) {
     ctx->perm_mode = false;
@@ -739,6 +752,21 @@
       ENSURE(ctx, ctx->d_pc_cnt, 128 * (size_t)score3_tile_buckets());
       ENSURE(ctx, ctx->d_pc_list, 8 * (size_t)tile_cap * (size_t)score3_tile_buckets());
     }
+    const int one_kernel = ((ctx->score_two_kernels || test_switch("LT_SCORE_TWO_KERNELS") || ctx->n_img >= (1 << 18))
+                                ? 0 : (test_switch("LT_TEST_Q_LOSE_TILE") ? 2 : 1)) |
+                           (test_switch("LT_TEST_DENSE_TABLES") ? 4 : 0) | (test_switch("LT_TEST_DENSE_FEW_ROWS") ? 8 : 0);
+    unsigned *const bucket_cnt = tile_classes ? (unsigned *)(ctx->d_scan_status.as<unsigned long long>() + n_status_scan) : nullptr;
+    if (meta_fused) {
+      const bool q_form = score3_q_form(one_kernel, split, score_f32, ctx->perm_mode && !staged_sorted, score_sorted, tile_classes,
+                                        pair_classes);
+      const lt::PlaceLists lists = {ctx->d_cand_meta.p, G, C_bound, ctx->d_tile_order.as<unsigned>(), bucket_cnt,
+                                    tile_classes ? ctx->d_tile_list.as<unsigned>() : nullptr,
+                                    pair_classes ? ctx->d_pc_cnt.as<unsigned>() : nullptr, q_form ? ctx->d_pc_list.p : nullptr,
+                                    tile_cap, tile_cap};
+      const hipEvent_t ev_pl = ev_place_end == 11 ? ev[11] : (sampled ? ev[4] : nullptr);
+      place_args(&lists, ev_markers ? nullptr : ev_pl);
+      if (ev_markers && ev_pl == ev[4] && sampled) HIPCHK(ctx, hipEventRecord(ev[4], st));
+    }
     launch_score3(st, C_bound, G, ctx->d_tri_off.as<long long>(), ctx->d_cand_node.as<unsigned>(), ctx->d_cand_meta.p,
                   ctx->perm_mode ? ctx->d_st_c.as<CRec>() : ctx->d_cand.as<CRec>(), ctx->d_node_img.as<int>(),
                   ctx->d_nb_off.as<long long>(), ctx->d_blk_order.as<int>(), ctx->d_cams.as<Cam>(),
@@ -747,18 +775,14 @@
                   (ctx->perm_mode && !staged_sorted) ? ctx->d_place_perm.as<unsigned>()
                                                      : (score_sorted ? ctx->d_perm.as<unsigned>() : nullptr),
                   score_sorted ? ctx->d_rng.p : nullptr, ctx->perm_mode && !staged_sorted,
-                  tile_classes ? (unsigned *)(ctx->d_scan_status.as<unsigned long long>() + n_status_scan) : nullptr,
-                  tile_classes ? ctx->d_tile_list.as<unsigned>() : nullptr, tile_cap,
+                  bucket_cnt, tile_classes ? ctx->d_tile_list.as<unsigned>() : nullptr, tile_cap,
                   staged_sorted ? ctx->d_place_perm.as<unsigned>() : nullptr,
                   staged_sorted ? ctx->d_ex_rec.as<unsigned>() : nullptr,
                   staged_sorted ? ctx->d_ex_z.as<float>() : nullptr, ctx->d_err.as<int>(),
                   split ? ctx->d_sp_slots.p : nullptr, sp_slot_cap, ctx->d_sp_cnt.as<unsigned>(),
                   ctx->d_sp_ovf.as<unsigned>(), ctx->d_sp_pairs.p, ctx->d_sp_desc.p, sp_chunks, sampled ? ev[5] : nullptr,
                   node_rec_valid ? ctx->d_node_rec.p : nullptr, pair_classes ? ctx->d_pc_cnt.as<unsigned>() : nullptr,
-                  pair_classes ? ctx->d_pc_list.p : nullptr, tile_cap,
-                  (((ctx->score_two_kernels || test_switch("LT_SCORE_TWO_KERNELS") || ctx->n_img >= (1 << 18))
-                        ? 0 : (test_switch("LT_TEST_Q_LOSE_TILE") ? 2 : 1)) |
-                   (test_switch("LT_TEST_DENSE_TABLES") ? 4 : 0) | (test_switch("LT_TEST_DENSE_FEW_ROWS") ? 8 : 0)));
+                  pair_classes ? ctx->d_pc_list.p : nullptr, tile_cap, one_kernel, meta_fused);
     if (C_bound <= 0 && sampled) HIPCHK(ctx, hipEventRecord(ev[5], st));
   }
   ENSURE(ctx, ctx->d_best_idx, 8 * (size_t)std::max<long long>(G, 1));
diff --git a/limap_amd/csrc/lt_devfn.h b/limap_amd/csrc/lt_devfn.h
--- a/limap_amd/csrc/lt_devfn.h
+++ b/limap_amd/csrc/lt_devfn.h
@@ -52,6 +52,47 @@
 static __device__ __forceinline__ void wave_lds_sync() {
   asm volatile("s_waitcnt lgkmcnt(0)" ::: "memory");
   __builtin_amdgcn_wave_barrier();
+}
+
+struct CandMeta {
+  unsigned off_lo, off_hi;
+  unsigned n;
+  unsigned nb;
+};
+static_assert(sizeof(CandMeta) == 16, "CandMeta is stored and loaded as one uint4");
+constexpr int kTileQueues = 8;
+constexpr int kTileBuckets = 32;
+__device__ __forceinline__ int tile_bucket(unsigned cost_sum_n) {
+  const unsigned b = cost_sum_n >> 7;
+  return (int)(b < (unsigned)(kTileBuckets - 1) ? b : (unsigned)(kTileBuckets - 1));
+}
+static __device__ __forceinline__ void score_stage_resets(long long i, long long stride, long long C, unsigned *__restrict__ draw,
+                                                          unsigned *__restrict__ pc_cnt, uint2 *__restrict__ fifo,
+                                                          unsigned fifo_cap) {
+  if (pc_cnt && i < kTileQueues * kTileBuckets) pc_cnt[i * 32] = 0;
+  if (i < 2 * kTileQueues + 1) draw[i * 32] = 0;
+  if (fifo) {
+    if (i >= 2 * kTileQueues + 1 && i < 3 * kTileQueues + 1) draw[i * 32] = 0xFFFFFFFFu;
+    if (i >= 3 * kTileQueues + 1 && i < 4 * kTileQueues + 1) draw[i * 32] = 0;
+    const long long per = ((C + 63) / 64 + kTileQueues - 1) / kTileQueues;
+    for (long long j = i; j < per * kTileQueues; j += stride)
+      fifo[(size_t)(j / per) * fifo_cap + (size_t)(j % per)] = make_uint2(0xFFFFFFFFu, 0u);
+  }
+}
+static __device__ __forceinline__ void tile_list_append(long long base, long long C, unsigned n, unsigned w_lo, unsigned w_hi,
+                                                        unsigned *__restrict__ bucket_cnt, unsigned *__restrict__ bucket_list,
+                                                        unsigned bucket_cap) {
+  unsigned sum = n;
+  for (int d = 32; d >= 1; d >>= 1) sum += (unsigned)__shfl_xor((int)sum, d);
+  const int last = (int)((C - base) < 64 ? (C - base) : 64) - 1;
+  const unsigned t_hi = (unsigned)__builtin_amdgcn_readlane((int)w_hi, last);
+  if (lane_id() == 0) {
+    const unsigned tile = (unsigned)(base >> 6);
+    const int qb = (int)(tile & (kTileQueues - 1)) * kTileBuckets + tile_bucket(sum);
+    const unsigned idx = atomicAdd(&bucket_cnt[qb * 32], 1u);
+    if (idx < bucket_cap)
+      reinterpret_cast<uint4 *>(bucket_list)[(size_t)qb * bucket_cap + idx] = uint4{tile, w_lo, t_hi, 0u};
+  }
 }
 
 
diff --git a/limap_amd/csrc/lt_device.h b/limap_amd/csrc/lt_device.h
--- a/limap_amd/csrc/lt_device.h
+++ b/limap_amd/csrc/lt_device.h
@@ -78,6 +78,15 @@
                    const double *cand_unc, Cand *best_c, double *best_score, int *best_src2, int *n_tris,
                    bool wide, const int *err_flag, const unsigned long long *pair_counter, long long *result3,
                    const unsigned *perm);
+
+struct PlaceLists {
+  const void *meta;
+  long long G;
+  long long C_bound;
+  unsigned *draw, *bucket_cnt, *bucket_list, *pc_cnt;
+  void *fifo;
+  unsigned bucket_cap, fifo_cap;
+};
 void launch_edge_fill(hipStream_t st, long long G, const long long *tri_off, const unsigned *edge_flag,
                       const long long *edge_off, const CRec *cand, int *edges2, const unsigned *perm);
 
diff --git a/limap_amd/csrc/lt_host.h b/limap_amd/csrc/lt_host.h
--- a/limap_amd/csrc/lt_host.h
+++ b/limap_amd/csrc/lt_host.h
@@ -52,13 +52,14 @@
 void launch_node_prefix(hipStream_t st, long long G, const int *node_img, const long long *seg_off,
                         const long long *nb_off, const long long *blk_line_base, unsigned *cnt_bl,
                         unsigned *base_bl, unsigned *n_tris, long long *tri_off, unsigned long long *status,
-                        int *err_flag, void *node_rec);
+                        int *err_flag, void *node_rec, void *cand_meta);
 void launch_expand_rows(hipStream_t st, int n_blk, const void *desc, const unsigned *stream, const unsigned *ovf, unsigned *rows);
 void launch_place(hipStream_t st, int n_blk, long long max_rows, const long long *m_off, const int *blk_img,
                   const long long *seg_off, const long long *blk_line_base, const unsigned *base_bl,
                   const unsigned *wave_count, const long long *tri_off, const CRec *st_r, const double *st_unc,
                   const unsigned *st_key, CRec *cand, double *cand_unc, unsigned *cand_node, const long long *group_base,
-                  unsigned *perm, const unsigned *blk_surv, const unsigned *blk_rnd0, const unsigned *round_count);
+                  unsigned *perm, const unsigned *blk_surv, const unsigned *blk_rnd0, const unsigned *round_count,
+                  const PlaceLists *lists, hipEvent_t ev_stop);
 void launch_pack_keys(hipStream_t st, int n_blk, long long max_rows, const long long *m_off,
                       const unsigned *wave_count, const long long *wave_pos, const unsigned *st_key,
                       unsigned *keys_c, unsigned *src_c, const long long *group_base);
@@ -77,7 +78,9 @@
                    unsigned *bucket_list, unsigned bucket_cap, const unsigned *place, unsigned *rec, const float *st_z,
                    int *err_flag, void *sp_slots, int sp_slot_cap, unsigned *sp_cnt, unsigned *sp_ovf, void *sp_pairs,
                    void *sp_desc, long long sp_chunks, hipEvent_t ev_after, const void *node_rec, unsigned *pc_cnt,
-                   void *pc_list, unsigned pc_cap, int one_kernel);
+                   void *pc_list, unsigned pc_cap, int one_kernel, bool meta_done);
+bool score3_q_form(int one_kernel, bool split, bool f32, bool perm_is_placement, bool ranges, bool tile_classes,
+                   bool pair_lists);
 size_t score_split_chunk_bytes();
 size_t score_split_entry_bytes();
 long long score_split_chunks(long long C);
diff --git a/limap_amd/csrc/lt_kernels_score.hip b/limap_amd/csrc/lt_kernels_score.hip
--- a/limap_amd/csrc/lt_kernels_score.hip
+++ b/limap_amd/csrc/lt_kernels_score.hip
@@ -29,18 +29,6 @@
 
 static inline unsigned nblk2(long long n, int bs) { return (unsigned)((n + bs - 1) / bs); }
 
-struct CandMeta {
-  unsigned off_lo, off_hi;
-  unsigned n;
-  unsigned nb;
-};
-
-constexpr int kTileQueues = 8;
-constexpr int kTileBuckets = 32;
-__device__ __forceinline__ int tile_bucket(unsigned cost_sum_n) {
-  const unsigned b = cost_sum_n >> 7;
-  return (int)(b < (unsigned)(kTileBuckets - 1) ? b : (unsigned)(kTileBuckets - 1));
-}
 __global__ void __launch_bounds__(256)
 k_cand_meta(long long G, const unsigned *__restrict__ cand_node, const long long *__restrict__ tri_off,
             const int *__restrict__ node_img, const long long *__restrict__ nb_off, CandMeta *__restrict__ meta,
@@ -50,15 +38,7 @@
   const long long C = tri_off[G];
   const long long stride = (long long)gridDim.x * blockDim.x;
   long long i = (long long)blockIdx.x * blockDim.x + threadIdx.x;
-  if (pc_cnt && i < kTileQueues * kTileBuckets) pc_cnt[i * 32] = 0;
-  if (i < 2 * kTileQueues + 1) draw[i * 32] = 0;
-  if (fifo) {
-    if (i >= 2 * kTileQueues + 1 && i < 3 * kTileQueues + 1) draw[i * 32] = 0xFFFFFFFFu;
-    if (i >= 3 * kTileQueues + 1 && i < 4 * kTileQueues + 1) draw[i * 32] = 0;
-    const long long per = ((C + 63) / 64 + kTileQueues - 1) / kTileQueues;
-    for (long long j = i; j < per * kTileQueues; j += stride)
-      fifo[(size_t)(j / per) * fifo_cap + (size_t)(j % per)] = make_uint2(0xFFFFFFFFu, 0u);
-  }
+  score_stage_resets(i, stride, C, draw, pc_cnt, fifo, fifo_cap);
   const long long C_up = (C + 63) & ~63ll;
   for (; i < C_up; i += stride) {
     unsigned n = 0, w_lo = 0, w_hi = 0;
@@ -81,20 +61,7 @@
       n = m.n;
       w_lo = m.off_lo; w_hi = m.off_lo + m.n;
     }
-    if (bucket_cnt) {
-      unsigned sum = n;
-      for (int d = 32; d >= 1; d >>= 1) sum += (unsigned)__shfl_xor((int)sum, d);
-      const long long base = i - lane_id();
-      const int last = (int)((C - base) < 64 ? (C - base) : 64) - 1;
-      const unsigned t_hi = (unsigned)__builtin_amdgcn_readlane((int)w_hi, last);
-      if (lane_id() == 0) {
-        const unsigned tile = (unsigned)(i >> 6);
-        const int qb = (int)(tile & (kTileQueues - 1)) * kTileBuckets + tile_bucket(sum);
-        const unsigned idx = atomicAdd(&bucket_cnt[qb * 32], 1u);
-        if (idx < bucket_cap)
-          reinterpret_cast<uint4 *>(bucket_list)[(size_t)qb * bucket_cap + idx] = uint4{tile, w_lo, t_hi, 0u};
-      }
-    }
+    if (bucket_cnt) tile_list_append(i - lane_id(), C, n, w_lo, w_hi, bucket_cnt, bucket_list, bucket_cap);
   }
 }
 
@@ -1877,6 +1844,10 @@
 size_t score_split_entry_bytes() { return 16; }
 long long score_split_chunks(long long C) { return C / kChunkCap + 1024; }
 int score3_tile_buckets() { return kTileBuckets * kTileQueues; }
+bool score3_q_form(int one_kernel, bool split, bool f32, bool perm_is_placement, bool ranges, bool tile_classes,
+                   bool pair_lists) {
+  return (one_kernel & 3) != 0 && split && f32 && perm_is_placement && !ranges && tile_classes && pair_lists;
+}
 void launch_score3(hipStream_t st, long long C, long long G, const long long *tri_off, const unsigned *cand_node,
                    void *meta, const CRec *cand, const int *node_img, const long long *nb_off,
                    const int *blk_order, const Cam *cams, double *score, unsigned long long *pair_counter,
@@ -1885,13 +1856,13 @@
                    unsigned *bucket_list, unsigned bucket_cap, const unsigned *place, unsigned *rec, const float *st_z,
                    int *err_flag, void *sp_slots, int sp_slot_cap, unsigned *sp_cnt, unsigned *sp_ovf, void *sp_pairs,
                    void *sp_desc, long long sp_chunks, hipEvent_t ev_after, const void *node_rec, unsigned *pc_cnt,
-                   void *pc_list, unsigned pc_cap, int one_kernel) {
+                   void *pc_list, unsigned pc_cap, int one_kernel, bool meta_done) {
   if (C <= 0) return;
   const bool dense_tables = (one_kernel & 4) != 0;
   const bool few_rows = (one_kernel & 8) != 0;
   one_kernel &= 3;
-  const bool q_form = one_kernel != 0 && sp_slots != nullptr && f32 && perm != nullptr && perm_is_placement && rng == nullptr &&
-                      bucket_cnt != nullptr && pc_list != nullptr;
+  const bool q_form = score3_q_form(one_kernel, sp_slots != nullptr, f32, perm != nullptr && perm_is_placement, rng != nullptr,
+                                    bucket_cnt != nullptr, pc_list != nullptr);
   static int n_cu = 0;
   if (n_cu == 0) {
     int dev = 0;
@@ -1901,11 +1872,12 @@
   }
   const long long n_tiles = (C + 63) / 64;
   static const bool ev_markers = getenv("LT_EV_MARKERS") != nullptr;
-  hipExtLaunchKernelGGL(k_cand_meta, dim3((unsigned)std::min<long long>(nblk2(C, 256), 16ll * n_cu)), dim3(256), 0, st,
-                        nullptr, ev_markers ? nullptr : ev_before, 0, G, cand_node, tri_off, node_img, nb_off,
-                        reinterpret_cast<CandMeta *>(meta), draw, bucket_cnt, bucket_list, bucket_cap,
-                        reinterpret_cast<const uint4 *>(node_rec), pc_cnt,
-                        q_form ? reinterpret_cast<uint2 *>(pc_list) : nullptr, pc_cap);
+  if (!meta_done)
+    hipExtLaunchKernelGGL(k_cand_meta, dim3((unsigned)std::min<long long>(nblk2(C, 256), 16ll * n_cu)), dim3(256), 0, st,
+                          nullptr, ev_markers ? nullptr : ev_before, 0, G, cand_node, tri_off, node_img, nb_off,
+                          reinterpret_cast<CandMeta *>(meta), draw, bucket_cnt, bucket_list, bucket_cap,
+                          reinterpret_cast<const uint4 *>(node_rec), pc_cnt,
+                          q_form ? reinterpret_cast<uint2 *>(pc_list) : nullptr, pc_cap);
   hipEvent_t ev_stop = ev_markers ? nullptr : ev_after;
   Score3Args a;
   a.G = G; a.tri_off = tri_off; a.meta = reinterpret_cast<const CandMeta *>(meta); a.cand = cand;
diff --git a/limap_amd/csrc/lt_kernels_v2.hip b/limap_amd/csrc/lt_kernels_v2.hip
--- a/limap_amd/csrc/lt_kernels_v2.hip
+++ b/limap_amd/csrc/lt_kernels_v2.hip
@@ -1,5 +1,7 @@
 
 #include "lt_devfn.h"
+
+#include <hip/hip_ext.h>
 
 #include <algorithm>
 
@@ -888,16 +890,52 @@
 #ifndef LT_PLACE_WG_PER_CU
 #define LT_PLACE_WG_PER_CU 8
 #endif
+struct TileLists {
+  const uint4 *meta;
+  long long G;
+  unsigned *draw, *bucket_cnt, *bucket_list, *pc_cnt;
+  uint2 *fifo;
+  unsigned bucket_cap, fifo_cap;
+  int n_wg;
+  int period;
+};
+static __device__ __forceinline__ void tile_lists_role(const TileLists &tl, const long long *__restrict__ tri_off, int wg) {
+  const long long C = tri_off[tl.G];
+  const long long stride = (long long)tl.n_wg * 256;
+  score_stage_resets((long long)wg * 256 + threadIdx.x, stride, C, tl.draw, tl.pc_cnt, tl.fifo, tl.fifo_cap);
+  if (!tl.bucket_cnt) return;
+  for (long long base = (long long)wg * 256 + (threadIdx.x & ~63u); base < C; base += stride) {
+    unsigned n = 0, w_lo = 0, w_hi = 0;
+    if (base + lane_id() < C) {
+      const uint4 m = tl.meta[base + lane_id()];
+      n = m.z;
+      w_lo = m.x; w_hi = m.x + m.z;
+    }
+    tile_list_append(base, C, n, w_lo, w_hi, tl.bucket_cnt, tl.bucket_list, tl.bucket_cap);
+  }
+}
 __global__ void __launch_bounds__(256)
 k_place_rounds(const long long *__restrict__ m_off, const int *__restrict__ blk_img, const long long *__restrict__ seg_off,
                const long long *__restrict__ blk_line_base, const unsigned *__restrict__ base_bl,
                const long long *__restrict__ tri_off, const CRec *__restrict__ st_r, const double *__restrict__ st_unc,
                const unsigned *__restrict__ st_key, CRec *__restrict__ cand, double *__restrict__ cand_unc,
                unsigned *__restrict__ cand_node, unsigned *__restrict__ perm, const unsigned *__restrict__ blk_surv,
-               const unsigned *__restrict__ blk_rnd0, const unsigned *__restrict__ round_count, int n_blk) {
+               const unsigned *__restrict__ blk_rnd0, const unsigned *__restrict__ round_count, int n_blk,
+               const TileLists tl) {
   const int wave = threadIdx.x >> 6;
   const int lane = lane_id();
-  for (int b = (int)blockIdx.x; b < n_blk; b += (int)gridDim.x) {
+  int b0 = (int)blockIdx.x;
+  if (tl.n_wg > 0) {
+    const int q = tl.period ? b0 / tl.period : b0;
+    const bool lists = q < tl.n_wg && (tl.period == 0 || b0 % tl.period == tl.period - 1);
+    if (lists) {
+      tile_lists_role(tl, tri_off, q);
+      return;
+    }
+    b0 -= q < tl.n_wg ? q : tl.n_wg;
+  }
+  const int n_place = (int)gridDim.x - tl.n_wg;
+  for (int b = b0; b < n_blk; b += n_place) {
   const int x = (wave + b) & 3;
   const int n_rounds = (int)((blk_surv[b] + 63u) >> 6);
   if (x >= n_rounds) continue;
@@ -940,7 +978,7 @@
       const unsigned rank = (unsigned)(lane - my_head) + (my_head == 0 ? carry : 0u);
       const long long pos = tri_off[key] + base_bl[lbase + (long long)(key - g1)] + rank;
       pos32 = (unsigned)pos;
-      cand_node[pos] = key;
+      if (cand_node) cand_node[pos] = key;
       if (perm) perm[pos] = (unsigned)(s0 + lane);
     }
     if (perm) continue;
@@ -963,7 +1001,7 @@
               const long long *__restrict__ nb_off, const long long *__restrict__ blk_line_base,
               unsigned *__restrict__ cnt_bl, unsigned *__restrict__ base_bl, unsigned *__restrict__ n_tris,
               long long *__restrict__ tri_off, unsigned long long *__restrict__ status, int *__restrict__ err_flag,
-              uint4 *__restrict__ node_rec) {
+              uint4 *__restrict__ node_rec, uint4 *__restrict__ cand_meta) {
   __shared__ unsigned s_tile;
   __shared__ long long s_wave[4];
   __shared__ long long s_prefix;
@@ -1049,7 +1087,14 @@
     tri_off[g] = off;
     n_tris[g] = run;
   }
-  if (node_rec && g < G) node_rec[g] = uint4{(unsigned)(off & 0xFFFFFFFFll), (unsigned)(off >> 32), run, nbv};
+  const uint4 rec = uint4{(unsigned)(off & 0xFFFFFFFFll), (unsigned)(off >> 32), run, nbv};
+  if (node_rec && g < G) node_rec[g] = rec;
+  if (cand_meta) {
+    using u32x4 = unsigned __attribute__((ext_vector_type(4)));
+    const u32x4 r4 = {rec.x, rec.y, rec.z, rec.w};
+    u32x4 *dst = reinterpret_cast<u32x4 *>(cand_meta) + off;
+    for (unsigned j = 0; j < run; ++j) dst[j] = r4;
+  }
 }
 
 template <int kTS>
@@ -1304,15 +1349,17 @@
 void launch_node_prefix(hipStream_t st, long long G, const int *node_img, const long long *seg_off,
                         const long long *nb_off, const long long *blk_line_base, unsigned *cnt_bl,
                         unsigned *base_bl, unsigned *n_tris, long long *tri_off, unsigned long long *status,
-                        int *err_flag, void *node_rec) {
+                        int *err_flag, void *node_rec, void *cand_meta) {
   hipLaunchKernelGGL(k_node_prefix, dim3(nblk2(G + 1, 256)), dim3(256), 0, st, G, node_img, seg_off, nb_off,
-                     blk_line_base, cnt_bl, base_bl, n_tris, tri_off, status, err_flag, reinterpret_cast<uint4 *>(node_rec));
+                     blk_line_base, cnt_bl, base_bl, n_tris, tri_off, status, err_flag, reinterpret_cast<uint4 *>(node_rec),
+                     reinterpret_cast<uint4 *>(cand_meta));
 }
 void launch_place(hipStream_t st, int n_blk, long long max_rows, const long long *m_off, const int *blk_img,
                   const long long *seg_off, const long long *blk_line_base, const unsigned *base_bl,
                   const unsigned *wave_count, const long long *tri_off, const CRec *st_r, const double *st_unc,
                   const unsigned *st_key, CRec *cand, double *cand_unc, unsigned *cand_node, const long long *group_base,
-                  unsigned *perm, const unsigned *blk_surv, const unsigned *blk_rnd0, const unsigned *round_count) {
+                  unsigned *perm, const unsigned *blk_surv, const unsigned *blk_rnd0, const unsigned *round_count,
+                  const PlaceLists *lists, hipEvent_t ev_stop) {
   if (n_blk <= 0 || max_rows <= 0) return;
   if (round_count) {
     static int n_cu = 0;
@@ -1322,9 +1369,23 @@
           hipDeviceGetAttribute(&n_cu, hipDeviceAttributeMultiprocessorCount, dev) != hipSuccess || n_cu <= 0)
         n_cu = 256;
     }
-    hipLaunchKernelGGL(k_place_rounds, dim3((unsigned)std::min<long long>(n_blk, (long long)n_cu * LT_PLACE_WG_PER_CU)), dim3(256), 0, st, m_off,
-                       blk_img, seg_off, blk_line_base, base_bl, tri_off, st_r, st_unc, st_key, cand, cand_unc, cand_node, perm,
-                       blk_surv, blk_rnd0, round_count, n_blk);
+    const long long slots = (long long)n_cu * LT_PLACE_WG_PER_CU;
+    TileLists tl = {};
+    long long n_place = std::min<long long>(n_blk, slots);
+    if (lists) {
+      tl.meta = reinterpret_cast<const uint4 *>(lists->meta);
+      tl.G = lists->G;
+      tl.draw = lists->draw; tl.bucket_cnt = lists->bucket_cnt; tl.bucket_list = lists->bucket_list; tl.pc_cnt = lists->pc_cnt;
+      tl.fifo = reinterpret_cast<uint2 *>(lists->fifo);
+      tl.bucket_cap = lists->bucket_cap; tl.fifo_cap = lists->fifo_cap;
+      const long long want = std::max<long long>(1, std::min<long long>((lists->C_bound + 255) / 256, n_cu));
+      n_place = std::min<long long>(n_blk, slots - want);
+      tl.n_wg = (int)want;
+      tl.period = n_place >= 4 * want ? 5 : 0;
+    }
+    hipExtLaunchKernelGGL(k_place_rounds, dim3((unsigned)(n_place + tl.n_wg)), dim3(256), 0, st, nullptr, ev_stop, 0, m_off,
+                          blk_img, seg_off, blk_line_base, base_bl, tri_off, st_r, st_unc, st_key, cand, cand_unc, cand_node, perm,
+                          blk_surv, blk_rnd0, round_count, n_blk, tl);
     return;
   }
   const int n_groups = gen_groups(max_rows);
```

Result: faster. 2.562 billion (median of 6 runs) (+1.7%).
